# sean-lo/OptimalMatrixCompletion.jl

Measured on AMD Instinct MI355X. Metric: B&B node-relaxations/sec, 100x100 k=1, higher is better.
Workload: dtype f64

## Files before the change

include/omc.h:

```cpp
#ifndef OMC_H
#define OMC_H

#include <stdint.h>

#ifdef __cplusplus
extern "C" {
#endif

#define OMC_VERSION 100

#define OMC_OPTIMAL 0
#define OMC_SLOW_PROGRESS 1
#define OMC_TIME_LIMIT 2
#define OMC_INFEASIBLE 3

#define OMC_CUT_LINEAR 0
#define OMC_CUT_LINEAR2 1
#define OMC_CUT_LINEAR3 2
#define OMC_DIR_LEFT 0
#define OMC_DIR_MIDDLE 1
#define OMC_DIR_RIGHT 2
#define OMC_DIR_INNER_LEFT 3
#define OMC_DIR_INNER_RIGHT 4
#define OMC_SMALLEST_1_EIGVEC 1
// ... 55 lines not shown
                    const double* U_upper, double* objective, double* dual_bound, int* status, int* iters,
                    double* Y, double* U, double* X, double* Theta, double* lambda_min, double* breakpoint_x,
                    double* solve_time);

int omc_relax_stage(omc_instance* h, int B, const omc_relax_params* params, int cut_type, const int* L,
                    const double* cut_x, const double* cut_Uhat, const int8_t* cut_dir, const double* U_lower,
                    const double* U_upper);
int omc_set_node_rho_scales(omc_instance* h, int B, const double* rho_scale);
int omc_relax_solve(omc_instance* h);
int omc_state_pool_create(omc_instance* h, int capacity);
int omc_state_pool_reserve_shor(omc_instance* h, int64_t nq_max);
int omc_relax_set_warm(omc_instance* h, int B, const int* load_from, const int* save_to);
int omc_shor_warm_compat(int64_t n_parent, const int64_t* parent_idx, int64_t n_soc_parent, const int64_t* parent_soc, int64_t n_child,
                         const int64_t* child_idx, int64_t n_soc_child, const int64_t* child_soc);
int omc_last_shor_warm_stats(omc_instance* h, int64_t out[4]);
int omc_state_pool_fetch_shor(omc_instance* h, int entry, int64_t* nq, double* X, double* Theta, double* V);
int omc_relax_submit(omc_instance* h);
int omc_relax_fetch_done(omc_instance* h, int max_nodes, int* node_ids, double* objective, double* dual_bound, int* status, int* iters,
                         double* U, double* lambda_min, double* breakpoint_x, double* Y, int* n_out);
int omc_relax_hold(omc_instance* h, int on);
int omc_relax_reserve(omc_instance* h, int extra_nodes, int max_cuts);
int omc_relax_append(omc_instance* h, int B, const int* L, const double* cut_x, const double* cut_Uhat, const int8_t* cut_dir,
                     const int* load_from, const int* save_to);
int omc_relax_poll(omc_instance* h, int* running, int* nodes_done, int* nodes_total);
int omc_relax_wait(omc_instance* h);
int omc_relax_fetch(omc_instance* h, double* objective, double* dual_bound, int* status, int* iters, double* Y,
                    double* U, double* X, double* Theta, double* lambda_min, double* breakpoint_x,
                    double* solve_time);

int omc_relax_stage_shor(omc_instance* h, int B, const omc_relax_params* params, int cut_type, const int* L,
                         const double* cut_x, const double* cut_Uhat, const int8_t* cut_dir, const double* U_lower,
                         const double* U_upper, const int64_t* n_shor, const int64_t* shor_idx, const int64_t* n_soc,
                         const int64_t* soc_idx);
int omc_relax_fetch_shor(omc_instance* h, double* W );
int omc_set_shor_keep_V(omc_instance* h, int keep);
int omc_relax_fetch_shor_V(omc_instance* h, double* V);
int omc_relax_batch_shor(omc_instance* h, int B, const omc_relax_params* params, int cut_type, const int* L,
                         const double* cut_x, const double* cut_Uhat, const int8_t* cut_dir, const double* U_lower,
                         const double* U_upper, const int64_t* n_shor, const int64_t* shor_idx, const int64_t* n_soc,
                         const int64_t* soc_idx, double* objective, double* dual_bound, int* status, int* iters, double* Y,
                         double* U, double* X, double* Theta, double* W, double* lambda_min, double* breakpoint_x,
                         double* solve_time);
int omc_set_shor_penalties(omc_instance* h, double rho, double r4, double r5);
int omc_relax_reserve_shor(omc_instance* h, int64_t nq_max, int extra_lists);
int omc_relax_append_shor(omc_instance* h, int B, const int* L, const double* cut_x, const double* cut_Uhat, const int8_t* cut_dir,
                          const int64_t* n_shor, const int64_t* shor_idx, const int64_t* n_soc, const int64_t* soc_idx,
                          const int* load_from, const int* save_to);
int omc_relax_fetch_done_shor(omc_instance* h, int n_ids, const int* node_ids, double* X, double* W, double* Theta);

int omc_relax_keep_certificates(omc_instance* h, int on);
int omc_relax_fetch_certificate(omc_instance* h, int n_ids, const int* node_ids, double* Lam, double* lam, int* R, double* Q, int* r,
                                double* Psi3, double* bound);
int omc_certificate_plan(int n, int k, int nnz, int max_cuts, int nonstandard_box_rows, int64_t* out);
int omc_dual_bound_batch(omc_instance* h, int B, int cut_type, int reference_quirk_q1, const int* L, const double* cut_x,
                         const double* cut_Uhat, const int8_t* cut_dir, const double* U_lower, const double* U_upper, const double* Lam,
                         const double* lam, const double* Psi3, double* Q_out, int* r_out, double* bound);

int omc_relax_keep_shor_certificates(omc_instance* h, int on);
int omc_relax_fetch_shor_certificate(omc_instance* h, int n_ids, const int* node_ids, double* scale, double* bound, double* lam, int* R, double* Q,
                                     int* r, double* Psi3, double* Gam, double* zeta, double* xi, double* Xbar, int* nq, int64_t* nq_stride);
int omc_shor_certificate_plan(int n, int m, int k, int64_t nq_stride, int max_cuts, int nonstandard_box_rows, int64_t* out);

int omc_shor_dual_bound_batch(omc_instance* h, int B, int cut_type, int reference_quirk_q1, const int* L, const double* cut_x,
                              const double* cut_Uhat, const int8_t* cut_dir, const double* U_lower, const double* U_upper, const int64_t* n_shor,
                              const int64_t* shor_idx, const int64_t* n_soc, const int64_t* soc_idx, int sanitise, int64_t nq_stride,
                              const double* scale, const double* lam, const double* Psi3, const double* Gam, const double* zeta, const double* xi,
                              const double* Xbar, double* bound, double* defects, double* terms);
int omc_shor_dual_bound_plan(int n, int m, int k, int B, int64_t nq_stride, int max_cuts, int nonstandard_box_rows, int sanitise, int64_t* out);
int omc_last_shor_dual_bound_ms(omc_instance* h, double* ms);

int omc_shor_index_build(omc_instance* h, int where, int64_t nq, const int64_t* shor_idx, int64_t n_soc, const int64_t* soc_idx, int64_t* counts,
                         double* r4, uint64_t* hash, int* mi, int* kid, int* cptr, int* cent, int* v1ptr, int* v1ent, int* v2ptr, int* v2ent,
                         int* slackrow, uint8_t* eclass, uint8_t* ctype);
int omc_shor_index_plan(int n, int m, int64_t nq, int64_t* out);
int omc_last_shor_index_stats(omc_instance* h, double* out);

int omc_altmin_batch(omc_instance* h, int B, int cut_type, int reference_quirk_q1, const int* L,
                     const double* cut_x, const double* cut_Uhat, const int8_t* cut_dir, const double* U_initial,
                     double eps, int max_iters, double time_limit, double* U, double* V, int* converged,
                     int* n_iters, double* objectives, double* solve_time);

int omc_altmin_master_objectives(omc_instance* h, int B, double* objective);
int omc_altmin_plan(int n, int m, int k, int max_cuts, int nolds, int64_t* out);

int omc_evaluate_objective(omc_instance* h, int B, const double* X, double* objective);

int omc_separation_batch(omc_instance* h, int B, int breakpoints, const double* Y, const double* U,
                         double* eigvals, double* x, int* feasible);

int omc_round_Y_batch(omc_instance* h, int B, const double* Y, double* U_rounded);
int omc_left_singular_batch(omc_instance* h, int B, const double* X, double* U_out);

int omc_psd_project_batch(omc_instance* h, int B, int N, const double* M, double lo, double hi, int algo,
                          const double* V0, double* P, double* evals, double* V);
int omc_column_prox_batch(omc_instance* h, int B, int mode, int algo, const double* Y, const double* alpha_old, const double* rho_f,
                          const double* s0, double* alpha, double* s, double* objcol, double* c0col, int* nfact);
int omc_colprox_plan(int n, int cmax, int block_min, int64_t* out);
int omc_last_cone_multi_stats(omc_instance* h, int64_t* out);
int omc_plain_multi_plan(int n, int plain_multi_min, int64_t* out);
double omc_plain_multi_tau(void);
int omc_last_plain_multi_stats(omc_instance* h, int64_t* out);
int omc_cone_multi_budget(int interval_max);
#define OMC_HARVEST_NONE 0
#define OMC_HARVEST_SYNC 1
#define OMC_HARVEST_ASYNC 2
int omc_harvest_plan(int nlive, int nfin, int pending, int check_index, int async_min_live);

int omc_shor_count(omc_instance* h, int n_classes, const int* num_entries_present, int64_t* count_per_class);
int omc_shor_indexes(omc_instance* h, int n_classes, const int* num_entries_present, int64_t capacity, int64_t* out,
                     int64_t* count);
int omc_violated_shor_minors(omc_instance* h, const double* X, int n_classes, const int* num_entries_present,
                             int64_t n_existing, const int64_t* existing, int n_minors, double* scores,
                             int64_t* minors, int* n_out);
int omc_shor_last_stats(omc_instance* h, double* ms, int64_t* candidates);
int omc_shor_last_select_stats(omc_instance* h, int64_t out[4]);

#define OMC_COMM_ID_BYTES 128
int omc_comm_unique_id(void* id_out);
int omc_comm_init(omc_instance* h, int rank, int world_size, const void* id);
int omc_allreduce_bounds(omc_instance* h, double* ub, double* lb, int* owner);
int omc_bcast_incumbent(omc_instance* h, int root, double* X);
int omc_allgather_records(omc_instance* h, const double* rows, int cnt, int width, double* out, int out_capacity_rows, int* counts);
int omc_comm_destroy(omc_instance* h);

#define OMC_KERNEL_COLPROX 0
#define OMC_KERNEL_CONE 1
#define OMC_KERNEL_GLOBAL 2
#define OMC_KERNEL_CHECK 3
#define OMC_KERNEL_SETUP 4
#define OMC_KERNEL_SMALL 5
#define OMC_KERNEL_ACCEL 6
#define OMC_KERNEL_CONESUB 7
#define OMC_KERNEL_CHECK_COL 8
#define OMC_KERNEL_CHECK_BUILD 9
#define OMC_KERNEL_HARVEST 10
#define OMC_KERNEL_SHOR_BIGCONE 11
#define OMC_KERNEL_SHOR_MINORS 12
#define OMC_KERNEL_SHOR_COLS 13
#define OMC_KERNEL_NCLASS 14
int omc_last_solver_info(omc_instance* h, double* info);
#define OMC_RES_CONE_SUB 0
#define OMC_RES_CONE_SUB_CERT 1
#define OMC_RES_CONE_SUB_SEP 2
#define OMC_RES_GLOBAL 3
#define OMC_RES_SMALL 4
#define OMC_RES_COLPROX_PAIR 5
#define OMC_RES_COLPROX_WIDE 6
#define OMC_RES_COLPROX 7
#define OMC_RES_CONE_WS 8
#define OMC_RES_CONE 9
#define OMC_RES_N 10
int omc_kernel_residency(omc_instance* h, int* out);
int omc_last_subspace_stats(omc_instance* h, int64_t* out);
int omc_last_shor_subspace_stats(omc_instance* h, int64_t* out);
int omc_tuning_set(omc_instance* h, const char* name, const char* value);
int omc_tuning_reload_env(omc_instance* h);
int omc_debug_stamps(omc_instance* h, double* out32);
int omc_debug_diag(omc_instance* h, double* out);
int omc_debug_aa(omc_instance* h, int* accepted, int* rejected);
int omc_debug_residuals(omc_instance* h, double* rp, double* rd);
int omc_last_kernel_stats(omc_instance* h, int64_t* launches , double* ms ,
                          int64_t* units );
#define OMC_HOST_CHECK_WAIT 0
#define OMC_HOST_CHECK_SCAN 1
#define OMC_HOST_LIST 2
#define OMC_HOST_EVENT_DRAIN 3
#define OMC_HOST_HARVEST_FLAGS 4
#define OMC_HOST_HARVEST_ENQUEUE 5
#define OMC_HOST_HARVEST_WAIT 6
#define OMC_HOST_HARVEST_BOOK 7
#define OMC_HOST_SETUP_ENQUEUE 8
#define OMC_HOST_CHECK_TOTAL 9
#define OMC_HOST_HARVEST_TOTAL 10
#define OMC_HOST_ASYNC_HARVESTS 11
#define OMC_HOST_QUIET_INTERVALS 12
#define OMC_HOST_BODY_RECORDS 13
#define OMC_HOST_BODY_WAITS 14
#define OMC_HOST_NPHASE 15
int omc_last_host_phases(omc_instance* h, double* ms , int64_t* count );

#ifdef __cplusplus
}
#endif
#endif
```

optimalmatrixcompletion.jl_amd/_lib.py:

```python
from __future__ import annotations

import ctypes as C
import os

import numpy as np

_HERE = os.path.dirname(os.path.abspath(__file__))
LIB_PATH = os.environ.get("OMC_AMD_LIB") or os.path.join(_HERE, "lib", "libomc_hip.so")

EXPORTS = [
    "omc_relax_params_default", "omc_last_error", "omc_version", "omc_device_count", "omc_instance_create",
    "omc_instance_create_bits", "omc_instance_destroy", "omc_relax_batch", "omc_relax_stage", "omc_relax_solve",
    "omc_relax_fetch", "omc_relax_submit", "omc_relax_poll", "omc_relax_wait", "omc_altmin_batch", "omc_evaluate_objective", "omc_separation_batch", "omc_round_Y_batch",
    "omc_last_kernel_stats", "omc_last_host_phases", "omc_kernel_residency", "omc_last_solver_info", "omc_last_subspace_stats", "omc_set_node_rho_scales", "omc_left_singular_batch", "omc_psd_project_batch", "omc_column_prox_batch", "omc_colprox_plan", "omc_last_cone_multi_stats", "omc_cone_multi_budget", "omc_plain_multi_plan", "omc_plain_multi_tau", "omc_last_plain_multi_stats", "omc_harvest_plan", "omc_relax_reserve", "omc_relax_append", "omc_relax_fetch_done", "omc_relax_hold", "omc_debug_stamps", "omc_tuning_set", "omc_tuning_reload_env", "omc_debug_residuals", "omc_debug_diag", "omc_debug_aa",
    "omc_shor_count", "omc_shor_indexes", "omc_violated_shor_minors", "omc_shor_last_stats", "omc_shor_last_select_stats",
    "omc_relax_stage_shor", "omc_relax_fetch_shor", "omc_relax_batch_shor", "omc_set_shor_penalties", "omc_set_shor_keep_V", "omc_relax_fetch_shor_V", "omc_last_shor_subspace_stats", "omc_state_pool_create", "omc_relax_set_warm",
    "omc_state_pool_reserve_shor", "omc_shor_warm_compat", "omc_last_shor_warm_stats", "omc_state_pool_fetch_shor",
    "omc_relax_reserve_shor", "omc_relax_append_shor", "omc_relax_fetch_done_shor",
    "omc_relax_keep_certificates", "omc_relax_fetch_certificate", "omc_certificate_plan", "omc_dual_bound_batch",
    "omc_relax_keep_shor_certificates", "omc_relax_fetch_shor_certificate", "omc_shor_certificate_plan",
    "omc_shor_dual_bound_batch", "omc_shor_dual_bound_plan", "omc_last_shor_dual_bound_ms",
    "omc_shor_index_build", "omc_shor_index_plan", "omc_last_shor_index_stats",
    "omc_altmin_master_objectives", "omc_altmin_plan", "omc_comm_unique_id", "omc_comm_init", "omc_allreduce_bounds", "omc_bcast_incumbent", "omc_allgather_records", "omc_comm_destroy",
]


class RelaxParams(C.Structure):
    _fields_ = [("eps_gap", C.c_double), ("eps_feas", C.c_double), ("max_iters", C.c_int), ("check_every", C.c_int),
                ("rho_scale", C.c_double), ("rho_f_ratio", C.c_double), ("relax", C.c_double), ("time_limit", C.c_double),
                ("reference_quirk_q1", C.c_int), ("breakpoints", C.c_int), ("stall_checks", C.c_int), ("bump_max", C.c_int), ("bump_ratio", C.c_double),
                ("bump_factor", C.c_double), ("bump_after", C.c_int), ("bump_window", C.c_int), ("slots", C.c_int),
                ("accel", C.c_int), ("aa_mem", C.c_int), ("aa_every", C.c_int), ("aa_start", C.c_int), ("aa_reg", C.c_double), ("aa_safeguard", C.c_double), ("first_wins", C.c_int),
                ("early_stop_after", C.c_int), ("early_stop_factor", C.c_double)]


class OmcError(RuntimeError):
    def __init__(self, code, msg):
        super().__init__(f"libomc_hip error {code}: {msg}")
        self.code = code


_lib = None


def load():
    global _lib
    if _lib is not None:
        return _lib
    if not os.path.exists(LIB_PATH):
        raise OmcError(-100, f"{LIB_PATH} not found: build it first (__graft_entry__.build()); there is no CPU fallback")
    lib = C.CDLL(LIB_PATH)
    dp = C.POINTER(C.c_double); ip = C.POINTER(C.c_int); vp = C.c_void_p
    lib.omc_last_error.restype = C.c_char_p
    lib.omc_version.restype = C.c_int
    lib.omc_device_count.restype = C.c_int
    lib.omc_relax_params_default.argtypes = [C.POINTER(RelaxParams)]
    lib.omc_instance_create.argtypes = [C.c_int, C.c_int, C.c_int, vp, vp, C.c_double, C.c_int, C.POINTER(vp)]
    lib.omc_instance_create_bits.argtypes = [C.c_int, C.c_int, C.c_int, vp, vp, C.c_double, C.c_int, C.POINTER(vp)]
    lib.omc_instance_destroy.argtypes = [vp]
    lib.omc_instance_destroy.restype = None
    lib.omc_relax_batch.argtypes = [vp, C.c_int, C.POINTER(RelaxParams), C.c_int] + [vp] * 17
    lib.omc_relax_stage.argtypes = [vp, C.c_int, C.POINTER(RelaxParams), C.c_int] + [vp] * 6
    lib.omc_relax_solve.argtypes = [vp]
    lib.omc_relax_stage_shor.argtypes = [vp, C.c_int, C.POINTER(RelaxParams), C.c_int] + [vp] * 10
    lib.omc_relax_fetch_shor.argtypes = [vp, vp]
    lib.omc_relax_batch_shor.argtypes = [vp, C.c_int, C.POINTER(RelaxParams), C.c_int] + [vp] * 22
    lib.omc_set_shor_penalties.argtypes = [vp, C.c_double, C.c_double, C.c_double]
    lib.omc_set_shor_keep_V.argtypes = [vp, C.c_int]
    lib.omc_relax_fetch_shor_V.argtypes = [vp, vp]
    lib.omc_last_shor_subspace_stats.argtypes = [vp, vp]
    lib.omc_state_pool_create.argtypes = [vp, C.c_int]
    lib.omc_relax_set_warm.argtypes = [vp, C.c_int, vp, vp]
    lib.omc_state_pool_reserve_shor.argtypes = [vp, C.c_int64]
    lib.omc_shor_warm_compat.argtypes = [C.c_int64, vp, C.c_int64, vp, C.c_int64, vp, C.c_int64, vp]
    lib.omc_last_shor_warm_stats.argtypes = [vp, vp]
    lib.omc_state_pool_fetch_shor.argtypes = [vp, C.c_int, vp, vp, vp, vp]
    lib.omc_relax_submit.argtypes = [vp]
    lib.omc_relax_poll.argtypes = [vp, vp, vp, vp]
    lib.omc_relax_wait.argtypes = [vp]
    lib.omc_relax_fetch.argtypes = [vp] + [vp] * 11
    lib.omc_altmin_batch.argtypes = [vp, C.c_int, C.c_int, C.c_int, vp, vp, vp, vp, vp, C.c_double, C.c_int, C.c_double,
                                     vp, vp, vp, vp, vp, vp]
    lib.omc_evaluate_objective.argtypes = [vp, C.c_int, vp, vp]
    lib.omc_separation_batch.argtypes = [vp, C.c_int, C.c_int, vp, vp, vp, vp, vp]
    lib.omc_round_Y_batch.argtypes = [vp, C.c_int, vp, vp]
    lib.omc_last_kernel_stats.argtypes = [vp, vp, vp, vp]
    lib.omc_last_solver_info.argtypes = [vp, vp]
    if hasattr(lib, "omc_last_host_phases"):
        lib.omc_last_host_phases.argtypes = [vp, vp, vp]
    if hasattr(lib, "omc_kernel_residency"):
        lib.omc_kernel_residency.argtypes = [vp, vp]
    lib.omc_last_subspace_stats.argtypes = [vp, vp]
    lib.omc_set_node_rho_scales.argtypes = [vp, C.c_int, vp]
    lib.omc_debug_stamps.argtypes = [vp, vp]
    lib.omc_left_singular_batch.argtypes = [vp, C.c_int, vp, vp]
    lib.omc_psd_project_batch.argtypes = [vp, C.c_int, C.c_int, vp, C.c_double, C.c_double, C.c_int, vp, vp, vp, vp]
    if hasattr(lib, "omc_column_prox_batch"):
        lib.omc_column_prox_batch.argtypes = [vp, C.c_int, C.c_int, C.c_int] + [vp] * 9
        lib.omc_colprox_plan.argtypes = [C.c_int, C.c_int, C.c_int, vp]
    lib.omc_last_cone_multi_stats.argtypes = [vp, vp]
    lib.omc_cone_multi_budget.argtypes = [C.c_int]
    if hasattr(lib, "omc_plain_multi_plan"):
        lib.omc_plain_multi_plan.argtypes = [C.c_int, C.c_int, vp]
        lib.omc_plain_multi_tau.argtypes = []
        lib.omc_plain_multi_tau.restype = C.c_double
        lib.omc_last_plain_multi_stats.argtypes = [vp, vp]
    if hasattr(lib, "omc_harvest_plan"):
        lib.omc_harvest_plan.argtypes = [C.c_int] * 5
    lib.omc_relax_reserve.argtypes = [vp, C.c_int, C.c_int]
    lib.omc_relax_hold.argtypes = [vp, C.c_int]
    lib.omc_relax_fetch_done.argtypes = [vp, C.c_int, vp, vp, vp, vp, vp, vp, vp, vp, vp, vp]
    lib.omc_relax_append.argtypes = [vp, C.c_int, vp, vp, vp, vp, vp, vp]
    lib.omc_relax_reserve_shor.argtypes = [vp, C.c_int64, C.c_int]
    lib.omc_relax_append_shor.argtypes = [vp, C.c_int] + [vp] * 10
    lib.omc_relax_fetch_done_shor.argtypes = [vp, C.c_int, vp, vp, vp, vp]
    if hasattr(lib, "omc_relax_keep_certificates"):
        lib.omc_relax_keep_certificates.argtypes = [vp, C.c_int]
        lib.omc_relax_fetch_certificate.argtypes = [vp, C.c_int] + [vp] * 8
        lib.omc_certificate_plan.argtypes = [C.c_int] * 5 + [vp]
        lib.omc_dual_bound_batch.argtypes = [vp, C.c_int, C.c_int, C.c_int] + [vp] * 12
    if hasattr(lib, "omc_relax_keep_shor_certificates"):
        lib.omc_relax_keep_shor_certificates.argtypes = [vp, C.c_int]
        lib.omc_relax_fetch_shor_certificate.argtypes = [vp, C.c_int] + [vp] * 14
        lib.omc_shor_certificate_plan.argtypes = [C.c_int, C.c_int, C.c_int, C.c_int64, C.c_int, C.c_int, vp]
    if hasattr(lib, "omc_shor_dual_bound_batch"):
        lib.omc_shor_dual_bound_batch.argtypes = [vp, C.c_int, C.c_int, C.c_int] + [vp] * 10 + [C.c_int, C.c_int64] + [vp] * 10
        lib.omc_shor_dual_bound_plan.argtypes = [C.c_int] * 4 + [C.c_int64, C.c_int, C.c_int, C.c_int, vp]
        lib.omc_last_shor_dual_bound_ms.argtypes = [vp, vp]
    if hasattr(lib, "omc_shor_index_build"):
        lib.omc_shor_index_build.argtypes = [vp, C.c_int, C.c_int64, vp, C.c_int64] + [vp] * 15
        lib.omc_shor_index_plan.argtypes = [C.c_int, C.c_int, C.c_int64, vp]
        lib.omc_last_shor_index_stats.argtypes = [vp, vp]
    lib.omc_tuning_set.argtypes = [vp, C.c_char_p, C.c_char_p]
    lib.omc_tuning_reload_env.argtypes = [vp]
    lib.omc_debug_residuals.argtypes = [vp, vp, vp]
    lib.omc_debug_diag.argtypes = [vp, vp]
    lib.omc_debug_aa.argtypes = [vp, vp, vp]
    lib.omc_shor_count.argtypes = [vp, C.c_int, vp, vp]
    lib.omc_shor_indexes.argtypes = [vp, C.c_int, vp, C.c_int64, vp, vp]
    lib.omc_violated_shor_minors.argtypes = [vp, vp, C.c_int, vp, C.c_int64, vp, C.c_int, vp, vp, vp]
    lib.omc_shor_last_stats.argtypes = [vp, vp, vp]
    lib.omc_shor_last_select_stats.argtypes = [vp, vp]
    lib.omc_altmin_master_objectives.argtypes = [vp, C.c_int, vp]
    lib.omc_altmin_plan.argtypes = [C.c_int, C.c_int, C.c_int, C.c_int, C.c_int, vp]
    lib.omc_comm_unique_id.argtypes = [vp]
    lib.omc_comm_init.argtypes = [vp, C.c_int, C.c_int, vp]
    lib.omc_allreduce_bounds.argtypes = [vp, vp, vp, vp]
    lib.omc_bcast_incumbent.argtypes = [vp, C.c_int, vp]
    lib.omc_allgather_records.argtypes = [vp, vp, C.c_int, C.c_int, vp, C.c_int, vp]
    lib.omc_comm_destroy.argtypes = [vp]
    _lib = lib
    return lib


def check(rc):
    if rc != 0:
        raise OmcError(rc, load().omc_last_error().decode("utf-8", "replace"))


def ptr(a):
    return None if a is None else a.ctypes.data_as(C.c_void_p)


def f64(a, order="F"):
    return np.require(np.asarray(a, dtype=np.float64), requirements=["ALIGNED"] + (["F_CONTIGUOUS"] if order == "F" else ["C_CONTIGUOUS"]))
```

optimalmatrixcompletion.jl_amd/api.py:

```python
from __future__ import annotations

import atexit
import weakref
import ctypes as C

import numpy as np

from . import _lib, certificate
from ._lib import RelaxParams, OmcError

CUT_TYPES = {"linear": 0, "linear2": 1, "linear3": 2}
DIR_CODES = {"left": 0, "middle": 1, "right": 2, "inner_left": 3, "inner_right": 4}
BREAKPOINTS = {"smallest_1_eigvec": 1, "smallest_2_eigvec": 2}
STATUS_NAMES = {0: "OPTIMAL", 1: "SLOW_PROGRESS", 2: "TIME_LIMIT", 3: "INFEASIBLE"}
KERNEL_CLASSES = ["colprox", "cone", "global", "check", "setup", "small", "accel", "cone_sub", "check_col", "check_build", "harvest",
                  "shor_bigcone", "shor_minors", "shor_cols"]
HOST_PHASES = ["check_wait", "check_scan", "list", "event_drain", "harvest_flags", "harvest_enqueue", "harvest_wait", "harvest_book",
               "setup_enqueue", "check_total", "harvest_total", "async_harvests", "quiet_intervals", "body_records", "body_waits"]
HOST_BODY_COUNTS = ("body_records", "body_waits")
RESIDENCY_KERNELS = ["k_cone_sub<0>", "k_cone_sub<1>", "k_cone_sub<2>", "k_global", "k_small", "k_colprox_pair", "k_colprox_wide", "k_colprox",
                     "k_cone_ws", "k_cone"]


def default_params(**kw) -> RelaxParams:
# ... 253 lines not shown
        _lib.check(self._lib.omc_relax_reserve(self._h, int(extra_nodes), int(max_cuts)))

    def append(self, nodes, disjunctive_cuts_type="linear", load_from=None, save_to=None):
        n, k = self.n, self.k
        L, cx, cU, cd = _pack_cuts(nodes, n, k, disjunctive_cuts_type)
        lf = None if load_from is None else np.ascontiguousarray(np.asarray(load_from, dtype=np.int32))
        sv = None if save_to is None else np.ascontiguousarray(np.asarray(save_to, dtype=np.int32))
        if (lf is not None and lf.shape != (len(nodes),)) or (sv is not None and sv.shape != (len(nodes),)):
            raise ValueError("load_from / save_to must hold one pool index per node")
        _lib.check(self._lib.omc_relax_append(self._h, len(nodes), _lib.ptr(L), _lib.ptr(cx), _lib.ptr(cU), _lib.ptr(cd), _lib.ptr(lf), _lib.ptr(sv)))
        self._B += len(nodes)

    def reserve_shor(self, nq_max, extra_lists):
        _lib.check(self._lib.omc_relax_reserve_shor(self._h, int(nq_max), int(extra_lists)))
        self._reserved_nq = int(nq_max)

    def append_shor(self, nodes, shor_info, disjunctive_cuts_type="linear", load_from=None, save_to=None):
        n, k = self.n, self.k
        if len(shor_info) != len(nodes):
            raise ValueError("one Shor_info per node")
        L, cx, cU, cd = _pack_cuts(nodes, n, k, disjunctive_cuts_type)
        lf = None if load_from is None else np.ascontiguousarray(np.asarray(load_from, dtype=np.int32))
        sv = None if save_to is None else np.ascontiguousarray(np.asarray(save_to, dtype=np.int32))
        if (lf is not None and lf.shape != (len(nodes),)) or (sv is not None and sv.shape != (len(nodes),)):
            raise ValueError("load_from / save_to must hold one pool index per node")
        nsh, nso, shi, soi = _pack_shor(shor_info)
        _lib.check(self._lib.omc_relax_append_shor(self._h, len(nodes), _lib.ptr(L), _lib.ptr(cx), _lib.ptr(cU), _lib.ptr(cd), _lib.ptr(nsh),
                                                   _lib.ptr(shi), _lib.ptr(nso), _lib.ptr(soi), _lib.ptr(lf), _lib.ptr(sv)))
        self._B += len(nodes)

    def fetch_done_shor(self, ids, want_W=False, want_Theta=False):
        n, m = self.n, self.m
        idv = np.ascontiguousarray(np.asarray(list(ids), dtype=np.int32))
        c = len(idv)
        X = np.zeros((max(c, 1), n * m)); W = np.zeros((max(c, 1), n * m)) if want_W else None; Th = np.zeros((max(c, 1), m * m)) if want_Theta else None
        _lib.check(self._lib.omc_relax_fetch_done_shor(self._h, c, _lib.ptr(idv), _lib.ptr(X), _lib.ptr(W), _lib.ptr(Th)))
        out = []
        for i in range(c):
            d = dict(node=int(idv[i]), X=X[i].reshape((n, m), order="F"))
            if want_W:
                d["W"] = W[i].reshape((n, m), order="F")
            if want_Theta:
                d["Theta"] = Th[i].reshape((m, m), order="F")
            out.append(d)
        return out

    def hold(self, on=True):
        _lib.check(self._lib.omc_relax_hold(self._h, 1 if on else 0))

    def fetch_done(self, max_nodes=4096, want_Y=False):
        n, k = self.n, self.k
        key = (int(max_nodes), bool(want_Y))
        if getattr(self, "_fd_key", None) != key:
            self._fd_key = key
            self._fd = (np.zeros(max_nodes, np.int32), np.zeros(max_nodes), np.zeros(max_nodes), np.zeros(max_nodes, np.int32), np.zeros(max_nodes, np.int32),
                        np.zeros((max_nodes, n * k)), np.zeros((max_nodes, 2)), np.zeros((max_nodes, n)), np.zeros(1, np.int32),
                        np.zeros((max_nodes, n * n)) if want_Y else None)
        ids, obj, lb, st, it, U, ev, bx, cnt, Y = self._fd
        _lib.check(self._lib.omc_relax_fetch_done(self._h, int(max_nodes), _lib.ptr(ids), _lib.ptr(obj), _lib.ptr(lb), _lib.ptr(st), _lib.ptr(it),
                                                  _lib.ptr(U), _lib.ptr(ev), _lib.ptr(bx), _lib.ptr(Y), _lib.ptr(cnt)))
        out = []
        for i in range(int(cnt[0])):
            d = dict(node=int(ids[i]), objective=float(obj[i]), dual_bound=float(lb[i]), status_code=int(st[i]), termination_status=STATUS_NAMES[int(st[i])],
                     feasible=int(st[i]) != 3, iters=int(it[i]), U=U[i].reshape((n, k), order="F").copy(), lambda_min=ev[i].copy(), breakpoint_vec=bx[i].copy())
            if want_Y:
                d["Y"] = Y[i].reshape((n, n), order="F").copy()
            out.append(d)
        return out

    def solve(self):
        _lib.check(self._lib.omc_relax_solve(self._h))

    def submit(self):
        _lib.check(self._lib.omc_relax_submit(self._h))

    def poll(self):
        r = np.zeros(3, np.int32)
        _lib.check(self._lib.omc_relax_poll(self._h, _lib.ptr(r[0:1]), _lib.ptr(r[1:2]), _lib.ptr(r[2:3])))
        return dict(running=bool(r[0]), nodes_done=int(r[1]), nodes_total=int(r[2]))

    def wait(self):
        _lib.check(self._lib.omc_relax_wait(self._h))

    def fetch(self, want_Y=True, want_X=True, want_Theta=False):
        B, n, m, k = self._B, self.n, self.m, self.k
        obj = np.zeros(B); lb = np.zeros(B); st = np.zeros(B, np.int32); it = np.zeros(B, np.int32)
        Y = np.zeros((B, n * n)) if want_Y else None
        U = np.zeros((B, n * k))
        X = np.zeros((B, n * m)) if want_X else None
        Th = np.zeros((B, m * m)) if want_Theta else None
        lmin = np.zeros((B, 2)); bx = np.zeros((B, n)); tm = np.zeros(B)
        _lib.check(self._lib.omc_relax_fetch(self._h, _lib.ptr(obj), _lib.ptr(lb), _lib.ptr(st), _lib.ptr(it), _lib.ptr(Y),
                                             _lib.ptr(U), _lib.ptr(X), _lib.ptr(Th), _lib.ptr(lmin), _lib.ptr(bx), _lib.ptr(tm)))
        out = []
        for b in range(B):
            r = {
                "objective": float(obj[b]), "dual_bound": float(lb[b]), "termination_status": STATUS_NAMES[int(st[b])],
                "status_code": int(st[b]), "feasible": int(st[b]) != 3, "iters": int(it[b]), "solve_time": float(tm[b]),
                "U": U[b].reshape((n, k), order="F"), "lambda_min": lmin[b].copy(), "breakpoint_vec": bx[b].copy(),
            }
            if want_Y: r["Y"] = Y[b].reshape((n, n), order="F")
            if want_X: r["X"] = X[b].reshape((n, m), order="F")
            if want_Theta: r["Theta"] = Th[b].reshape((m, m), order="F")
            out.append(r)
        return out

    def matrix_completion_SDP_relaxation(self, nodes, disjunctive_cuts_type="linear", params=None, U_lower=None, U_upper=None,
                                         want_Y=True, want_X=True, want_Theta=False, rho_scales=None, add_Shor_valid_inequalities=False,
                                         shor_info=None, shor_penalties=None, want_V=False, load_from=None, save_to=None):
        if add_Shor_valid_inequalities:
            if shor_info is None:
                raise ValueError("add_Shor_valid_inequalities = true needs node.Shor_info (OMC.jl:1508)")
            self.stage_shor(nodes, shor_info, disjunctive_cuts_type, params, U_lower, U_upper, shor_penalties, keep_V=(want_V and self.k == 1),
                            load_from=load_from, save_to=save_to)
            self.solve()
            out = self.fetch(want_Y, want_X, want_Theta)
            for r, Wb in zip(out, self.fetch_shor()):
                r["W"] = Wb
            if want_V and self.k == 1:
                for r, Vb, (mi, _) in zip(out, self.fetch_shor_V(), shor_info):
                    r["V"] = Vb[:len(np.asarray(mi).reshape(-1, 4))]
            elif want_V:
                for r, (mi, _) in zip(out, shor_info):
                    r.update(shor_rank_k_extension(self.k, r["X"], r["W"], mi))
            return out
        self.stage(nodes, disjunctive_cuts_type, params, U_lower, U_upper, rho_scales, load_from, save_to)
        self.solve()
        return self.fetch(want_Y, want_X, want_Theta)

    def kernel_stats(self):
        nc = len(KERNEL_CLASSES); la = np.zeros(nc, np.int64); ms = np.zeros(nc); un = np.zeros(nc, np.int64)
        _lib.check(self._lib.omc_last_kernel_stats(self._h, _lib.ptr(la), _lib.ptr(ms), _lib.ptr(un)))
        return {KERNEL_CLASSES[i]: dict(launches=int(la[i]), ms=float(ms[i]), units=int(un[i])) for i in range(nc)}

    def host_phases(self):
        if not hasattr(self._lib, "omc_last_host_phases"):
            raise OmcError(-100, "this build of the library has no omc_last_host_phases")
        ms = np.zeros(len(HOST_PHASES)); cnt = np.zeros(len(HOST_PHASES), np.int64)
        _lib.check(self._lib.omc_last_host_phases(self._h, _lib.ptr(ms), _lib.ptr(cnt)))
        return {HOST_PHASES[i]: dict(ms=float(ms[i]), count=int(cnt[i])) for i in range(len(HOST_PHASES)) if HOST_PHASES[i] not in HOST_BODY_COUNTS}

    def event_counts(self):
        if not hasattr(self._lib, "omc_last_host_phases"):
            raise OmcError(-100, "this build of the library has no omc_last_host_phases")
        ms = np.zeros(len(HOST_PHASES)); cnt = np.zeros(len(HOST_PHASES), np.int64)
        _lib.check(self._lib.omc_last_host_phases(self._h, _lib.ptr(ms), _lib.ptr(cnt)))
        return {name[len("body_"):]: int(cnt[HOST_PHASES.index(name)]) for name in HOST_BODY_COUNTS}

    def subspace_stats(self):
        out = np.zeros(8, np.int64)
        _lib.check(self._lib.omc_last_subspace_stats(self._h, _lib.ptr(out)))
        return dict(calls=int(out[0]), power_steps=int(out[1]), fallbacks=int(out[2]), seeds=int(out[3]), fail_positive=int(out[4]),
                    fail_steps=int(out[5]), fail_cholesky=int(out[6]), ritz_passes=int(out[7]))

    def shor_subspace_stats(self):
        out = np.zeros(8, np.int64)
        _lib.check(self._lib.omc_last_shor_subspace_stats(self._h, _lib.ptr(out)))
        return dict(calls=int(out[0]), power_steps=int(out[1]), fallbacks=int(out[2]), seeds=int(out[3]), fail_positive=int(out[4]),
                    fail_steps=int(out[5]), fail_cholesky=int(out[6]), ritz_passes=int(out[7]))

    def kernel_residency(self):
        out = np.zeros(len(RESIDENCY_KERNELS), np.int32)
        _lib.check(self._lib.omc_kernel_residency(self._h, _lib.ptr(out)))
        return {nm: int(v) for nm, v in zip(RESIDENCY_KERNELS, out)}

    def solver_info(self):
        info = np.zeros(8)
        _lib.check(self._lib.omc_last_solver_info(self._h, _lib.ptr(info)))
        return dict(solve_seconds=info[0], jacobi_sweeps=int(info[1]), rho=info[2], r_max=int(info[3]), cone_lds=bool(info[4]),
                    global_lds=bool(info[5]), small_lds=bool(info[6]), R_max=int(info[7]))

    def keep_certificates(self, on=True):
        _lib.check(self._lib.omc_relax_keep_certificates(self._h, 1 if on else 0))

    def certificate_plan(self, max_cuts=0, nonstandard_box_rows=0):
        return certificate_plan(self.n, self.k, int(self.indices.sum()), max_cuts, nonstandard_box_rows)

    def _support(self):
        cols, rows = np.nonzero(self.indices.T)
        return rows, cols

    def fetch_certificate(self, ids):
        n, m, k = self.n, self.m, self.k
        idv = np.ascontiguousarray(np.asarray(list(ids), dtype=np.int32))
        c = len(idv)
        info = self.solver_info()
        Rmax, rmax = max(info["R_max"], 1), max(info["r_max"], 1)
        rows, cols = self._support()
        nnz = rows.size
        ps = (rmax + k) ** 2
        Lam = np.zeros((max(c, 1), max(nnz, 1))); lam = np.zeros((max(c, 1), Rmax)); R = np.zeros(max(c, 1), np.int32)
        Q = np.zeros((max(c, 1), n * rmax)); r = np.zeros(max(c, 1), np.int32); Psi = np.zeros((max(c, 1), ps)); bd = np.zeros(max(c, 1))
        if nnz:
            Lam = np.zeros((max(c, 1), nnz))
        _lib.check(self._lib.omc_relax_fetch_certificate(self._h, c, _lib.ptr(idv), _lib.ptr(Lam), _lib.ptr(lam), _lib.ptr(R), _lib.ptr(Q),
                                                         _lib.ptr(r), _lib.ptr(Psi), _lib.ptr(bd)))
        out = []
        for i in range(c):
            ri = int(r[i]); N3 = ri + k
            dense = np.zeros((n, m)); dense[rows, cols] = Lam[i, :nnz]
            out.append(certificate.Certificate(Lam=dense, lam=lam[i, :int(R[i])].copy(), Q=Q[i, :n * ri].reshape((n, ri), order="F").copy(),
                                               Psi3=Psi[i, :N3 * N3].reshape((N3, N3), order="F").copy(), bound=float(bd[i])))
        return out

    def keep_shor_certificates(self, on=True):
        _lib.check(self._lib.omc_relax_keep_shor_certificates(self._h, 1 if on else 0))

    def shor_certificate_plan(self, nq_stride, max_cuts=0, nonstandard_box_rows=0):
        return shor_certificate_plan(self.n, self.m, self.k, nq_stride, max_cuts, nonstandard_box_rows)

    def fetch_shor_certificate(self, ids):
        n, m, k = self.n, self.m, self.k
        idv = np.ascontiguousarray(np.asarray(list(ids), dtype=np.int32))
        c = len(idv); c1 = max(c, 1)
        stride = np.zeros(1, np.int64)
        _lib.check(self._lib.omc_relax_fetch_shor_certificate(self._h, 0, None, *([None] * 12), _lib.ptr(stride)))
        ns = int(stride[0])
        info = self.solver_info()
        Rmax, rmax = max(info["R_max"], 1), max(info["r_max"], 1)
        ps = (rmax + k) ** 2
        sc = np.zeros(c1); bd = np.zeros(c1); lam = np.zeros((c1, Rmax)); R = np.zeros(c1, np.int32); Q = np.zeros((c1, n * rmax)); r = np.zeros(c1, np.int32)
        Psi = np.zeros((c1, ps)); Gam = np.zeros((c1, 15 * max(ns, 1))); zeta = np.zeros((c1, m)); xi = np.zeros((c1, n * m)); Xb = np.zeros((c1, n * m))
        nq = np.zeros(c1, np.int32)
        _lib.check(self._lib.omc_relax_fetch_shor_certificate(self._h, c, _lib.ptr(idv), _lib.ptr(sc), _lib.ptr(bd), _lib.ptr(lam), _lib.ptr(R), _lib.ptr(Q),
                                                              _lib.ptr(r), _lib.ptr(Psi), _lib.ptr(Gam) if ns else None, _lib.ptr(zeta), _lib.ptr(xi), _lib.ptr(Xb),
                                                              _lib.ptr(nq), None))
        out = []
        for i in range(c):
            ri = int(r[i]); N3 = ri + k
            G = certificate.unpack_gam(Gam[i, :15 * ns].reshape(15, ns), int(nq[i])) if ns else np.zeros((0, 5, 5))
            out.append(certificate.ShorCertificate(scale=float(sc[i]), lam=lam[i, :int(R[i])].copy(), Q=Q[i, :n * ri].reshape((n, ri), order="F").copy(),
                                                   Psi3=Psi[i, :N3 * N3].reshape((N3, N3), order="F").copy(), Gam=G, zeta=zeta[i].copy(),
                                                   xi=xi[i].reshape((n, m), order="F").copy(), Xbar=Xb[i].reshape((n, m), order="F").copy(),
                                                   bound=float(bd[i])))
        return out

    def _bounds_flat(self, B, U_lower, U_upper):
        lo = hi = None
        if U_lower is not None:
            lo = np.ascontiguousarray(np.stack([np.asfortranarray(np.asarray(u, float)).ravel(order="F") for u in U_lower]))
        if U_upper is not None:
            hi = np.ascontiguousarray(np.stack([np.asfortranarray(np.asarray(u, float)).ravel(order="F") for u in U_upper]))
        for a in (lo, hi):
            if a is not None and a.shape != (B, self.n * self.k):
                raise ValueError("U_lower / U_upper: one (n, k) matrix per node")
        return lo, hi

    def row_basis(self, nodes, disjunctive_cuts_type="linear", U_lower=None, U_upper=None, reference_quirk_q1=True):
        n, k, B = self.n, self.k, len(nodes)
        L, cx, cU, cd = _pack_cuts(nodes, n, k, disjunctive_cuts_type)
        lo, hi = self._bounds_flat(B, U_lower, U_upper)
        args = (self._h, B, CUT_TYPES[disjunctive_cuts_type], int(bool(reference_quirk_q1)), _lib.ptr(L), _lib.ptr(cx), _lib.ptr(cU), _lib.ptr(cd),
                _lib.ptr(lo), _lib.ptr(hi), None, None, None)
        r = np.zeros(B, np.int32)
        _lib.check(self._lib.omc_dual_bound_batch(*args, None, _lib.ptr(r), None))
        rmax = max(1, int(r.max()))
        Q = np.zeros((B, n * rmax))
        _lib.check(self._lib.omc_dual_bound_batch(*args, _lib.ptr(Q), _lib.ptr(r), None))
        return [Q[b, :n * int(r[b])].reshape((n, int(r[b])), order="F").copy() for b in range(B)]

    def dual_bound(self, nodes, certs, disjunctive_cuts_type="linear", U_lower=None, U_upper=None, reference_quirk_q1=True):
        n, m, k, B = self.n, self.m, self.k, len(nodes)
        if len(certs) != B:
            raise ValueError("one certificate per node")
        L, cx, cU, cd = _pack_cuts(nodes, n, k, disjunctive_cuts_type)
        lo, hi = self._bounds_flat(B, U_lower, U_upper)
        dlo, dhi = certificate.default_U_bounds(n, k)
        Rb = []
        for b in range(B):
            lb_ = dlo if lo is None else lo[b]; hb_ = dhi if hi is None else hi[b]
            Rb.append(1 + int((np.asarray(lb_) > -1.0).sum()) + int((np.asarray(hb_) < 1.0).sum()) + int(L[b]) * (2 * k + 1))
        rb = [int(np.asarray(c.Q).shape[1]) for c in certs]
        Rmax, rmax = max(Rb), max(1, max(rb))
        rows, cols = self._support()
        nnz = rows.size
        ps = (rmax + k) ** 2
        Lam = np.zeros((B, max(nnz, 1))); lam = np.zeros((B, Rmax)); Psi = np.zeros((B, ps))
        for b, c in enumerate(certs):
            if np.asarray(c.Lam).shape != (n, m) or len(c.lam) != Rb[b] or np.asarray(c.Psi3).shape != (rb[b] + k, rb[b] + k):
                raise ValueError(f"certificate {b}: Lam must be n x m, lam hold {Rb[b]} multipliers and Psi3 be of order r + k")
            Lam[b, :nnz] = np.asarray(c.Lam, float)[rows, cols]; lam[b, :Rb[b]] = c.lam
            Psi[b, :(rb[b] + k) ** 2] = np.asarray(c.Psi3, float).ravel(order="F")
        r = np.zeros(B, np.int32); bd = np.zeros(B)
        _lib.check(self._lib.omc_dual_bound_batch(self._h, B, CUT_TYPES[disjunctive_cuts_type], int(bool(reference_quirk_q1)), _lib.ptr(L), _lib.ptr(cx),
                                                  _lib.ptr(cU), _lib.ptr(cd), _lib.ptr(lo), _lib.ptr(hi), None, None, None, None, _lib.ptr(r), None))
        if [int(v) for v in r] != rb:
            raise ValueError(f"Q of the certificates has {rb} columns, the library's row basis {[int(v) for v in r]}: build Psi3 in the basis of row_basis()")
        _lib.check(self._lib.omc_dual_bound_batch(self._h, B, CUT_TYPES[disjunctive_cuts_type], int(bool(reference_quirk_q1)), _lib.ptr(L), _lib.ptr(cx),
                                                  _lib.ptr(cU), _lib.ptr(cd), _lib.ptr(lo), _lib.ptr(hi), _lib.ptr(Lam), _lib.ptr(lam), _lib.ptr(Psi),
                                                  None, None, _lib.ptr(bd)))
        return bd

    def shor_dual_bound(self, nodes, shor_info, certs, disjunctive_cuts_type="linear", U_lower=None, U_upper=None, reference_quirk_q1=True,
                        sanitise=True, want_defects=False, want_terms=False, nq_stride=None):
        if not hasattr(self._lib, "omc_shor_dual_bound_batch"):
            raise _lib.OmcError(-100, "this libomc_hip.so has no omc_shor_dual_bound_batch")
        n, m, k, B = self.n, self.m, self.k, len(nodes)
        if len(certs) != B or len(shor_info) != B:
            raise ValueError("one certificate and one (minors, SOC list) pair per node")
        L, cx, cU, cd = _pack_cuts(nodes, n, k, disjunctive_cuts_type)
        lo, hi = self._bounds_flat(B, U_lower, U_upper)
        nsh, nso, shi, soi = _pack_shor(shor_info)
        dlo, dhi = certificate.default_U_bounds(n, k)
        Rb = []
        for b in range(B):
            lb_ = dlo if lo is None else lo[b]; hb_ = dhi if hi is None else hi[b]
# ... 281 lines not shown
```

optimalmatrixcompletion.jl_amd/csrc/omc_api.cpp:

```cpp
#include <hip/hip_runtime.h>
#include <stdint.h>
#include <limits.h>
#include <stdio.h>
#include <stdlib.h>
#include <string.h>
#include <math.h>
#include <string>
#include <vector>
#include <algorithm>
#include <atomic>
#include <thread>
#include <mutex>
#include <execinfo.h>
#include <signal.h>
#include <unistd.h>

#include "omc_altmin.h"
#include "omc_api_internal.h"

thread_local std::string g_err;

static void knob_set(Tuning& t, const Knob& kb, const char* value) {
  if (kb.flag) t.*kb.flag = value != nullptr;
  else t.*kb.num = value ? atoi(value) : Tuning{}.*kb.num;
// ... 286 lines not shown
  return 0;
}

int put_descriptors(const OmcWS& w, const NodePack& pk, int B, size_t rows, size_t first, const int* L, const double* cut_x, hipStream_t s) {
  const size_t n = w.n, k = w.k, Rm = w.Rmax, Lm = w.Lmax, rm = w.rmax;
  std::vector<int> hR(rows, 0), hrr(rows, 0), hk(rows * Rm, 0), hc(rows * Rm, 0), hbi(rows * Rm, 0), hbj(rows * Rm, 0);
  std::vector<double> hcoef(rows * Rm * k, 0.0), hrhs(rows * Rm, 0.0), hx(rows * Lm * n, 0.0), hQ(rows * n * rm, 0.0);
  long cutbase = 0;
  for (int b = 0; b < B; ++b) {
    hR[b] = (int)pk.rk[b].size();
    for (int r = 0; r < hR[b]; ++r) {
      hk[(size_t)b * Rm + r] = pk.rk[b][r]; hc[(size_t)b * Rm + r] = pk.rc[b][r];
      hbi[(size_t)b * Rm + r] = pk.rbi[b][r]; hbj[(size_t)b * Rm + r] = pk.rbj[b][r];
      hrhs[(size_t)b * Rm + r] = pk.rrhs[b][r];
      for (size_t j = 0; j < k; ++j) hcoef[((size_t)b * Rm + r) * k + j] = pk.rcoef[b][(size_t)r * k + j];
    }
    const int Lb = L ? L[b] : 0;
    for (int l = 0; l < Lb; ++l) memcpy(&hx[((size_t)b * Lm + l) * n], cut_x + (size_t)(cutbase + l) * n, sizeof(double) * n);
    cutbase += Lb;
    memcpy(&hQ[(size_t)b * n * rm], pk.Qn[b].data(), sizeof(double) * pk.Qn[b].size());
    hrr[b] = pk.rrv[b];
  }
  HIPCHK(hipMemcpyAsync(w.R + first, hR.data(), sizeof(int) * hR.size(), hipMemcpyHostToDevice, s));
  HIPCHK(hipMemcpyAsync(w.rkind + first * Rm, hk.data(), sizeof(int) * hk.size(), hipMemcpyHostToDevice, s));
  HIPCHK(hipMemcpyAsync(w.rcut + first * Rm, hc.data(), sizeof(int) * hc.size(), hipMemcpyHostToDevice, s));
  HIPCHK(hipMemcpyAsync(w.rbi + first * Rm, hbi.data(), sizeof(int) * hbi.size(), hipMemcpyHostToDevice, s));
  HIPCHK(hipMemcpyAsync(w.rbj + first * Rm, hbj.data(), sizeof(int) * hbj.size(), hipMemcpyHostToDevice, s));
  HIPCHK(hipMemcpyAsync(w.rcoef + first * Rm * k, hcoef.data(), 8 * hcoef.size(), hipMemcpyHostToDevice, s));
  HIPCHK(hipMemcpyAsync(w.rrhs + first * Rm, hrhs.data(), 8 * hrhs.size(), hipMemcpyHostToDevice, s));
  HIPCHK(hipMemcpyAsync(w.cutx + first * Lm * n, hx.data(), 8 * hx.size(), hipMemcpyHostToDevice, s));
  HIPCHK(hipMemcpyAsync(w.Qb + first * n * rm, hQ.data(), 8 * hQ.size(), hipMemcpyHostToDevice, s));
  HIPCHK(hipMemcpyAsync(w.rr + first, hrr.data(), sizeof(int) * hrr.size(), hipMemcpyHostToDevice, s));
  HIPCHK(hipStreamSynchronize(s));
  return 0;
}

static constexpr int CP_SERIES = 6;
static constexpr int CP_MAXPASS = 60;
static constexpr int SUB_GUARD = 2;
static constexpr int SUB_CHUNK = 3;
static constexpr double SUB_TOL = 1e-10;
static constexpr double SUB_ADAPT = 1e-3;

int check_cut_type(int cut_type) {
  if (cut_type != OMC_CUT_LINEAR && cut_type != OMC_CUT_LINEAR2 && cut_type != OMC_CUT_LINEAR3)
    return fail(OMC_ERR_INVALID_ENUM, "Invalid input for disjunctive cuts type: must be linear, linear2 or linear3 (OMC.jl:1456-1462)");
  return 0;
}

int stage_base(omc_instance* h, int B, const omc_relax_params* params, int cut_type, const int* L, const double* cut_x, const double* cut_Uhat,
                      const int8_t* cut_dir, const double* U_lower, const double* U_upper, const StageMode& mode) {
  if (!h) return fail(OMC_ERR_ARGUMENT, "handle is NULL");
  if (B <= 0) return fail(OMC_ERR_ARGUMENT, "B must be positive");
  { int rcc = check_cut_type(cut_type); if (rcc) return rcc; }
  HIPCHK(hipSetDevice(h->device));
  h->staged = false;
  const bool shor = mode.shor;
  h->shor_on = false; h->shor_via_base = false;
  if (params) h->params = *params; else omc_relax_params_default(&h->params);
  if (shor) {
    h->params.early_stop_factor = 0.0;
    h->params.stall_checks = std::max(h->params.stall_checks, 40);
    h->params.bump_max = std::min(h->params.bump_max, 1);
    h->params.first_wins = 0; h->params.accel = 0;
  }
  const omc_relax_params& P = h->params;
  if (P.breakpoints != OMC_SMALLEST_1_EIGVEC && P.breakpoints != OMC_SMALLEST_2_EIGVEC)
    return fail(OMC_ERR_INVALID_ENUM, "Invalid input for disjunctive cuts breakpoints (OMC.jl:2440-2446)");
  const int n = h->n, m = h->m, k = h->k;
  NodePack pk;
  { int rcp = pack_nodes(h, P, cut_type, B, L, cut_x, cut_Uhat, cut_dir, U_lower, U_upper, pk); if (rcp) return rcp; }
  int Rmax = pk.Rmax, rmax = pk.rmax, Lmax = pk.Lmax;
  const int extra_nodes = h->reserve_nodes, extra_cuts = h->reserve_cuts;
  h->reserve_nodes = 0; h->reserve_cuts = 0;
  if (extra_nodes > 0) {
    Lmax = std::max(Lmax, extra_cuts);
    Rmax = std::max(Rmax, 1 + k * (k + 1) / 2 + extra_cuts * (2 * k + 1));
    rmax = std::max(rmax, std::min(n, k + extra_cuts));
  }
  OmcWS& w = h->ws;
  memset(&w, 0, sizeof(w));
  const int Bcap = B + extra_nodes;
  const int S = (P.slots > 0) ? std::min(P.slots, Bcap) : std::min(Bcap, 256);
  h->Btot = B; h->Btot_live.store(B); h->node_cap = B + extra_nodes; h->staged_cut_type = cut_type; { std::lock_guard<std::mutex> lk(h->append_mu); h->append_closed = false; }
  { std::lock_guard<std::mutex> lk(h->done_mu); h->done_q.clear(); h->done_read = 0; }
  h->hold.store(0);
  w.nB = S;
  w.B = S; w.Btot = B; w.max_iters = P.max_iters; w.n = n; w.m = m; w.k = k; w.nnz = h->nnz; w.Rmax = Rmax; w.Lmax = std::max(Lmax, 1); w.rmax = rmax;
  w.max_sweeps = MAX_SWEEPS;
  w.breakpoints = P.breakpoints; w.stall_checks = P.stall_checks > 0 ? P.stall_checks : 1000000;
  w.gamma = h->gamma; w.sumA2 = h->sumA2;
  {
    const double sh = 1.0 + h->gamma * (double)k / (double)n;
    w.rho = P.rho_scale * 0.5 * h->gamma * h->sumA2 / ((double)m * sh * sh);
  }
  if (shor) w.rho = h->shor_rho * P.rho_scale;
  if (!(w.rho > 0.0)) w.rho = 1.0;
  w.clip_hi = 1.0; w.inv_s2 = 1.0; w.shor = 0;
  w.rho_f_ratio = P.rho_f_ratio;
  w.bump_max = P.bump_max; w.bump_ratio = P.bump_ratio; w.bump_factor = P.bump_factor; w.bump_after = P.bump_after;
  w.bump_gap = P.bump_window * std::max(1, P.check_every);
  w.accel = P.accel ? 1 : 0; w.aa_mem = std::max(2, std::min(P.aa_mem, AA_MAXMEM)); w.aa_every = std::max(1, P.aa_every);
  w.aa_start = std::max(2, P.aa_start); w.aa_reg = P.aa_reg; w.aa_safeguard = P.aa_safeguard;
  {
    std::vector<double> hr((size_t)B + extra_nodes, w.rho);
    if (h->rho_scale_per_node.size() == (size_t)B)
      for (int b = 0; b < B; ++b) hr[b] = w.rho / P.rho_scale * h->rho_scale_per_node[b];
    h->rho_scale_per_node.clear();
    int r0 = upload(h->brhon, hr.data(), sizeof(double) * hr.size(), h->stream); if (r0) return r0;
    HIPCHK(hipStreamSynchronize(h->stream));
    w.rho_node = h->brhon.as<double>();
    BIND(h->brho, w.rho_b, (size_t)S);
  }
  w.relax = P.relax; w.eps_gap = P.eps_gap; w.eps_feas = P.eps_feas;
  w.check_every = std::max(1, P.check_every); w.early_stop_after = P.early_stop_after; w.early_stop_factor = (P.first_wins ? 0.0 : P.early_stop_factor);
  const StageDims sd = {(size_t)S, (size_t)B + (size_t)extra_nodes, (size_t)n, (size_t)m, (size_t)k, (size_t)h->nnz, (size_t)rmax, (size_t)Rmax};
  {
    ENS_CARVE(h->bgap, [&](Carve& c) { walk_gap(c, sd, w); });
    BIND(h->bvotes, w.slow_votes, (size_t)S);
    ENS(h->bslotlist, sizeof(int) * (size_t)S);
    w.slot_list = nullptr;
  }
  std::vector<double> wY((size_t)n * n);
  for (size_t e = 0; e < (size_t)n * n; ++e) wY[e] = shor ? 3.0 : P.rho_f_ratio * h->Ncnt[e] + 2.0;
  int rc_ = 0;
  if ((rc_ = upload(h->dwY, wY.data(), sizeof(double) * n * n, h->stream))) return rc_;
  w.col_ptr = h->dcol_ptr.as<int>(); w.col_idx = h->dcol_idx.as<int>(); w.col_val = h->dcol_val.as<double>();
  {
    const bool pair_on = !h->tun.no_colprox_pair && mode.colprox_force != 2;
    if ((rc_ = build_colprox_lists(h, mode.colprox_force == 1 ? INT_MAX : mode.colprox_force == 2 ? 1 : h->tun.colprox_block_min, pair_on))) return rc_;
    w.cp_pair = pair_on ? 1 : 0;
  }
  w.cp_nblock = h->nblock; w.cp_block = h->nblock ? h->dblock.as<int>() : nullptr;
  w.cp_nslab = h->nslab; w.cp_slab = h->nslab ? h->dslab.as<int>() : nullptr;
  w.cp_isblock = (h->nblock + h->nslab) ? h->disblock.as<unsigned char>() : nullptr; w.cp_nrest = h->nrest; w.cp_nfact = nullptr;
  w.cone_512 = h->tun.cone_512 ? 1 : 0; w.cp_series = CP_SERIES; w.cp_maxpass = CP_MAXPASS; w.cp_xcd = h->tun.colprox_no_xcd ? 0 : 1;
  w.cp_nsolo = h->nsolo; w.cp_solo = h->nsolo ? h->dsolo.as<int>() : nullptr;
  w.cp_nwide = h->nwide; w.cp_wide = h->nwide ? h->dwide.as<int>() : nullptr;
  w.Ncnt = h->dNcnt.as<double>(); w.wY1 = h->dwY.as<double>();
  w.row_ptr = h->drow_ptr.as<int>(); w.row_idx = h->drow_idx.as<int>();
  const size_t sB = (size_t)S;
  const size_t sN = (size_t)B + (size_t)extra_nodes;
  hipStream_t s0 = h->stream;
  const size_t nn = (size_t)n * n, nk = (size_t)n * k, nz = (size_t)h->nnz;
  BIND(h->bY, w.Y, sB * nn); BIND(h->bYp, w.Yp, sB * nn); BIND(h->bU, w.U, sB * nk);
  BIND(h->bD1, w.D1, sB * nn); BIND(h->bD3, w.D3, sB * nn); BIND(h->bW1, w.W1, sB * nn); BIND(h->bE3, w.E3, sB * nn);
  BIND(h->bdS, w.dS, sB * rmax * rmax);
  ENS_CARVE(h->bsm, [&](Carve& c) { walk_small_cone(c, sd, w); });
  BIND(h->balpha, w.alpha, sB * nz); BIND(h->balphaX, w.alphaX, sB * nz); BIND(h->bsval, w.sval, sB * m);
  BIND(h->bMchk, w.Mchk, sB * nn);
  size_t chk_bytes = 0;
  ENS_CARVE(h->bchk, [&](Carve& c) { walk_check(c, sd, w); }, &chk_bytes);
  BIND(h->bG, w.G, sB * Rmax * Rmax); BIND(h->blam, w.lam, sB * Rmax);
  ENS_CARVE(h->bscal, [&](Carve& c) { walk_scalars(c, sd, w); });
  BIND(h->bbx, w.bx, sB * n);
  ENS_CARVE(h->bint, [&](Carve& c) { walk_slot_ints(c, sd, w); });
  w.np16 = (n + 15) & ~15;
  const size_t pp = (size_t)w.np16 * w.np16, p16 = (size_t)w.np16 * 16;
  BIND(h->bMbuf, w.Mbuf, sB * pp); BIND(h->bVrow, w.Vrow, sB * pp);
  BIND(h->blamD, w.lamD, sB * m * n, s0);
  w.lamDX = nullptr;
  if (n > 144 || shor) BIND(h->blamDX, w.lamDX, sB * m * n, s0);
  {
    size_t subS_bytes = 0, subI_bytes = 0;
    BIND(h->bXs, w.Xs, sB * p16, s0);
    ENS_CARVE(h->bsubS, [&](Carve& c) { walk_sub_doubles(c, sd, w); }, &subS_bytes);
    ENS_CARVE(h->bsubI, [&](Carve& c) { walk_sub_ints(c, sd, w); }, &subI_bytes);
    HIPCHK(hipMemsetAsync(h->bsubS.p, 0, subS_bytes, s0));
    HIPCHK(hipMemsetAsync(h->bsubI.p, 0, subI_bytes, s0));
    w.ws_phase = 0;
    w.sub_guard = SUB_GUARD; w.sub_qmax = h->tun.sub_qmax; w.sub_chunk = SUB_CHUNK;
    w.sub_tol = SUB_TOL; w.sub_adapt = SUB_ADAPT; w.sub_debug = h->tun.sub_debug;
    w.sub_enable = 0;
    size_t subSC_bytes = 0, subIC_bytes = 0;
    BIND(h->bXsC, w.XsC, sB * p16, s0);
    ENS_CARVE(h->bsubSC, [&](Carve& c) { walk_subC_doubles(c, sd, w); }, &subSC_bytes);
    ENS_CARVE(h->bsubIC, [&](Carve& c) { walk_subC_ints(c, sd, w); }, &subIC_bytes);
    HIPCHK(hipMemsetAsync(h->bsubSC.p, 0, subSC_bytes, s0));
    HIPCHK(hipMemsetAsync(h->bsubIC.p, 0, subIC_bytes, s0));
    w.cert_enable = 0;
  }
  BIND(h->bMbufC, w.MbufC, sB * pp, s0); BIND(h->bVrowC, w.VrowC, sB * pp, s0); BIND(h->bchkS, w.fro2c, sB); BIND(h->bchkI, w.vvalidC, sB, s0);
  w.Yx = nullptr;
  if (!shor && !P.accel) BIND(h->bYx, w.Yx, sB * nn);
  w.skip_yp = (w.Yx && !h->tun.dense_proj) ? 1 : 0;
  ENS_CARVE(h->bobjcol, [&](Carve& c) { walk_objcol(c, sd, w); });
  if (w.accel) {
    w.aa_dim = 4 * n * n + 2 * rmax * k + k * k + h->nnz;
    const size_t ring = sB * (size_t)(w.aa_mem + 1) * w.aa_dim;
    size_t aaI_bytes = 0;
    BIND(h->baaF, w.aa_F, ring); BIND(h->baaG, w.aa_G, ring); BIND(h->baaZ, w.aa_zin, sB * (size_t)w.aa_dim); BIND(h->baaS, w.aa_fn, sB);
    ENS_CARVE(h->baaI, [&](Carve& c) { walk_aa_ints(c, sd, w); }, &aaI_bytes);
    HIPCHK(hipMemsetAsync(h->baaI.p, 0, aaI_bytes, s0));
  }
  HIPCHK(hipMemsetAsync(w.ws_need, 0, sizeof(int), s0));
  {
    size_t map_bytes = 0;
    ENS_CARVE(h->bslotint, [&](Carve& c) { walk_slot_map(c, sd, w.node_of, w.init, w.fin); }, &map_bytes);
    std::vector<int> hs(map_bytes / sizeof(int));
    int *h_node = nullptr, *h_init = nullptr, *h_fin = nullptr;
    { Carve hc(hs.data()); walk_slot_map(hc, sd, h_node, h_init, h_fin); }
    for (size_t b = 0; b < sB; ++b) { h_node[b] = (int)b; h_init[b] = 1; h_fin[b] = 1; }
    HIPCHK(hipMemcpyAsync(h->bslotint.p, hs.data(), map_bytes, hipMemcpyHostToDevice, h->stream));
    HIPCHK(hipStreamSynchronize(h->stream));
    BIND(h->boY, w.oY, sN * nn); BIND(h->boU, w.oU, sN * nk); BIND(h->boal, w.oalphaX, sN * nz); BIND(h->bobx, w.obx, sN * n);
    ENS_CARVE(h->boscal, [&](Carve& c) { walk_out_scalars(c, sd, w); });
    ENS_CARVE(h->boint, [&](Carve& c) { walk_out_ints(c, sd, w); });
  }
  if ((h->keep_cert && !shor) || (h->keep_shor_cert && shor)) {
    const size_t cnnz = shor ? 0 : (size_t)h->nnz;
    size_t cbD_bytes = 0, cbI_bytes = 0, ocD_bytes = 0;
    ENS_CARVE(h->bcbD, [&](Carve& c) { walk_cert_slot(c, sd, cnnz, w); }, &cbD_bytes);
    ENS_CARVE(h->bcbI, [&](Carve& c) { walk_cert_flags(c, sd, w); }, &cbI_bytes);
    ENS_CARVE(h->bocD, [&](Carve& c) { walk_cert_node(c, sd, cnnz, w); }, &ocD_bytes);
    BIND(h->bocI, w.ocHave, sN, s0);
    HIPCHK(hipMemsetAsync(h->bcbD.p, 0, cbD_bytes, s0)); HIPCHK(hipMemsetAsync(h->bcbI.p, 0, cbI_bytes, s0));
    HIPCHK(hipMemsetAsync(h->bocD.p, 0, ocD_bytes, s0));
    if (shor) { w.cbLam = nullptr; w.ocLam = nullptr; }
  }
  w.load_from = nullptr; w.save_to = nullptr;
  const bool warm_ok = !shor || mode.warm_filtered;
  if (h->pool_cap > 0 && warm_ok && extra_nodes > 0) {
    if (h->warm_load.size() != (size_t)B) h->warm_load.assign(B, -1);
    if (h->warm_save.size() != (size_t)B) h->warm_save.assign(B, -1);
    h->warm_load.resize(sN, -1); h->warm_save.resize(sN, -1);
  } else if (extra_nodes == 0) {
    if (h->warm_load.size() != (size_t)B) h->warm_load.clear();
    if (h->warm_save.size() != (size_t)B) h->warm_save.clear();
  }
  h->save_host.assign(sN, -1);
  if (h->pool_cap > 0 && !shor && h->warm_load.size() == sN) {
    std::lock_guard<std::mutex> lk(h->sig_mu);
    for (int& e : h->warm_load) if (e >= 0 && (size_t)e < h->pool_sig.size() && h->pool_sig[e].kind == 2) e = -1;
  }
  if (h->pool_cap > 0 && warm_ok && (h->warm_load.size() == sN || h->warm_save.size() == sN)) {
    if (h->warm_save.size() == sN) h->save_host = h->warm_save;
    if (h->warm_load.size() == sN) { if ((rc_ = upload(h->bwarmL, h->warm_load.data(), sizeof(int) * sN, h->stream))) return rc_; w.load_from = h->bwarmL.as<int>(); }
    if (h->warm_save.size() == sN) { if ((rc_ = upload(h->bwarmS, h->warm_save.data(), sizeof(int) * sN, h->stream))) return rc_; w.save_to = h->bwarmS.as<int>(); }
    HIPCHK(hipStreamSynchronize(h->stream));
    w.pY = h->pY.as<double>(); w.pD1 = h->pD1.as<double>(); w.pD3 = h->pD3.as<double>(); w.pU = h->pU.as<double>(); w.palpha = h->palpha.as<double>();
    w.psval = h->psval.as<double>(); w.pXs = h->pXs.as<double>(); w.ptheta = h->ptheta.as<double>(); w.pscal = h->pscal.as<double>();
  }
  h->warm_load.clear(); h->warm_save.clear();
  BIND(h->bQb, w.Qb, sN * n * rmax); BIND(h->brr, w.rr, sN); BIND(h->bR, w.R, sN);
  BIND(h->brkind, w.rkind, sN * Rmax); BIND(h->brcut, w.rcut, sN * Rmax); BIND(h->brbi, w.rbi, sN * Rmax); BIND(h->brbj, w.rbj, sN * Rmax);
  BIND(h->brcoef, w.rcoef, sN * Rmax * k); BIND(h->brrhs, w.rrhs, sN * Rmax); BIND(h->bcutx, w.cutx, sN * w.Lmax * n);
  if ((rc_ = put_descriptors(w, pk, B, sN, 0, L, cut_x, h->stream))) return rc_;
  w.geo = omc_plan_geometry(n, w.np16, k, rmax, Rmax, h->cmax, h->tun.global_nolds, h->tun.cone_multi_min, h->tun.plain_multi_min);
  BIND(h->bmwstat, w.mw_stat, sB * 4, s0);
  w.mw_budget = MAX_SWEEPS; w.ev_out = nullptr;
  w.pmw_stat = nullptr;
  if (w.geo.plain_mw) BIND(h->bpmwstat, w.pmw_stat, sB * 4, s0);
  geom_set_cpblock(w.geo, h->cpb_cl, h->cpb_cs);
  w.geo.cp_scratch_stride = h->crest_max > w.geo.cp_lds_c ? cp_body_layout(h->crest_max).doubles : 0;
  if (w.geo.cpb_slab_stride && !shor) BIND(h->bcpb, w.cp_bslab, sB * h->nslab * w.geo.cpb_slab_stride);
  if (w.geo.cp_scratch_stride) BIND(h->bcp, w.cp_scratch, sB * m * w.geo.cp_scratch_stride);
  if (w.geo.ws.slab_stride) BIND(h->bcone, w.cone_scratch, sB * w.geo.ws.slab_stride);
  if (w.geo.glob.slab_stride) BIND(h->bglob, w.glob_scratch, sB * w.geo.glob.slab_stride);
  if (w.geo.small.slab_stride) BIND(h->bsmall, w.small_scratch, sB * w.geo.small.slab_stride);
  w.sub_enable = (w.geo.ws_lpp && n >= 48 && w.geo.sub_lds <= OMC_MAX_DYN_LDS && !h->tun.no_subspace) ? 1 : 0;
  w.sub_zscratch = nullptr;
  if (w.sub_enable && w.np16 > 512) BIND(h->bsubz, w.sub_zscratch, sB * 16 * (size_t)(w.np16 + 2));
  w.cert_enable = (w.sub_enable && w.np16 > 512) ? 1 : 0;
  if (!w.sub_enable) w.sep_done = nullptr;
  if (!(!shor && w.sub_enable && w.geo.glob.use_lds && glob_w1_fits(n) && !h->tun.dense_proj)) w.w1_fac = nullptr;
  HIPCHK(hipMemsetAsync(w.sweeps, 0, sizeof(int) * S, s0));
  HIPCHK(hipMemsetAsync(w.stamps, 0, (size_t)((char*)h->bchk.p + chk_bytes - (char*)w.stamps), s0));
  HIPCHK(hipStreamSynchronize(h->stream));
  h->staged = true;
  return 0;
}

int omc_relax_stage(omc_instance* h, int B, const omc_relax_params* params, int cut_type, const int* L,
                    const double* cut_x, const double* cut_Uhat, const int8_t* cut_dir, const double* U_lower,
                    const double* U_upper) {
  return stage_base(h, B, params, cut_type, L, cut_x, cut_Uhat, cut_dir, U_lower, U_upper, StageMode{});
}

int omc_set_node_rho_scales(omc_instance* h, int B, const double* rho_scale) {
  if (!h || B <= 0 || !rho_scale) return fail(OMC_ERR_ARGUMENT, "NULL argument");
  for (int b = 0; b < B; ++b) if (!(rho_scale[b] > 0.0)) return fail(OMC_ERR_ARGUMENT, "rho_scale must be positive");
  h->rho_scale_per_node.assign(rho_scale, rho_scale + B);
  return 0;
}

int omc_state_pool_create(omc_instance* h, int capacity) {
  if (!h) return fail(OMC_ERR_ARGUMENT, "handle is NULL");
  if (capacity < 0) return fail(OMC_ERR_ARGUMENT, "capacity must be non-negative");
  HIPCHK(hipSetDevice(h->device));
  const size_t c = (size_t)capacity, n = h->n, k = h->k, np16 = (h->n + 15) & ~15;
  if (capacity > 0) {
    ENS(h->pY, c * n * n * 8); ENS(h->pD1, c * n * n * 8); ENS(h->pD3, c * n * n * 8); ENS(h->pU, c * n * k * 8); ENS(h->palpha, c * (size_t)h->nnz * 8);
    ENS(h->psval, c * (size_t)h->m * 8); ENS(h->pXs, c * np16 * 16 * 8); ENS(h->ptheta, c * 16 * 8); ENS(h->pscal, c * 4 * 8);
  }
  h->pool_cap = capacity;
  { std::lock_guard<std::mutex> lk(h->sig_mu); h->pool_sig.assign(c, omc_instance::PoolSig{}); }
  h->pool_shor = false; h->pool_nqmax = 0;
  return 0;
}

int omc_relax_set_warm(omc_instance* h, int B, const int* load_from, const int* save_to) {
  if (!h || B <= 0) return fail(OMC_ERR_ARGUMENT, "omc_relax_set_warm: bad arguments");
  if (h->pool_cap <= 0) return fail(OMC_ERR_ARGUMENT, "omc_relax_set_warm: no state pool (omc_state_pool_create)");
  h->warm_load.clear(); h->warm_save.clear();
  for (int b = 0; b < B; ++b) {
    if (load_from && load_from[b] >= h->pool_cap) return fail(OMC_ERR_ARGUMENT, "load_from index beyond the pool");
// ... 118 lines not shown
int require_finished_ids(omc_instance* h, int n_ids, const int* ids, bool upto_read_only, const char* who) {
  bool ended = false;
  if (!upto_read_only) { std::lock_guard<std::mutex> lk(h->append_mu); ended = h->append_closed; }
  std::lock_guard<std::mutex> lk(h->done_mu);
  std::vector<char> seen((size_t)std::max(h->node_cap, 1), 0);
  const size_t upto = ended ? h->done_q.size() : h->done_read;
  for (size_t i = 0; i < upto; ++i) if ((size_t)h->done_q[i] < seen.size()) seen[h->done_q[i]] = 1;
  for (int i = 0; i < n_ids; ++i)
    if (ids[i] < 0 || (size_t)ids[i] >= seen.size() || !seen[ids[i]])
      return fail(OMC_ERR_ARGUMENT, std::string(who) + ": node " + std::to_string(ids[i]) +
                                        (upto_read_only ? " is out of range or has not been returned by omc_relax_fetch_done"
                                                        : " is out of range or has not finished (omc_relax_fetch_done has not returned it)"));
  return 0;
}

int require_certificates(const OmcWS& w, int n_ids, const int* ids, hipStream_t fs, const char* who) {
  std::vector<int> have(n_ids, 0);
  for (int i = 0; i < n_ids; ++i) HIPCHK(hipMemcpyAsync(&have[i], w.ocHave + ids[i], sizeof(int), hipMemcpyDeviceToHost, fs));
  HIPCHK(hipStreamSynchronize(fs));
  for (int i = 0; i < n_ids; ++i)
    if (!have[i]) return fail(OMC_ERR_ARGUMENT, std::string(who) + ": node " + std::to_string(ids[i]) + " never reached a rigorous check (no certificate)");
  return 0;
}

int omc_relax_submit(omc_instance* h) {
  if (!h || !h->staged) return fail(OMC_ERR_ARGUMENT, "omc_relax_submit: nothing staged");
  if (h->worker.joinable()) return fail(OMC_ERR_ARGUMENT, "omc_relax_submit: a solve is already in flight (call omc_relax_wait first)");
  h->nodes_done.store(0); h->worker_running.store(1); h->worker_rc = 0; h->worker_err.clear();
  h->worker = std::thread([h]() {
    const int rc = omc_relax_solve(h);
    h->worker_rc = rc;
    if (rc) h->worker_err = g_err;
    h->worker_running.store(0);
  });
  return 0;
}

int omc_relax_poll(omc_instance* h, int* running, int* nodes_done, int* nodes_total) {
  if (!h) return fail(OMC_ERR_ARGUMENT, "handle is NULL");
  if (running) *running = h->worker_running.load();
  if (nodes_done) *nodes_done = h->nodes_done.load();
  if (nodes_total) *nodes_total = h->Btot_live.load();
  return 0;
}

int omc_relax_wait(omc_instance* h) {
  if (!h) return fail(OMC_ERR_ARGUMENT, "handle is NULL");
  if (!h->worker.joinable()) return fail(OMC_ERR_ARGUMENT, "omc_relax_wait: no solve in flight");
  h->worker.join();
  if (h->worker_rc) g_err = h->worker_err;
  return h->worker_rc;
}

int omc_relax_fetch(omc_instance* h, double* objective, double* dual_bound, int* status, int* iters, double* Y,
                    double* U, double* X, double* Theta, double* lambda_min, double* breakpoint_x, double* solve_time) {
  if (!h || !h->staged) return fail(OMC_ERR_ARGUMENT, "omc_relax_fetch: nothing staged");
  HIPCHK(hipSetDevice(h->device));
  const OmcWS& w = h->ws;
  const size_t B = w.Btot, n = w.n, m = w.m, k = w.k;
  hipStream_t s = h->stream;
  if (objective) HIPCHK(hipMemcpyAsync(objective, w.oobj, 8 * B, hipMemcpyDeviceToHost, s));
  if (dual_bound) HIPCHK(hipMemcpyAsync(dual_bound, w.olb, 8 * B, hipMemcpyDeviceToHost, s));
  if (status) HIPCHK(hipMemcpyAsync(status, w.ostatus, 4 * B, hipMemcpyDeviceToHost, s));
  if (iters) HIPCHK(hipMemcpyAsync(iters, w.oiters, 4 * B, hipMemcpyDeviceToHost, s));
  if (Y) HIPCHK(hipMemcpyAsync(Y, w.oY, 8 * B * n * n, hipMemcpyDeviceToHost, s));
  if (U) HIPCHK(hipMemcpyAsync(U, w.oU, 8 * B * n * k, hipMemcpyDeviceToHost, s));
  if (lambda_min) HIPCHK(hipMemcpyAsync(lambda_min, w.olmin, 8 * 2 * B, hipMemcpyDeviceToHost, s));
  if (breakpoint_x) HIPCHK(hipMemcpyAsync(breakpoint_x, w.obx, 8 * B * n, hipMemcpyDeviceToHost, s));
  if (h->shor_on) {
    if (X) HIPCHK(hipMemcpyAsync(X, h->sh.oX, 8 * B * n * m, hipMemcpyDeviceToHost, s));
    if (Theta) HIPCHK(hipMemcpyAsync(Theta, h->sh.oTh, 8 * B * m * m, hipMemcpyDeviceToHost, s));
  } else if (X || Theta) {
    double *dX = nullptr, *dTh = nullptr;
    BIND(h->bXout, dX, B * n * m);
    omc_launch_make_X(&w, dX, s);
    if (X) HIPCHK(hipMemcpyAsync(X, dX, 8 * B * n * m, hipMemcpyDeviceToHost, s));
    if (Theta) {
      BIND(h->bThout, dTh, B * m * m);
      omc_launch_make_Theta(&w, dX, dTh, s);
      HIPCHK(hipMemcpyAsync(Theta, dTh, 8 * B * m * m, hipMemcpyDeviceToHost, s));
    }
  }
  HIPCHK(hipStreamSynchronize(s));
  if (solve_time) for (size_t b = 0; b < B; ++b) solve_time[b] = h->last_solve_seconds;
  return 0;
}

int omc_relax_batch(omc_instance* h, int B, const omc_relax_params* params, int cut_type, const int* L,
                    const double* cut_x, const double* cut_Uhat, const int8_t* cut_dir, const double* U_lower,
                    const double* U_upper, double* objective, double* dual_bound, int* status, int* iters, double* Y,
                    double* U, double* X, double* Theta, double* lambda_min, double* breakpoint_x, double* solve_time) {
  int rc = omc_relax_stage(h, B, params, cut_type, L, cut_x, cut_Uhat, cut_dir, U_lower, U_upper);
  if (rc) return rc;
  rc = omc_relax_solve(h);
  if (rc) return rc;
  return omc_relax_fetch(h, objective, dual_bound, status, iters, Y, U, X, Theta, lambda_min, breakpoint_x, solve_time);
}

int omc_debug_residuals(omc_instance* h, double* rp, double* rd) {
  if (!h || !rp || !rd || !h->ws.rp) return fail(OMC_ERR_ARGUMENT, "nothing staged");
  HIPCHK(hipMemcpy(rp, h->ws.rp, 8 * (size_t)h->ws.B, hipMemcpyDeviceToHost));
  HIPCHK(hipMemcpy(rd, h->ws.rd, 8 * (size_t)h->ws.B, hipMemcpyDeviceToHost));
  return 0;
}

int omc_tuning_set(omc_instance* h, const char* name, const char* value) {
  if (!h || !name) return fail(OMC_ERR_ARGUMENT, "omc_tuning_set: handle or name is NULL");
  for (const Knob& kb : OMC_KNOBS) if (!strcmp(kb.name, name)) { knob_set(h->tun, kb, value); return 0; }
  return fail(OMC_ERR_ARGUMENT, "omc_tuning_set: unknown knob");
}

int omc_tuning_reload_env(omc_instance* h) {
  if (!h) return fail(OMC_ERR_ARGUMENT, "handle is NULL");
  tuning_from_env(h->tun);
  return 0;
}

int omc_debug_stamps(omc_instance* h, double* out32) {
  if (!h || !out32 || !h->ws.stamps) return fail(OMC_ERR_ARGUMENT, "no stamps");
  if (h->tun.sub_debug == 3 && h->ws.B >= 8) {
    HIPCHK(hipMemcpy(out32, h->ws.stamps, 96 * 8, hipMemcpyDeviceToHost));
    return 0;
  }
  HIPCHK(hipMemcpy(out32, h->ws.stamps, 32 * 8, hipMemcpyDeviceToHost));
  return 0;
}

int omc_debug_aa(omc_instance* h, int* accepted, int* rejected) {
  if (!h || !accepted || !rejected || !h->ws.accel || !h->ws.aa_nacc) return fail(OMC_ERR_ARGUMENT, "acceleration is off or nothing staged");
  HIPCHK(hipMemcpy(accepted, h->ws.aa_nacc, 4 * (size_t)h->ws.B, hipMemcpyDeviceToHost));
  HIPCHK(hipMemcpy(rejected, h->ws.aa_nrej, 4 * (size_t)h->ws.B, hipMemcpyDeviceToHost));
  return 0;
}

int omc_debug_diag(omc_instance* h, double* out ) {
  if (!h || !out || !h->ws.stamps) return fail(OMC_ERR_ARGUMENT, "no diagnostics");
  HIPCHK(hipMemcpy(out, h->ws.stamps + 32, 8 * 8 * (size_t)h->ws.B, hipMemcpyDeviceToHost));
  return 0;
}

int omc_last_host_phases(omc_instance* h, double* ms, int64_t* count) {
  if (!h || !ms || !count) return fail(OMC_ERR_ARGUMENT, "NULL argument");
  for (int q = 0; q < OMC_HOST_NPHASE; ++q) { ms[q] = h->host_ms[q]; count[q] = h->host_cnt[q]; }
  return 0;
}

int omc_last_solver_info(omc_instance* h, double* info) {
  if (!h || !info) return fail(OMC_ERR_ARGUMENT, "NULL argument");
  info[0] = h->last_solve_seconds; info[1] = (double)h->total_sweeps; info[2] = h->ws.rho; info[3] = (double)h->ws.rmax;
  info[4] = (double)h->ws.geo.cone.use_lds; info[5] = (double)h->ws.geo.glob.use_lds; info[6] = (double)h->ws.geo.small.use_lds; info[7] = (double)h->ws.Rmax;
  return 0;
}

int omc_last_subspace_stats(omc_instance* h, int64_t* out) {
  if (!h || !out) return fail(OMC_ERR_ARGUMENT, "NULL argument");
  for (int q = 0; q < 8; ++q) out[q] = h->sub_tot[q];
  return 0;
}

int omc_kernel_residency(omc_instance* h, int* out) {
  if (!h || !out) return fail(OMC_ERR_ARGUMENT, "NULL argument");
  if (!h->ws.geo.sub_lds) return fail(OMC_ERR_ARGUMENT, "omc_kernel_residency: nothing staged yet (the geometry is planned by omc_relax_stage)");
  HIPCHK(hipSetDevice(h->device));
  omc_query_residency(&h->ws, out);
  return 0;
}

int omc_last_kernel_stats(omc_instance* h, int64_t* launches, double* ms, int64_t* units) {
  if (!h) return fail(OMC_ERR_ARGUMENT, "handle is NULL");
  for (int c = 0; c < OMC_KERNEL_NCLASS; ++c) {
    if (launches) launches[c] = h->launches[c];
    if (ms) ms[c] = h->ms[c];
    if (units) units[c] = h->units[c];
  }
  return 0;
}
```

optimalmatrixcompletion.jl_amd/csrc/omc_device.h:

```cpp
#ifndef OMC_DEVICE_H
#define OMC_DEVICE_H
#include <hip/hip_runtime.h>
#include <stdint.h>

#define ROW_TRACE 0
#define ROW_BOX 1
#define ROW_BOUND 2
#define ROW_CUT 3

#define CONE_CLIP01 0
#define CONE_EVALS 2
#define CONE_SEP 3
#define CONE_TOPK 4
#define CONE_BIG 5
#define SMALL_PROJ 0
#define SMALL_RECOVER 1

#define OMC_ST_OPTIMAL 0
#define OMC_ST_SLOW 1
#define OMC_ST_TIME 2
#define OMC_ST_INFEASIBLE 3

#include "omc_layout.h"

struct OmcWS {
  int nB;
  int B, Btot, n, m, k, nnz, Rmax, Lmax, breakpoints, rmax, stall_checks, np16, max_sweeps, max_iters;
  int *node_of, *init, *fin;
  const int* slot_list;
  int check_every, early_stop_after; double early_stop_factor;
  double *gap_prev, *gap_rate; int* slow_votes;
  const double* rho_node;
  double *oY, *oU, *oalphaX, *obx, *oobj, *olb, *olmin, *orho; int *ostatus, *oiters;
  double gamma, rho, rho_f_ratio, relax, eps_gap, eps_feas, sumA2;
  double* rho_b;
  double* bfac;
  int *nbump, *lastbump;
  int bump_max, bump_after, bump_gap; double bump_ratio, bump_factor;
  const int* col_ptr;
  const int* col_idx;
  const double* col_val;
  const double* Ncnt;
  const int* row_ptr;
  const int* row_idx;
  double* lamD;
  double* lamDX;
  const double* wY1;
  double *Y, *Yp;
  double* U;
  double *D1, *D3;
  double *W1, *E3;
  int* w1_fac;
  int skip_yp;
  double* Qb;
  int* rr;
  double *Vt, *D3V, *W3V, *Q3V;
  double *D3T, *W3T, *Q3T;
  double* dS;
  double *alpha, *alphaX;
  double* sval;
  double *objcol, *c0col;
  double* Mchk;
  int check_xs;
  double *Mbuf, *Vrow;
  double* fro2;
  int* vvalid;
  double *MbufC, *VrowC, *fro2c; int* vvalidC; int ws_mode;
  int sub_enable, sub_qmax, sub_chunk, sub_debug; double sub_tol, sub_adapt;
  double* sub_zscratch;
  double* Xs;
  double* sub_theta;
  double* trM;
  double* V3; int* v3valid;
  int *sub_wait, *sub_nfail;
  int *sub_on, *cone_done;
  int* ws_first; int ws_phase;
  int* ws_need;
  int sub_guard;
  int* sep_done;
  int cert_enable; double *XsC, *sub_thetaC, *trMc, *lb_est; int *sub_onC, *confirm;
  int shor;
  int shN;
  const double *shP0, *shD0;
  double clip_hi;
  double inv_s2;
  const int *load_from, *save_to;
  double *pY, *pD1, *pD3, *pU, *palpha, *psval, *pXs, *ptheta, *pscal;
  int mw_budget; int* mw_stat; double* ev_out;
  int* pmw_stat;
  int* sub_stat;
  int* R;
  int *rkind, *rcut, *rbi, *rbj;
  double* rcoef;
  double* rrhs;
  double* cutx;
  double* G;
  int setup_gram_inline;
  double* lam;
  double *obj, *objout, *objprev, *lbprev, *lb, *c0, *evsum, *cpen, *cst, *rp, *rd, *lmin;
  double* bx;
  int *done, *status, *iters, *sweeps, *stall;
  int* rowov;
  OmcGeom geo;
  double* cp_scratch;
  int cp_pair; int cp_nsolo; const int* cp_solo;
  int cp_nwide; const int* cp_wide;
  int cp_nrest;
  int cp_nblock, cp_nslab; const int *cp_block, *cp_slab; const unsigned char* cp_isblock; double* cp_bslab; int* cp_nfact;
  double* Yx;
  int cone_512;
  int cp_series;
  int cp_maxpass;
  int cp_xcd;
  double *cone_scratch, *glob_scratch, *small_scratch;
  double* chk_scratch;
  double* stamps;
  int accel, aa_mem, aa_every, aa_start, aa_dim;
  double aa_reg, aa_safeguard;
  double *aa_F, *aa_G, *aa_zin;
  double* aa_fn;
  int *aa_hist, *aa_head, *aa_pending, *aa_valid, *aa_nacc, *aa_nrej;
  int *cert_flag, *cert_have;
  double *cb_rho, *cbLam, *cblam, *cbPsi, *cbBound;
  double *ocLam, *oclam, *ocPsi, *ocBound; int* ocHave;
};
#define AA_MAXMEM 10
struct OmcDualIn { const double *Lam, *lam, *Psi3; double* T1; const double* c0col; const int* colbad; };

#ifdef __cplusplus
extern "C" {
#endif
void omc_launch_setup(const OmcWS* w, hipStream_t s);
void omc_launch_setup_gram(const OmcWS* w, const int* jobs, int njobs, int nnodes, hipStream_t s);
void omc_launch_colprox(const OmcWS* w, int mode, hipStream_t s);
void omc_launch_cone(const OmcWS* w, int mode, hipStream_t s);
void omc_launch_global(const OmcWS* w, hipStream_t s);
void omc_launch_small(const OmcWS* w, int mode, hipStream_t s);
void omc_launch_cone_ws(const OmcWS* w, hipStream_t s);
void omc_launch_cone_mw(const OmcWS* w, hipStream_t s);
void omc_launch_cone_plain_mw(const OmcWS* w, int mode, hipStream_t s);
void omc_launch_cone_sub(const OmcWS* w, hipStream_t s);
void omc_launch_check_zero(const OmcWS* w, hipStream_t s);
void omc_launch_check_build(const OmcWS* w, hipStream_t s);
void omc_launch_check_final(const OmcWS* w, int last, int phase, hipStream_t s);
void omc_launch_cert_sub(const OmcWS* w, hipStream_t s);
void omc_launch_sep_sub(const OmcWS* w, hipStream_t s);
void omc_launch_rho_rescale(const OmcWS* w, hipStream_t s);
void omc_launch_harvest(const OmcWS* w, hipStream_t s);
void omc_launch_state_save(const OmcWS* w, hipStream_t s);
void omc_launch_dual_assemble(const OmcWS* w, const OmcDualIn* in, hipStream_t s);
void omc_launch_cert_snapshot(const OmcWS* w, hipStream_t s);
void omc_launch_cert_harvest(const OmcWS* w, hipStream_t s);
void omc_launch_aa(const OmcWS* w, hipStream_t s);
void omc_launch_make_X(const OmcWS* w, double* X, hipStream_t s);
void omc_launch_make_Theta(const OmcWS* w, const double* X, double* Th, hipStream_t s);
void omc_launch_eval_objective(int B, int n, int m, double gamma, const double* A, const uint8_t* mask, const double* X,
                               double* out, hipStream_t s);
int omc_set_max_lds(void);
void omc_query_residency(const OmcWS* w, int* out );
void omc_colprox_sweep_residency(int* pair, int* wide);
void omc_launch_gram_XXt(const OmcWS* w, const double* X, int B, hipStream_t s);
void omc_launch_colprox_sweep(const OmcWS* w, hipStream_t s);
void omc_launch_colprox_block(const OmcWS* w, int mode, hipStream_t s);
int omc_colprox_block_set_lds(void);
#ifdef __cplusplus
}
#endif
#endif
```

optimalmatrixcompletion.jl_amd/csrc/omc_device.hip:

```cpp
#include <hip/hip_runtime.h>
#include <type_traits>
#include <stdint.h>
#include "omc_device.h"
#include "omc.h"

#include "omc_wave.h"


#ifdef OMC_STAMPS
#define STAMP(slot) do { __syncthreads(); if (blockIdx.x == 0 && threadIdx.x == 0) { long long t_ = __builtin_amdgcn_s_memtime(); w.stamps[slot] += (double)(t_ - t_prev_); t_prev_ = t_; } } while (0)
#define STAMP_BEGIN() long long t_prev_ = __builtin_amdgcn_s_memtime()
#define DIAG_T0() long long t_diag0_ = __builtin_amdgcn_s_memtime()
#define DIAG_ADD(cls, b, v) atomicAdd(&w.stamps[32 + (size_t)(cls) * w.B + (b)], (double)(v))
#define DIAG_CYC(cls, b) DIAG_ADD(cls, b, __builtin_amdgcn_s_memtime() - t_diag0_)
#define WSTAMP_BEGIN() long long tw_prev_ = __builtin_amdgcn_s_memtime()
#define WSTAMP_BEGIN2() tw_prev_ = __builtin_amdgcn_s_memtime()
#define WSTAMP(slot) do { if (b == 0 && j == 0 && lane == 0) { long long t_ = __builtin_amdgcn_s_memtime(); w.stamps[slot] += (double)(t_ - tw_prev_); tw_prev_ = t_; } } while (0)
#else
#define WSTAMP_BEGIN() do {} while (0)
#define WSTAMP_BEGIN2() do {} while (0)
#define WSTAMP(slot) do {} while (0)
#define STAMP(slot) do {} while (0)
#define STAMP_BEGIN() do {} while (0)
#define DIAG_T0() do {} while (0)
#define DIAG_ADD(cls, b, v) do {} while (0)
#define DIAG_CYC(cls, b) do {} while (0)
#endif

__device__ __forceinline__ double rowU_entry(const OmcWS& w, int nb, int r, int i, int j) {
  const int kind = w.rkind[(size_t)nb * w.Rmax + r];
  if (kind == ROW_TRACE) return 0.0;
  if (kind == ROW_BOX) {
    return (w.rbi[(size_t)nb * w.Rmax + r] == i && w.rbj[(size_t)nb * w.Rmax + r] == j)
               ? w.rcoef[((size_t)nb * w.Rmax + r) * w.k]
               : 0.0;
  }
  const int l = w.rcut[(size_t)nb * w.Rmax + r];
  return w.cutx[((size_t)nb * w.Lmax + l) * w.n + i] * w.rcoef[((size_t)nb * w.Rmax + r) * w.k + j];
}

__device__ __forceinline__ void gram_pair(const OmcWS& w, int nb, int r, int s, double* G, double* red) {
  const int n = w.n, k = w.k, tid = threadIdx.x, T = blockDim.x;
  const int kr = w.rkind[(size_t)nb * w.Rmax + r], ks = w.rkind[(size_t)nb * w.Rmax + s];
  double acc = 0.0;
  const bool yr = (kr == ROW_TRACE || kr == ROW_CUT), ys = (ks == ROW_TRACE || ks == ROW_CUT);
  if (yr && ys) {
    const double* xr = (kr == ROW_CUT) ? w.cutx + ((size_t)nb * w.Lmax + w.rcut[(size_t)nb * w.Rmax + r]) * n : nullptr;
    const double* xs = (ks == ROW_CUT) ? w.cutx + ((size_t)nb * w.Lmax + w.rcut[(size_t)nb * w.Rmax + s]) * n : nullptr;
    if (!xr && !xs) {
      for (int i = tid; i < n; i += T) acc += 1.0 / w.wY1[(size_t)i * n + i];
    } else if (!xr || !xs) {
      const double* x = xr ? xr : xs;
      for (int i = tid; i < n; i += T) acc += x[i] * x[i] / w.wY1[(size_t)i * n + i];
    } else {
      for (int e = tid; e < n * n; e += T) {
        int i = e % n, j = e / n;
        acc += xr[i] * xr[j] * xs[i] * xs[j] / w.wY1[e];
      }
    }
  }
  if (kr != ROW_TRACE && ks != ROW_TRACE) {
    for (int e = tid; e < n * k; e += T) {
      int i = e % n, j = e / n;
      double a = rowU_entry(w, nb, r, i, j);
      if (a != 0.0) acc += a * rowU_entry(w, nb, s, i, j) * 0.5;
    }
  }
  double tot = block_sum(acc, red);
  if (tid == 0) { G[(size_t)r * w.Rmax + s] = tot; G[(size_t)s * w.Rmax + r] = tot; }
}

__global__ void k_setup(OmcWS w) {
  if (!w.init[blockIdx.x]) return;
  const int nb = w.node_of[blockIdx.x];
  const int b = blockIdx.x, n = w.n, k = w.k, tid = threadIdx.x, T = blockDim.x, rm = w.rmax;
  __shared__ double red[32];
  double* Y = w.Y + (size_t)b * n * n;
  double* Yp = w.Yp + (size_t)b * n * n;
  const double d0 = (double)k / (double)n;
  const int lf = w.load_from ? w.load_from[nb] : -1;
  const bool warm = lf >= 0;
  const int NP = w.np16;
  const int rc = w.rr[nb];
  const double* Qc = w.Qb + (size_t)nb * n * rm;
  if (warm) {
    const double fw = w.pscal[(size_t)lf * 4] / w.rho_node[nb];
    double fr2 = 0.0, tr1 = 0.0;
    for (int e = tid; e < n * n; e += T) {
      const int i = e % n, j = e / n;
      const double y = w.pY[(size_t)lf * n * n + e], d1 = w.pD1[(size_t)lf * n * n + e] * fw;
      Y[e] = y; Yp[e] = y; if (w.Yx) w.Yx[(size_t)b * n * n + e] = y;
      w.D1[(size_t)b * n * n + e] = d1; w.D3[(size_t)b * n * n + e] = w.pD3[(size_t)lf * n * n + e] * fw; w.E3[(size_t)b * n * n + e] = 0.0;
      const double mv = y - d1;
      w.Mbuf[(size_t)b * NP * NP + (size_t)j * NP + i] = mv; fr2 += mv * mv; if (i == j) tr1 += mv;
    }
    for (int e = tid; e < NP * NP; e += T) {
      const int i = e % NP, j = e / NP;
      if (i >= n || j >= n) w.Mbuf[(size_t)b * NP * NP + e] = 0.0;
      w.Vrow[(size_t)b * NP * NP + e] = 0.0;
    }
    for (int e = tid; e < NP * 16; e += T) w.Xs[(size_t)b * NP * 16 + e] = w.pXs[(size_t)lf * NP * 16 + e];
    if (tid < 16) w.sub_theta[(size_t)b * 16 + tid] = w.ptheta[(size_t)lf * 16 + tid];
    fr2 = block_sum(fr2, red); tr1 = block_sum(tr1, red);
    if (tid == 0) {
      w.fro2[b] = fr2; w.trM[b] = tr1; w.sub_on[b] = (w.sub_enable && w.pscal[(size_t)lf * 4 + 1] != 0.0) ? 1 : 0; w.sub_wait[b] = 0; w.sub_nfail[b] = 0; w.cone_done[b] = 0; if (w.w1_fac) w.w1_fac[b] = 0; w.v3valid[b] = 0; w.sub_onC[b] = 0; w.confirm[b] = 1; w.lb_est[b] = -1e300; w.vvalid[b] = 0; if (w.vvalidC) w.vvalidC[b] = 0; if (w.ws_first) { w.ws_first[b] = w.sub_on[b] ? 0 : 1; if (w.ws_need && !w.sub_on[b]) *w.ws_need = 1; }
    }
    for (int e = tid; e < rm * k; e += T) {
      const int a = e % rm, j = e / rm;
      double v = 0.0;
      if (a < rc) for (int i = 0; i < n; ++i) v += Qc[(size_t)a * n + i] * w.pU[(size_t)lf * n * k + (size_t)j * n + i];
      w.Vt[(size_t)b * rm * k + e] = v; w.D3V[(size_t)b * rm * k + e] = 0.0;
      w.W3V[(size_t)b * rm * k + e] = 0.0; w.Q3V[(size_t)b * rm * k + e] = 0.0;
    }
    __syncthreads();
    __threadfence_block();
    for (int e = tid; e < n * k; e += T) {
      const int i = e % n, j = e / n;
      double v = 0.0;
      for (int a = 0; a < rc; ++a) v += Qc[(size_t)a * n + i] * w.Vt[(size_t)b * rm * k + (size_t)j * rm + a];
      w.U[(size_t)b * n * k + e] = v;
    }
    for (int e = tid; e < w.nnz; e += T) w.alpha[(size_t)b * w.nnz + e] = w.palpha[(size_t)lf * w.nnz + e];
    for (int e = tid; e < w.m; e += T) w.sval[(size_t)b * w.m + e] = w.psval[(size_t)lf * w.m + e];
  } else {
  for (int e = tid; e < n * n; e += T) {
    int i = e % n, j = e / n;
    double v = (i == j) ? d0 : 0.0;
    Y[e] = v; Yp[e] = v; if (w.Yx) w.Yx[(size_t)b * n * n + e] = v;
    w.D1[(size_t)b * n * n + e] = 0.0; w.D3[(size_t)b * n * n + e] = 0.0; w.E3[(size_t)b * n * n + e] = 0.0;
  }
  {
    for (int e = tid; e < NP * NP; e += T) {
      int i = e % NP, j = e / NP;
      w.Mbuf[(size_t)b * NP * NP + e] = (i == j && i < n) ? d0 : 0.0;
      w.Vrow[(size_t)b * NP * NP + e] = 0.0;
    }
    if (tid == 0) {
      w.fro2[b] = d0 * d0 * n; w.trM[b] = d0 * n; w.sub_on[b] = 0; w.sub_wait[b] = 0; w.sub_nfail[b] = 0; w.cone_done[b] = 0; if (w.w1_fac) w.w1_fac[b] = 0; w.v3valid[b] = 0; w.sub_onC[b] = 0; w.confirm[b] = 1; w.lb_est[b] = -1e300; w.vvalid[b] = 0; if (w.vvalidC) w.vvalidC[b] = 0; if (w.ws_first) { w.ws_first[b] = w.sub_on[b] ? 0 : 1; if (w.ws_need && !w.sub_on[b]) *w.ws_need = 1; }
    }
  }
  for (int e = tid; e < n * k; e += T) w.U[(size_t)b * n * k + e] = 0.0;
  for (int e = tid; e < rm * k; e += T) {
    w.Vt[(size_t)b * rm * k + e] = 0.0; w.D3V[(size_t)b * rm * k + e] = 0.0;
    w.W3V[(size_t)b * rm * k + e] = 0.0; w.Q3V[(size_t)b * rm * k + e] = 0.0;
  }
  for (int e = tid; e < w.nnz; e += T) w.alpha[(size_t)b * w.nnz + e] = 0.0;
  for (int e = tid; e < w.m; e += T) w.sval[(size_t)b * w.m + e] = -1.0;
  }
  for (int e = tid; e < k * k; e += T) {
    w.D3T[(size_t)b * k * k + e] = 0.0; w.Q3T[(size_t)b * k * k + e] = 0.0;
    w.W3T[(size_t)b * k * k + e] = ((e % k) == (e / k)) ? 1.0 : 0.0;
  }
  const int R = w.R[nb];
  for (int e = tid; e < w.Rmax; e += T) w.lam[(size_t)b * w.Rmax + e] = 0.0;
  if (tid == 0) {
    w.init[b] = 0; w.rho_b[b] = w.rho_node[nb];
    if (w.accel) { w.aa_valid[b] = 0; w.aa_hist[b] = 0; w.aa_head[b] = 0; w.aa_pending[b] = 0; w.aa_nacc[b] = 0; w.aa_nrej[b] = 0; }
    w.done[b] = 0; w.rowov[b] = 0; w.gap_prev[b] = 1e300; w.gap_rate[b] = 1.0; w.slow_votes[b] = 0; w.status[b] = OMC_ST_SLOW; w.iters[b] = 0; w.stall[b] = 0; w.nbump[b] = 0; w.lastbump[b] = 0; w.bfac[b] = 1.0;
    w.obj[b] = 1e300; w.objout[b] = 1e300; w.objprev[b] = 1e300; w.lbprev[b] = -1e300; w.lb[b] = -1e300; w.rp[b] = 1e300; w.rd[b] = 1e300;
  }
  if (w.setup_gram_inline) {
    double* G = w.G + (size_t)b * w.Rmax * w.Rmax;
    for (int r = 0; r < R; ++r)
      for (int s = r; s < R; ++s) gram_pair(w, nb, r, s, G, red);
  }
}

__global__ void __launch_bounds__(256) k_setup_gram(OmcWS w, const int* jobs, int njobs, int nnodes) {
  const int q = blockIdx.y;
  if (q >= njobs) return;
  const int b = jobs[2 * q], nb = jobs[2 * q + 1];
  if (b < 0 || b >= w.B || nb < 0 || nb >= nnodes) return;
  const int R = w.R[nb];
  const int npairs = gram_npairs(R);
  int p = blockIdx.x * GRAM_CHUNK;
  if (p >= npairs) return;
  const int pend = (p + GRAM_CHUNK < npairs) ? p + GRAM_CHUNK : npairs;
  __shared__ double red[32];
  double* G = w.G + (size_t)b * w.Rmax * w.Rmax;
  int r, s;
  gram_pair_of(p, R, &r, &s);
  for (; p < pend; ++p) {
    gram_pair(w, nb, r, s, G, red);
    gram_pair_next(R, &r, &s);
  }
}

template <class PT>
__device__ __forceinline__ void colprox_body(const OmcWS& w, int mode, int b, int j, int off, int c, int lane, PT base) {
  const int n = w.n;
  const CpBodyLayout L = cp_body_layout(c);
  auto Bm = base;
  auto Lm = Bm + L.Lm, va = Bm + L.va, vy = Bm + L.vy, vz = Bm + L.vz, vo = Bm + L.vo;
  const int* idx = w.col_idx + off;
  const double g = w.gamma;
  const double* Y = w.Y + (size_t)b * n * n;
  const double* Yp = w.Yp + (size_t)b * n * n;
  double* alpha = ((mode == 0) ? w.alpha : w.alphaX) + (size_t)b * w.nnz + off;
  for (int p = lane; p < c; p += WAVE) {
    va[p] = w.col_val[off + p];
    vo[p] = (mode == 0) ? alpha[p] : 0.0;
  }
  WAVE_SYNC();
  const double rho_f = w.rho_b[b] * w.rho_f_ratio;
  const double coef = (mode == 0) ? g / (2.0 * rho_f) : 0.0;
  for (int e = lane; e < c * c; e += WAVE) {
    int p = e / c, q = e - p * c;
    if (q > p) continue;
    size_t a = (size_t)idx[q] * n + idx[p];
    double yv = (mode == 0) ? (w.Yx ? w.Yx[(size_t)b * n * n + a] : (2.0 * Y[a] - Yp[a])) : Y[a];
    double v = g * (yv - coef * vo[p] * vo[q]);
    if (p == q) v += 1.0;
    Bm[TRI(p, q)] = v;
  }
  WAVE_SYNC();
  double s = 0.0;
  const bool regpath = (c <= WAVE);
  auto dinv = vz;
  const double a_reg = (lane < c) ? va[lane] : 0.0;
  auto solve2 = [&](double& y_out, double& z_out, bool want_z) {
    if (regpath) {
      for (int p = lane; p < c; p += WAVE) dinv[p] = 1.0 / Lm[TRI(p, p)];
      WAVE_SYNC();
      y_out = wave_chol_solve_reg(Lm, dinv, c, a_reg, lane);
      z_out = want_z ? wave_chol_solve_reg(Lm, dinv, c, y_out, lane) : 0.0;
    } else {
      wave_chol_solve(Lm, c, va, vy, lane);
      if (want_z) wave_chol_solve(Lm, c, vy, vz, lane);
    }
  };
  if (mode == 0) {
    const double cp = g * g / (2.0 * rho_f);
    double sprev = w.sval[(size_t)b * w.m + j];
    s = (sprev > 0.0) ? sprev : 0.0;
    double lo = 0.0, hi = -1.0;
    bool lo_valid = false;
    double yr = 0.0, zr = 0.0;
    bool have_final = false;
    int nfact_ = 0; (void)nfact_;
    for (int it = 0; it < 60; ++it) {
      ++nfact_;
      for (int e = lane; e < c * c; e += WAVE) {
        int p = e / c, q = e - p * c;
        if (q <= p) Lm[TRI(p, q)] = Bm[TRI(p, q)] + ((p == q) ? cp * s : 0.0);
      }
      WAVE_SYNC();
      bool ok = wave_cholesky(Lm, c, lane);
      if (!ok) {
        lo = s; lo_valid = false;
        s = (hi > 0.0) ? 0.5 * (s + hi) : (2.0 * s + 1.0);
        continue;
      }
      solve2(yr, zr, true);
      double yy = 0.0, yz = 0.0;
      if (regpath) { yy = yr * yr; yz = yr * zr; }
      else for (int p = lane; p < c; p += WAVE) { yy += vy[p] * vy[p]; yz += vy[p] * vz[p]; }
      yy = wave_sum(yy); yz = wave_sum(yz);
      const double ph = yy - s, dph = -2.0 * cp * yz - 1.0;
      if (ph >= 0.0) { lo = s; lo_valid = true; } else { hi = s; }
      double sn = s - ph / dph;
      if (!(sn > lo) && !lo_valid) sn = 0.5 * (lo + s);
      if (sn < lo) sn = lo;
      if (hi > 0.0 && sn > hi) sn = 0.5 * (lo + hi);
      if (fabs(sn - s) <= 1e-13 * fmax(1.0, fabs(s))) { have_final = true; break; }
      s = sn;
    }
    if (!have_final) {
      ++nfact_;
      for (int e = lane; e < c * c; e += WAVE) {
        int p = e / c, q = e - p * c;
        if (q <= p) Lm[TRI(p, q)] = Bm[TRI(p, q)] + ((p == q) ? cp * s : 0.0);
      }
      WAVE_SYNC();
      wave_cholesky(Lm, c, lane);
      solve2(yr, zr, false);
    }
    if (lane == 0) w.sval[(size_t)b * w.m + j] = s;
    if (lane == 0 && w.cp_nfact) w.cp_nfact[(size_t)b * w.m + j] = nfact_;
    if (lane == 0) DIAG_ADD(1, b, nfact_);
    double* lamD = w.lamD + ((size_t)b * w.m + j) * n;
    if (regpath) { if (lane < c) { alpha[lane] = yr; lamD[idx[lane]] = yr; } }
    else for (int p = lane; p < c; p += WAVE) { alpha[p] = vy[p]; lamD[idx[p]] = vy[p]; }
  } else {
    for (int e = lane; e < c * c; e += WAVE) {
      int p = e / c, q = e - p * c;
      if (q <= p) Lm[TRI(p, q)] = Bm[TRI(p, q)];
    }
    WAVE_SYNC();
    bool ok = wave_cholesky(Lm, c, lane);
    if (!ok) {
      for (int p = lane; p < c; p += WAVE) { alpha[p] = 0.0; if (w.lamDX) w.lamDX[((size_t)b * w.m + j) * n + idx[p]] = 0.0; }
// ... 1558 lines not shown
    while (c * n - ((c * (c - 1)) >> 1) > q) --c;
    while ((c + 1) * n - ((c * (c + 1)) >> 1) <= q) ++c;
    j = c; i = c + q - (c * n - ((c * (c - 1)) >> 1));
  };
  struct In2 { double y, nc, d1, d3, e3; };
  auto load2 = [&](int e) { In2 v; v.y = Y[e]; v.nc = w.Ncnt[e]; v.d1 = D1[e]; v.d3 = D3[e]; v.e3 = E3[e]; return v; };
  auto target2 = [&](int e, int i, int j, double w1, const In2& v) {
    const double y = v.y;
    const double first = w.shor ? rho * (rx * w.shP0[(size_t)b * w.shN * w.shN + (size_t)j * w.shN + i] + (1.0 - rx) * y + w.shD0[(size_t)b * w.shN * w.shN + (size_t)j * w.shN + i])
                                : rho_f * v.nc * y;
    tY[TRIX(i, j)] = first + rho * (rx * w1 + (1.0 - rx) * y + v.d1) + rho * (y + (1.0 - rx) * v.d3 + rx * v.e3);
  };
  for (int q0 = tid; q0 < ntri; q0 += 4 * T) {
    int ii[4], jj[4], ee[4]; bool ok[4]; double w1[4]; In2 v[4];
#pragma unroll
    for (int u = 0; u < 4; ++u) {
      const int q = q0 + u * T;
      ok[u] = q < ntri;
      tri_ij(ok[u] ? q : q0, ii[u], jj[u]);
      ee[u] = jj[u] * n + ii[u];
    }
#pragma unroll
    for (int u = 0; u < 4; ++u) w1[u] = ok[u] ? w1_at(ee[u], ii[u], jj[u]) : 0.0;
#pragma unroll
    for (int u = 0; u < 4; ++u) v[u] = load2(ee[u]);
#pragma unroll
    for (int u = 0; u < 4; ++u) if (ok[u]) target2(ee[u], ii[u], jj[u], w1[u], v[u]);
  }
  for (int e = tid; e < r * k; e += T) {
    int a = e % r, j = e / r;
    tV[(size_t)j * rm + a] = rx * W3V[(size_t)j * rm + a] + (1.0 - rx) * Vt[(size_t)j * rm + a] + D3V[(size_t)j * rm + a];
  }
  for (int e = tid; e < R; e += T) mu[e] = lam[e] / rho;
  __syncthreads();
  STAMP(14);
  if (!w.shor) {
    mfma_LLt<2>(lamD, n, m, [&](int i, int j, double v) {
      const int t = TRIX(i, j);
      double x = tY[t];
      x += 0.5 * g * v;
      tY[t] = x / (rho * w.wY1[(size_t)j * n + i]);
    });
    STAMP(15);
  } else {
    for (int q = tid; q < ntri; q += T) {
      int i, j; tri_ij(q, i, j);
      tY[TRIX(i, j)] /= (rho * w.wY1[(size_t)j * n + i]);
    }
    STAMP(28);
  }
  for (int e = tid; e < n * k; e += T) {
    int i = e % n, j = e / n;
    double acc = 0.0;
    for (int a = 0; a < r; ++a) acc += Q[(size_t)a * n + i] * tV[(size_t)j * rm + a];
    tU[e] = acc;
  }
  __syncthreads();
  STAMP(9);
  const double* cutx = w.cutx + (size_t)nb * w.Lmax * n;
  double *xs = tY + L.xs, *qrow = tY + L.qrow;
  __shared__ int s_crow[GL_XS]; __shared__ int s_nc, s_rnext; __shared__ double s_qp[8][GL_XS];
  if (tid == 0) s_rnext = 0;
  for (;;) {
    __syncthreads();
    if (tid < WAVE) {
      int c = 0, rr0 = s_rnext, rn = R;
      const unsigned long long below = (1ull << tid) - 1ull;
      for (; rr0 < R && c < GL_XS; rr0 += WAVE) {
        const int rr = rr0 + tid;
        const bool cut = rr < R && w.rkind[(size_t)nb * w.Rmax + rr] == ROW_CUT;
        const unsigned long long mk = __ballot(cut);
        const int pos = c + __popcll(mk & below);
        if (cut && pos < GL_XS) s_crow[pos] = rr;
        const unsigned long long last = __ballot(cut && pos == GL_XS - 1);
        if (last) rn = rr0 + __builtin_ctzll(last) + 1;
        c += __popcll(mk);
      }
      if (tid == 0) { s_nc = (c < GL_XS) ? c : GL_XS; s_rnext = rn; }
    }
    __syncthreads();
    const int nc = s_nc, rnext = s_rnext;
    if (nc == 0) break;
    for (int e = tid; e < nc * n; e += T) { const int c = e / n, i = e - c * n; xs[e] = cutx[(size_t)w.rcut[(size_t)nb * w.Rmax + s_crow[c]] * n + i]; }
    __syncthreads();
    {
      const int wv_ = tid >> 6, lane_ = tid & 63, nw_ = T >> 6, li = lane_ & 15, lk = lane_ >> 4;
      const bool vc = li < nc;
      const double* xc = xs + (size_t)(vc ? li : 0) * n;
      double qsum = 0.0;
      for (int ti = wv_; ti < nt16; ti += nw_) {
        const int ia = (ti << 4) + li; const bool va = ia < n; const int ic = va ? ia : 0;
        double4v acc = {0.0, 0.0, 0.0, 0.0};
        for (int k0 = 0; k0 < n; k0 += 4) {
          const int kk = k0 + lk; const bool vk = kk < n; const int kc = vk ? kk : 0;
          const double a = tY[TRIX(ic, kc)], bv = xc[kc];
          acc = __builtin_amdgcn_mfma_f64_16x16x4f64((va && vk) ? a : 0.0, (vc && vk) ? bv : 0.0, acc, 0, 0, 0);
        }
#pragma unroll
        for (int r4 = 0; r4 < 4; ++r4) {
          const int i = (ti << 4) + lk + 4 * r4;
          const double xv = xc[(i < n) ? i : 0];
          qsum += (vc && i < n) ? xv * acc[r4] : 0.0;
        }
      }
      qsum += __shfl_xor(qsum, 16, WAVE);
      qsum += __shfl_xor(qsum, 32, WAVE);
      if (lk == 0) s_qp[wv_][li] = qsum;
    }
    __syncthreads();
    if (tid < nc) {
      double q = 0.0;
      for (int v = 0; v < (T >> 6); ++v) q += s_qp[v][tid];
      qrow[s_crow[tid]] = q;
    }
    if (rnext >= R) break;
  }
  __syncthreads();
  {
    const int wv_ = tid >> 6, lane_ = tid & 63, nw_ = T >> 6;
    int mk = 0, mc = 0; double mf = 0.0, mr = 0.0;
    int it = 0;
    for (int rr = wv_; rr < R; rr += nw_, ++it) {
      if ((it & 63) == 0) {
        const int r2 = rr + nw_ * lane_;
        if (r2 < R) { const size_t d = (size_t)nb * w.Rmax + r2; mk = w.rkind[d]; mc = w.rcut[d]; mf = w.rcoef[d * k]; mr = w.rrhs[d]; }
      }
      const int kind = __shfl(mk, it & 63, WAVE);
      double acc = 0.0;
      if (kind == ROW_TRACE) {
        for (int i = lane_; i < n; i += WAVE) acc += tY[TRIX(i, i)];
      } else if (kind == ROW_BOX) {
        if (lane_ == 0) acc = w.rcoef[((size_t)nb * w.Rmax + rr) * k] * tU[(size_t)w.rbj[(size_t)nb * w.Rmax + rr] * n + w.rbi[(size_t)nb * w.Rmax + rr]];
      } else {
        const double* x = cutx + (size_t)__shfl(mc, it & 63, WAVE) * n;
        const double* cf = w.rcoef + ((size_t)nb * w.Rmax + rr) * k;
        const double c0 = __shfl(mf, it & 63, WAVE);
        if (kind == ROW_CUT && lane_ == 0) acc = qrow[rr];
        for (int j = 0; j < k; ++j) {
          const double cj = (j == 0) ? c0 : cf[j];
          if (cj != 0.0) for (int i = lane_; i < n; i += WAVE) acc += cj * x[i] * tU[(size_t)j * n + i];
        }
      }
      const double tot = wave_sum(acc);
      const double rhs = __shfl(mr, it & 63, WAVE);
      if (lane_ == 0) cvec[rr] = tot - rhs;
    }
  }
  const double* G = w.G + (size_t)b * w.Rmax * w.Rmax;
  const bool gstage = (size_t)w.Rmax * w.Rmax <= (size_t)GL_XS * n;
  if (gstage) {
    for (int e = tid; e < R * w.Rmax; e += T) xs[e] = G[e];
    G = xs;
  }
  __syncthreads();
  STAMP(10);
  if (tid < WAVE) { const int ov = wave_nnqp(G, w.Rmax, cvec, mu, R, s_Gp, s_sv, s_tmp, s_pl, tid); if (tid == 0) w.rowov[b] = ov; }
  __syncthreads();
  for (int e = tid; e < R; e += T) lam[e] = rho * mu[e];
  __shared__ int s_nact; __shared__ int s_act[NNQP_PMAX]; __shared__ double s_mu[NNQP_PMAX]; __shared__ double s_trace_mu;
  int& s_nnz = s_nc;
  if (tid < WAVE) {
    int c0 = 0, c2 = 0; double tm = 0.0;
    const unsigned long long below = (1ull << tid) - 1ull;
    for (int r0 = 0; r0 < R; r0 += WAVE) {
      const int rr = r0 + tid;
      const double mv = (rr < R) ? mu[rr] : 0.0;
      const int kind = (mv != 0.0) ? w.rkind[(size_t)nb * w.Rmax + rr] : -1;
      const unsigned long long nz = __ballot(mv != 0.0), cut = __ballot(kind == ROW_CUT);
      unsigned long long trc = __ballot(kind == ROW_TRACE);
      const int p0 = c0 + __popcll(nz & below), p2 = c2 + __popcll(cut & below);
      if (mv != 0.0 && p0 < NNQP_PMAX) s_pl[p0] = rr;
      if (kind == ROW_CUT && p2 < NNQP_PMAX) { s_act[p2] = w.rcut[(size_t)nb * w.Rmax + rr]; s_mu[p2] = mv; }
      for (; trc; trc &= trc - 1) tm += mu[r0 + __builtin_ctzll(trc)];
      c0 += __popcll(nz); c2 += __popcll(cut);
    }
    if (tid == 0) { s_nnz = (c0 < NNQP_PMAX) ? c0 : NNQP_PMAX; s_nact = (c2 < NNQP_PMAX) ? c2 : NNQP_PMAX; s_trace_mu = tm; }
  }
  __syncthreads();
  STAMP(11);
  const int nnz = s_nnz;
  for (int e = tid; e < n * k; e += T) {
    int i = e % n, j = e / n;
    double corr = 0.0;
    for (int c = 0; c < nnz; ++c) { const int rr = s_pl[c]; corr += mu[rr] * rowU_entry(w, nb, rr, i, j); }
    tU[e] = 0.5 * corr;
  }
  const int nact = s_nact, nstg = (nact < GL_XS) ? nact : GL_XS;
  for (int e = tid; e < nstg * n; e += T) { const int a = e / n, i = e - a * n; xs[e] = cutx[(size_t)s_act[a] * n + i]; }
  if (f1) stage_w1();
  __syncthreads();
  double rp2 = 0.0, rd2 = 0.0, fr2 = 0.0, tr1 = 0.0;
  double* Mb = w.Mbuf + (size_t)b * NP * NP;
  for (int e = tid; e < r * k; e += T) {
    int a = e % r, j = e / r;
    double qc = 0.0;
    for (int i = 0; i < n; ++i) qc += Q[(size_t)a * n + i] * tU[(size_t)j * n + i];
    const size_t ix = (size_t)j * rm + a;
    double vn = tV[ix] - qc, vold = Vt[ix], w3 = W3V[ix];
    D3V[ix] += rx * w3 + (1.0 - rx) * vold - vn;
    rp2 += 2.0 * (w3 - vn) * (w3 - vn); rd2 += 2.0 * (vn - vold) * (vn - vold);
    tV[ix] = vn;
  }
  for (int e = tid; e < k * k; e += T) {
    double zi = ((e % k) == (e / k)) ? 1.0 : 0.0;
    double w3t = w.W3T[(size_t)b * k * k + e];
    w.D3T[(size_t)b * k * k + e] += rx * (w3t - zi);
    rp2 += (w3t - zi) * (w3t - zi);
  }
  __syncthreads();
  for (int e = tid; e < r * k; e += T) { int a = e % r, j = e / r; Vt[(size_t)j * rm + a] = tV[(size_t)j * rm + a]; }
  for (int e = tid; e < n * k; e += T) {
    int i = e % n, j = e / n;
    double acc = 0.0;
    for (int a = 0; a < r; ++a) acc += Q[(size_t)a * n + i] * tV[(size_t)j * rm + a];
    U[e] = acc;
  }
  STAMP(12);
  auto corr_at = [&](int i, int j) {
    double corr = (i == j) ? s_trace_mu : 0.0;
    for (int a = 0; a < nstg; ++a) { const double* x = xs + (size_t)a * n; corr += s_mu[a] * (x[i] * x[j]); }
    for (int a = nstg; a < nact; ++a) { const double* x = cutx + (size_t)s_act[a] * n; corr += s_mu[a] * (x[i] * x[j]); }
    return corr;
  };
  struct In6 { double t, wy, yold, e3, d3, d1; };
  auto load6 = [&](size_t a1, int i, int j) { In6 v; v.t = tY[TRIX(i, j)]; v.wy = w.wY1[a1]; v.yold = Y[a1]; v.e3 = E3[a1]; v.d3 = D3[a1]; v.d1 = D1[a1]; return v; };
  auto update6 = [&](size_t a1, int i, int j, double w1, double corr, const In6& v) {
    const double yn = v.t - corr / v.wy;
    const double yold = v.yold;
    const double e3 = v.e3, d3 = v.d3;
    const double d1n = v.d1 + rx * w1 + (1.0 - rx) * yold - yn;
    const double w3y = yold - d3 + e3;
    const double d3n = (1.0 - rx) * d3 + yold + rx * e3 - yn;
    D1[a1] = d1n; D3[a1] = d3n;
    const double mv = yn - d1n;
    Mb[(size_t)j * NP + i] = mv;
    fr2 += mv * mv;
    if (i == j) tr1 += mv;
    rp2 += (w1 - yn) * (w1 - yn) + (w3y - yn) * (w3y - yn);
    rd2 += (yn - yold) * (yn - yold);
    if (!w.skip_yp) Yp[a1] = yold;
    Y[a1] = yn;
    if (w.Yx) w.Yx[(size_t)b * n * n + a1] = 2.0 * yn - yold;
  };
  const int di6 = (2 * T) % n, dj6 = (2 * T) / n;
  int i6 = tid % n, j6 = tid / n, ib6 = (tid + T) % n, jb6 = (tid + T) / n;
  for (int e = tid; e < n * n; e += 2 * T) {
    const int eb = e + T; const bool two = eb < n * n;
    const int i = i6, j = j6, ib = two ? ib6 : i, jb = two ? jb6 : j;
    i6 += di6; j6 += dj6; if (i6 >= n) { i6 -= n; ++j6; }
    ib6 += di6; jb6 += dj6; if (ib6 >= n) { ib6 -= n; ++jb6; }
    const size_t a1 = (size_t)j * n + i, a1b = (size_t)jb * n + ib;
    const double w1 = w1_at(a1, i, j), w1b = two ? w1_at(a1b, ib, jb) : 0.0;
    const double corr = corr_at(i, j), corrb = two ? corr_at(ib, jb) : 0.0;
    const In6 v = load6(a1, i, j), vb = load6(a1b, ib, jb);
    update6(a1, i, j, w1, corr, v);
    if (two) update6(a1b, ib, jb, w1b, corrb, vb);
  }
  STAMP(13);
  rp2 = block_sum(rp2, red);
  rd2 = block_sum(rd2, red);
  fr2 = block_sum(fr2, red);
  tr1 = block_sum(tr1, red);
  if (tid == 0) { w.rp[b] = sqrt(rp2); w.rd[b] = sqrt(rd2); w.fro2[b] = fr2; w.trM[b] = tr1; w.cone_done[b] = 0; if (w.w1_fac) w.w1_fac[b] = 0; w.iters[b] += 1; if (w.ws_first) { const int f = (!w.sub_on[b] || w.sub_wait[b] > 0) ? 1 : 0; w.ws_first[b] = f; if (f && w.ws_need) *w.ws_need = 1; } DIAG_CYC(4, b); }
}

#define CB_LIST 256
__global__ void __launch_bounds__(512) k_check_build(OmcWS w) {
  __shared__ double red[32];
  __shared__ int s_arow[CB_LIST], s_ccut[CB_LIST], s_na, s_nc;
  __shared__ double s_alam[CB_LIST], s_clam[CB_LIST], s_xs[CB_XS];
  const int b = blockIdx.x, tid = threadIdx.x, T = blockDim.x;
  if (w.done[b]) return;
  const int nb = w.node_of[b];
  const int n = w.n, k = w.k, m = w.m, R = w.R[nb], rm = w.rmax, r = w.rr[nb];
  double* M = w.Mchk + (size_t)b * n * n;
  const double* E3 = w.E3 + (size_t)b * n * n;
  const double* lam = w.lam + (size_t)b * w.Rmax;
  const double* cutx = w.cutx + (size_t)nb * w.Lmax * n;
  const double* Q = w.Qb + (size_t)nb * n * rm;
  const double rho = w.rho_b[b], g = w.gamma;
  double* cU = w.chk_scratch + (size_t)b * n * k;
  const bool listed = R <= CB_LIST;
  if (listed && tid < WAVE) {
    int na = 0, nc = 0;
    const unsigned long long below = (1ull << tid) - 1ull;
    for (int r0 = 0; r0 < R; r0 += WAVE) {
      const int rr = r0 + tid;
      const double lv = rr < R ? lam[rr] : 0.0;
      const bool act = lv != 0.0;
      const bool cut = act && w.rkind[(size_t)nb * w.Rmax + rr] == ROW_CUT;
      const unsigned long long ma = __ballot(act), mc = __ballot(cut);
      if (act) { const int pos = na + __popcll(ma & below); s_arow[pos] = rr; s_alam[pos] = lv; }
      if (cut) { const int pos = nc + __popcll(mc & below); s_ccut[pos] = w.rcut[(size_t)nb * w.Rmax + rr]; s_clam[pos] = lv; }
      na += __popcll(ma); nc += __popcll(mc);
    }
    if (tid == 0) { s_na = na; s_nc = nc; }
  }
  {
    double so = 0.0, sc = 0.0;
    for (int j = tid; j < m; j += T) { so += w.objcol[(size_t)b * m + j]; sc += w.c0col[(size_t)b * m + j]; }
    so = block_sum(so, red); sc = block_sum(sc, red);
    if (tid == 0) { w.obj[b] = so; w.c0[b] = sc; }
  }
  if (listed) {
    const int na = s_na, nc = s_nc;
    const int cap = (w.check_xs * n <= CB_XS) ? w.check_xs : CB_XS / n;
    const int ncs = nc < cap ? nc : cap;
    for (int e = tid; e < ncs * n; e += T) { const int c = e / n, i = e - c * n; s_xs[e] = cutx[(size_t)s_ccut[c] * n + i]; }
    __syncthreads();
// ... 710 lines not shown
```

optimalmatrixcompletion.jl_amd/csrc/omc_host.h:

```cpp
#pragma once
#include <hip/hip_runtime.h>
#include <stdint.h>
#include <atomic>
#include <mutex>
#include <string>
#include <thread>
#include <unordered_map>
#include <vector>

#include "omc.h"
#include "omc_carve.h"
#include "omc_device.h"
#include "omc_shor_relax.h"
#include "omc_shor_index.h"
#include "omc_walks.h"

extern thread_local std::string g_err;
static inline int fail(int code, const std::string& msg) { g_err = msg; return code; }
#define HIPCHK(x)                                                                                         \
  do {                                                                                                    \
    hipError_t e_ = (x);                                                                                  \
    if (e_ != hipSuccess) {                                                                               \
      g_err = std::string(#x) + ": " + hipGetErrorString(e_);                                             \
      return (int)e_ > 0 ? (int)e_ : 999;                                                                 \
    }                                                                                                     \
  } while (0)

struct DevBuf {
  void* p = nullptr; size_t cap = 0;
  DevBuf() = default;
  DevBuf(const DevBuf&) = delete;
  DevBuf& operator=(const DevBuf&) = delete;
  ~DevBuf() { release(); }
  int ensure(size_t bytes) {
    if (bytes <= cap) return 0;
    if (p) (void)hipFree(p);
    p = nullptr; cap = 0;
    size_t want = bytes + bytes / 4 + 256;
    hipError_t e = hipMalloc(&p, want);
    if (e != hipSuccess) { g_err = std::string("hipMalloc: ") + hipGetErrorString(e); return (int)e; }
    cap = want;
    return 0;
  }
  void release() { if (p) (void)hipFree(p); p = nullptr; cap = 0; }
  template <class T> T* as() { return (T*)p; }
};
#define ENS(buf, bytes) do { int r_ = (buf).ensure(bytes); if (r_) return r_; } while (0)

template <class F> static inline int carve_ensure(DevBuf& b, F&& walk, size_t* bytes = nullptr) {
  Carve measure;
  walk(measure);
  if (bytes) *bytes = measure.bytes();
  const int rc = b.ensure(measure.bytes());
  if (rc) return rc;
  Carve place(b.p);
  walk(place);
  return 0;
}
#define ENS_CARVE(buf, ...) do { int r_ = carve_ensure(buf, __VA_ARGS__); if (r_) return r_; } while (0)

template <class T> static inline int bind(DevBuf& b, T*& field, size_t count) {
  field = nullptr;
  const int rc = b.ensure(count * sizeof(T));
  if (rc) return rc;
  field = (T*)b.p;
  return 0;
}
template <class T> static inline int bind(DevBuf& b, T*& field, size_t count, hipStream_t zero_on) {
  const int rc = bind(b, field, count);
  if (rc) return rc;
  HIPCHK(hipMemsetAsync(b.p, 0, count * sizeof(T), zero_on));
  return 0;
}
#define BIND(...) do { int r_ = bind(__VA_ARGS__); if (r_) return r_; } while (0)

struct PinBuf {
  void* p = nullptr; size_t cap = 0;
  PinBuf() = default;
  PinBuf(const PinBuf&) = delete;
  PinBuf& operator=(const PinBuf&) = delete;
  ~PinBuf() { if (p) (void)hipHostFree(p); }
  int ensure(size_t bytes) {
    if (bytes <= cap) return 0;
    if (p) (void)hipHostFree(p);
    p = nullptr; cap = 0;
    hipError_t e = hipHostMalloc(&p, bytes, hipHostMallocDefault);
    if (e != hipSuccess) { g_err = std::string("hipHostMalloc: ") + hipGetErrorString(e); return (int)e; }
    cap = bytes;
    return 0;
  }
  template <class T> T* as() { return (T*)p; }
};

struct Tuning {
  bool altmin_nolds = false;
  bool colprox_no_xcd = false;
  bool cone_512 = false;
  bool dense_proj = false;
  bool host_phases = false;
  bool global_nolds = false;
  bool no_colprox_pair = false;
  bool no_graph = false;
  bool no_subspace = false;
  bool no_ws_split = false;
  bool segv_trace = false;
  bool setup_gram_inline = false;
  bool shor_explicit = false;
  bool shor_no_subspace = false;
  int check_xs = 16;
  int colprox_block_min = 65;
  int cone_multi_min = 1025;
  int event_merge = 1;
  int graph_max = 16;
  int harvest_async = 1;
  int harvest_async_min_live = 256;
  int plain_multi_min = 1025;
  int shor_index_device_min = 0;
  int shor_select_kb = 1048576;
  int streams = 4;
  int sub_debug = 0;
  int sub_qmax = 24;
  int timing_stride = 1;
  int ws_quiet = 1;
};
struct Knob { const char* name; bool Tuning::*flag; int Tuning::*num; };
inline const Knob OMC_KNOBS[] = {
  {"OMC_ALTMIN_NOLDS", &Tuning::altmin_nolds, nullptr},      {"OMC_COLPROX_NO_XCD", &Tuning::colprox_no_xcd, nullptr},
  {"OMC_CONE_512", &Tuning::cone_512, nullptr},              {"OMC_DENSE_PROJ", &Tuning::dense_proj, nullptr},
  {"OMC_GLOBAL_NOLDS", &Tuning::global_nolds, nullptr},      {"OMC_HOST_PHASES", &Tuning::host_phases, nullptr},
  {"OMC_NO_COLPROX_PAIR", &Tuning::no_colprox_pair, nullptr},
  {"OMC_NO_GRAPH", &Tuning::no_graph, nullptr},              {"OMC_NO_SUBSPACE", &Tuning::no_subspace, nullptr},
  {"OMC_NO_WS_SPLIT", &Tuning::no_ws_split, nullptr},        {"OMC_SEGV_TRACE", &Tuning::segv_trace, nullptr},
  {"OMC_SETUP_GRAM_INLINE", &Tuning::setup_gram_inline, nullptr},
  {"OMC_SHOR_EXPLICIT", &Tuning::shor_explicit, nullptr},    {"OMC_SHOR_NO_SUBSPACE", &Tuning::shor_no_subspace, nullptr},
  {"OMC_COLPROX_BLOCK_MIN", nullptr, &Tuning::colprox_block_min},
  {"OMC_CHECK_XS", nullptr, &Tuning::check_xs},              {"OMC_CONE_MULTI_MIN", nullptr, &Tuning::cone_multi_min},
  {"OMC_EVENT_MERGE", nullptr, &Tuning::event_merge},
  {"OMC_GRAPH_MAX", nullptr, &Tuning::graph_max},            {"OMC_SHOR_SELECT_KB", nullptr, &Tuning::shor_select_kb},
  {"OMC_SHOR_INDEX_DEVICE_MIN", nullptr, &Tuning::shor_index_device_min},
  {"OMC_HARVEST_ASYNC", nullptr, &Tuning::harvest_async},    {"OMC_HARVEST_ASYNC_MIN_LIVE", nullptr, &Tuning::harvest_async_min_live},
  {"OMC_WS_QUIET", nullptr, &Tuning::ws_quiet},
  {"OMC_STREAMS", nullptr, &Tuning::streams},                {"OMC_PLAIN_MULTI_MIN", nullptr, &Tuning::plain_multi_min},
  {"OMC_SUB_DEBUG", nullptr, &Tuning::sub_debug},            {"OMC_SUB_QMAX", nullptr, &Tuning::sub_qmax},
  {"OMC_TIMING_STRIDE", nullptr, &Tuning::timing_stride},
};

struct omc_instance {
  int n = 0, m = 0, k = 0, device = 0, nnz = 0, cmax = 0;
  double gamma = 0, sumA2 = 0;
  std::vector<int> col_ptr, col_idx; std::vector<double> col_val;
  std::vector<double> A; std::vector<uint8_t> mask;
  std::vector<double> Ncnt;
  std::vector<int> row_ptr, row_idx; std::vector<double> row_val;
  DevBuf drow_ptr, drow_idx, drow_val, aR, arkind, arcut, arbi, arbj, arcoef, arrhs, acutx, aU0, aU, aV, aobj, aint, aG, aG2;
  hipStream_t stream = nullptr;
  Tuning tun;
  hipStream_t gs[3] = {};
  hipEvent_t gev[5] = {};
  hipEvent_t gevc[5] = {};
  hipEvent_t ev_main = nullptr;
  PinBuf pin_flags[2], pin_list[2], pin_done, pin_jobs; DevBuf bgramjobs;
  hipEvent_t ev_up[4] = {}; bool ev_up_rec[4] = {}; hipEvent_t ev_gram = nullptr; bool ev_gram_rec = false;
  double host_ms[OMC_HOST_NPHASE] = {0}; int64_t host_cnt[OMC_HOST_NPHASE] = {0};
  DevBuf dA, dmask, dcol_ptr, dcol_idx, dcol_val, dNcnt, dwY, dsolo, dwide;
  int nwide = 0;
  int nsolo = 0;
  DevBuf dblock, dslab, disblock, bcpb, bnfact;
  int nblock = 0, nslab = 0, nrest = 0, cpb_cl = 0, cpb_cs = 0, crest_max = 0;
  bool lists_valid = false; int lists_block_min = 0; bool lists_pair = true;
  DevBuf bYx, bY, bYp, bU, bD1, bD3, bW1, bE3, bQb, brr, bsm, bdS, balpha, balphaX, bsval, bMchk, bsmall, bchk;
  DevBuf bR, brkind, brcut, brbi, brbj, brcoef, brrhs, bcutx, bG, blam;
  DevBuf bobjcol, baaF, baaG, baaZ, baaS, baaI, bMbufC, bVrowC, bchkS, bchkI;
  DevBuf bslotlist, bgap, bvotes, blamDX, bXsC, bsubSC, bsubIC;
  DevBuf bsubz, bscal, bbx, bint, bcp, bcone, bglob, bXout, bThout, bXin, bMbuf, bVrow, bXs, bsubS, bsubI;
  long long sub_tot[8] = {0};
  DevBuf bmwstat, sbigmw, pjM, pjV, pjW, pjS, pjD, pjI;
  long long mw_tot[5] = {0};
  DevBuf bpmwstat; long long pmw_tot[4] = {0};
  OmcWS ws{};
  omc_relax_params params{};
  bool staged = false;
  double last_solve_seconds = 0; long long total_sweeps = 0; int last_iters_total = 0;
  std::thread worker; std::atomic<int> worker_running{0}, nodes_done{0}; int worker_rc = 0; std::string worker_err;
  int reserve_nodes = 0, reserve_cuts = 0, node_cap = 0, staged_cut_type = 0; std::atomic<int> Btot_live{0}; bool append_closed = true; std::mutex append_mu; hipStream_t append_stream = nullptr;
  std::atomic<int> hold{0};
  std::vector<int> done_q; size_t done_read = 0; std::mutex done_mu; hipStream_t fetch_stream = nullptr;
  void* comm = nullptr; int comm_rank = 0, comm_world = 1; DevBuf bcomm, amobj; int amobj_B = 0;
  int wall_khz = 0;
  std::vector<double> rho_scale_per_node; DevBuf brho, brhon, blamD, bslotint, boY, boU, boal, bobx, boscal, boint;
  int Btot = 0;
  bool keep_cert = false; DevBuf bcbD, bcbI, bocD, bocI;
  bool keep_shor_cert = false; DevBuf scbD, socD, socNq;
  DevBuf dbD, dbI, dbM, dbS, dbL;
  DevBuf sdD, sdI, sdGi, sdGb, sdGr; double sdb_ms = 0.0;
  DevBuf sbits, scb, scx, scz, soff, stot, sout, shi, slo, sexist, shist, sohi, solo, scnt;
  bool shor_ready = false; int shor_W = 0; long long shor_pairs = 0;
  double shor_last_ms = 0; long long shor_last_candidates = 0;
  int64_t shor_sel[4] = {0, 0, 0, 0};
  bool shor_on = false, shor_keep_V = false, shor_via_base = false; std::vector<int> shor_slackrow; DevBuf soV; double shor_rho = 0.05, shor_r4 = 0.0, shor_r5 = 2.0;
  ShWS sh{}; OmcWS wbig{};
  DevBuf sgInts, sgBytes, sgGroups, sgNodeGroup, sAh, sX, sW, sTh, sV1, sV2, sV3, sD0, sP0, sMbufB, sVrowB, sTq, sPq, sNq, sD5x, sD5t, snu5, sP5x,
      scolpart, sminpart, sminpart2, sfroB, svvB, se1, se2, soX, soW, soTh, sbigscr, sXsB, ssubSB, ssubIB;
  long long big_sub_tot[8] = {0};
  struct ShorListKey { int64_t nq = 0, nsoc = 0; uint64_t hlist = 0; std::vector<int64_t> idx, soc; };
  int64_t reserve_shor_nq = 0; int reserve_shor_lists = 0; bool reserve_shor_set = false;
  std::unordered_map<uint64_t, std::vector<int>> sh_byhash; std::vector<ShorListKey> sh_lists;
  int sh_group_cap = 0; size_t sh_int_used = 0, sh_int_cap = 0, sh_byte_used = 0, sh_byte_cap = 0;
  DevBuf sxD; ShorIndexDims sx_dims{}; ShorIndexWS sx{}; int* sx_stage_int = nullptr; uint8_t* sx_stage_byte = nullptr;
  int sh_index_min = 0; double shidx_stats[5] = {0, 0, 0, 0, 0};
  int pool_cap = 0; DevBuf pY, pD1, pD3, pU, palpha, psval, pXs, ptheta, pscal, bwarmL, bwarmS; std::vector<int> warm_load, warm_save;
  struct PoolSig { int kind = 0; int64_t nq = 0, nsoc = 0; uint64_t hlist = 0, hsoc = 0; };
  bool pool_shor = false; int64_t pool_nqmax = 0; DevBuf pShor, pShorHdr, sloadpart;
  std::vector<PoolSig> pool_sig, node_sig; std::mutex sig_mu;
  std::vector<int> save_host;
  int64_t shor_warm_stats[4] = {0, 0, 0, 0};
  int64_t launches[OMC_KERNEL_NCLASS] = {0}; double ms[OMC_KERNEL_NCLASS] = {0}; int64_t units[OMC_KERNEL_NCLASS] = {0};
  size_t nnz_rows() const { return row_idx.size(); }
  std::vector<hipEvent_t> ev_pool[2];
};

static constexpr int MAX_SWEEPS = 30;
```

optimalmatrixcompletion.jl_amd/csrc/omc_layout.h:

```cpp
#ifndef OMC_LAYOUT_H
#define OMC_LAYOUT_H
#include <hip/hip_runtime.h>
#include <stddef.h>

#define NNQP_PMAX 64
#define NNQP_GP_DOUBLES (NNQP_PMAX * (NNQP_PMAX + 1) / 2)
#define NNQP_STATIC_BYTES ((NNQP_GP_DOUBLES + 2 * NNQP_PMAX) * 8 + NNQP_PMAX * 4)
#define OMC_MAX_DYN_LDS (144 * 1024)
#define SUBP 16
#define GL_XS 16
#define OMC_HD __host__ __device__ inline
struct ConeLayout { int Np, ld; size_t ev, wgt, sel; };
OMC_HD ConeLayout cone_carve(int N, int ld) { const int Np = (N + 1) & ~1; const size_t ev = (size_t)Np * ld; return {Np, ld, ev, ev + Np, ev + 2 * Np}; }
OMC_HD ConeLayout cone_layout(int N) { return cone_carve(N, ((N + 1) & ~1) | 1); }
OMC_HD size_t cone_bytes(int N) { const ConeLayout L = cone_layout(N); return L.sel * 8 + (size_t)L.Np * 4 + 16; }
OMC_HD size_t ws_bytes(int N, int ld) { const ConeLayout L = cone_carve(N, ld); return (L.sel + L.Np) * 8 + (size_t)(L.Np + 2) * 4 + 64; }
OMC_HD int ws_rpl(int N, int lpp) { return (((N + lpp - 1) / lpp) + 1) & ~1; }
struct WsGeometry { int lpp, rpl, ld, use_lds; size_t bytes; };
OMC_HD WsGeometry ws_geometry(int N) {
  const int Np2 = (N + 1) & ~1;
  int lpp = 16; while (lpp > 4 && lpp * (Np2 / 2) > 512) lpp >>= 1;
  int rpl = ws_rpl(N, lpp), Nrp = rpl * lpp;
  int ld = Nrp + ((16 - (Nrp & 31)) & 31);
  if (ws_bytes(N, ld) > OMC_MAX_DYN_LDS) ld = Nrp + 2;
  const int use_lds = ws_bytes(N, ld) <= OMC_MAX_DYN_LDS;
  if (!use_lds) {
    lpp = 16; rpl = ws_rpl(N, 16);
    if (rpl > 32 && N <= 1024) { lpp = 64; rpl = ws_rpl(N, 64); }
    ld = rpl * lpp + 2;
  }
  return {rpl <= 32 ? lpp : 0, rpl, ld, use_lds, ws_bytes(N, ld)};
}
#define GRAM_CHUNK 8
#define CB_XS 4096
OMC_HD int gram_npairs(int R) { return R * (R + 1) / 2; }
OMC_HD int gram_chunks(int R) { return (gram_npairs(R) + GRAM_CHUNK - 1) / GRAM_CHUNK; }
OMC_HD void gram_pair_of(int p, int R, int* r, int* s) {
  int rr = 0;
  while (p >= R - rr) { p -= R - rr; ++rr; }
  *r = rr; *s = rr + p;
}
OMC_HD void gram_pair_next(int R, int* r, int* s) { if (++*s == R) { ++*r; *s = *r; } }
#define MW_B 16
#define MW_MAXSW 32
#define MW_MIN_ORDER 145
#define MW_MAX_ORDER 4096
#define MW_TAU_PLAIN 1e-14
#define MW_PLAIN_SWEEPS 30
struct MwLayout { int ld, Ncp, nb; size_t ev, lam, wgt, sel, smax, head, bytes, fro; };
OMC_HD MwLayout mw_layout(int N) {
  const int NP = (N + 15) & ~15, Ncp = (N + 2 * MW_B - 1) & ~(2 * MW_B - 1), ld = NP + 4;
  static_assert(2 * MW_B >= 16, "fro: the NP / 16 partial sums of the plain sequence lie in the Ncp words of wgt, NP <= Ncp");
  const size_t ev = (size_t)Ncp * ld, sel = ev + 3 * (size_t)Ncp, smax = sel + Ncp / 2, head = smax + MW_MAXSW;
  return {ld, Ncp, Ncp / MW_B, ev, ev + Ncp, ev + 2 * (size_t)Ncp, sel, smax, head, (head + 4) * 8, ev + 2 * (size_t)Ncp};
}
OMC_HD int mw_plain_launches(const MwLayout& L, int sweeps) { return sweeps * (L.nb - 1) + 4; }
struct SubLayout { int LD, zglob; size_t Za, Cs, Hs, Gj, th, evj, red, wgt, sel, bytes; };
OMC_HD SubLayout sub_layout(int np16) {
  const int LD = np16 + 2, zglob = np16 > 512; const size_t blk = (size_t)SUBP * LD, Cs = (zglob ? 1 : 2) * blk, th = Cs + 4 * 256 + 2 * 16 * 17;
  return {LD, zglob, blk, Cs, Cs + 4 * 256, Cs + 4 * 256 + 16 * 17, th, th + 16, th + 32, th + 64, th + 80, (th + 80 + 8) * 8};
}
#define SMALL_STATIC_LDS 1024
struct SmallLayout { int ld3; size_t M3, Gm, ev, wgt, sel, Cc, Qs, bytes; };
OMC_HD SmallLayout small_layout(int n, int rmax, int k) {
  const int ld3 = rmax + k, Npm = (ld3 + 1) & ~1, ldm = Npm | 1;
  const size_t M3 = (size_t)n * rmax, Gm = M3 + (size_t)ld3 * ld3, ev = Gm + (size_t)Npm * ldm, sel = ev + 2 * Npm, Cc = sel + Npm / 2, Qs = Cc + (size_t)rmax * k + 2;
  return {ld3, M3, Gm, ev, ev + Npm, sel, Cc, Qs, (Qs + (size_t)n * 16) * 8 + 104};
}
#define GLOB_STATIC_LDS ((size_t)NNQP_STATIC_BYTES + 2560)
struct GlobLayout { size_t tU, tV, cvec, mu, xs, qrow, bytes; };
OMC_HD GlobLayout glob_layout(int n, int k, int rmax, int Rmax) {
  const size_t tU = (size_t)n * (n + 1) / 2, tV = tU + (size_t)n * k, cvec = tV + (size_t)rmax * k, xs = cvec + 2 * Rmax, qrow = xs + (size_t)GL_XS * n;
  return {tU, tV, cvec, cvec + Rmax, xs, qrow, (qrow + Rmax) * 8 + 80};
}
OMC_HD bool glob_w1_fits(int n) { return (size_t)SUBP * n <= (size_t)NNQP_GP_DOUBLES; }
struct CpRegLayout { int Lm, vo, pinv, sidx, doubles; };
OMC_HD CpRegLayout cp_reg_layout(int c, int keepB) { const int tri = (c * (c + 1)) >> 1, vo = (keepB ? 2 : 1) * tri; return {keepB ? tri : 0, vo, vo + c, vo + 2 * c, vo + 4 * c + 8}; }
struct CpBodyLayout { size_t Lm, va, vy, vz, vo, doubles; };
OMC_HD CpBodyLayout cp_body_layout(int c) { const size_t tri = (size_t)c * (c + 1) / 2, va = 2 * tri; return {tri, va, va + c, va + 2 * c, va + 3 * c, va + 4 * c + 8}; }
#define CPB_TILE 256
#define CPB_STATIC_LDS 4352
struct CpBlockLayout { int nb, ntiles; size_t panel, va, vy, vz, vw, vo, sidx, doubles, slab; };
OMC_HD int cpb_tile(int I, int J) { return ((I * (I + 1)) >> 1) + J; }
OMC_HD CpBlockLayout cp_block_layout(int c, int lds) {
  const int nb = c > 0 ? (c + 15) >> 4 : 1, nt = (nb * (nb + 1)) >> 1;
  const size_t cp = (size_t)16 * nb, va = (size_t)CPB_TILE * (lds ? nt : (nb > 1 ? nb - 1 : 1));
  return {nb, nt, 0, va, va + cp, va + 2 * cp, va + 3 * cp, va + 4 * cp, va + 5 * cp, va + 5 * cp + cp / 2, lds ? 0 : (size_t)CPB_TILE * nt};
}
OMC_HD int cp_block_fits(int c, int lds) { return cp_block_layout(c, lds).doubles * 8 <= (size_t)OMC_MAX_DYN_LDS; }
OMC_HD int cp_block_lds_cmax() { int nb = 1; while (cp_block_fits(16 * (nb + 1), 1)) ++nb; return 16 * nb; }
OMC_HD int cp_block_cmax() { int nb = 1; while (cp_block_fits(16 * (nb + 1), 0)) ++nb; return 16 * nb; }
OMC_HD void cp_block_plan(int cmax, int block_min, long long* out) {
  const int ldsc = cp_block_lds_cmax(), on = cmax >= block_min && cmax >= 1 && cmax <= cp_block_cmax();
  const CpBlockLayout L = cp_block_layout(cmax, cmax <= ldsc);
  out[0] = ldsc; out[1] = on ? (long long)(L.doubles * 8) : 0; out[2] = on ? (long long)L.slab : 0;
  out[3] = on ? (long long)((160 * 1024) / (L.doubles * 8 + CPB_STATIC_LDS)) : 0; out[4] = on;
}
struct Altmin1Layout { size_t v, h, g, u0, cvec, mu, bytes; };
OMC_HD Altmin1Layout altmin1_layout(int n, int m, int Rmax) { const size_t h = (size_t)n + m, cvec = h + 3 * n; return {(size_t)n, h, h + n, h + 2 * n, cvec, cvec + Rmax, (cvec + 2 * Rmax + 8) * 8}; }
struct AltminKLayout { size_t ut, u0, g, H, Hinv, v, cvec, mu, bytes; };
OMC_HD AltminKLayout altmink_layout(int n, int m, int k, int Rmax) {
  const size_t nk = (size_t)n * k, H = 4 * nk, v = H + 2 * nk * k, cvec = v + (size_t)k * m;
  return {nk, 2 * nk, 3 * nk, H, H + nk * k, v, cvec, cvec + Rmax, (cvec + 2 * Rmax + 8) * 8};
}
struct AltminWLayout { size_t ut, u0, g, H, Hinv, v, cvec, mu, th, th2, q, qt, step, tmp, act, J, P, Lc, bytes; };
OMC_HD AltminWLayout altminw_layout(int n, int m, int k, int Rmax) {
  const size_t nk = (size_t)n * k, mq = (size_t)k * k, H = 4 * nk, v = H + 2 * nk * k, cvec = v + (size_t)k * m, th = cvec + 2 * Rmax, J = th + 7 * mq, Lc = J + 2 * mq * mq;
  return {nk, 2 * nk, 3 * nk, H, H + nk * k, v, cvec, cvec + Rmax, th, th + mq, th + 2 * mq, th + 3 * mq, th + 4 * mq, th + 5 * mq, th + 6 * mq, J, J + mq * mq, Lc,
          (Lc + mq * (mq + 1) / 2 + 8) * 8};
}
struct KernelPlan { int use_lds; size_t lds_bytes, slab_stride; };
OMC_HD KernelPlan plan_block(size_t bytes, bool fits) { return {fits ? 1 : 0, fits ? bytes : 0, fits ? 0 : bytes / 8 + 8}; }
#define ALTMIN_KMAX 8
OMC_HD int altmin_variant(int k) { return k == 1 ? 1 : (k <= 4 ? 2 : 3); }
OMC_HD KernelPlan altmin_plan(int n, int m, int k, int Rmax, int nolds) {
  const int var = altmin_variant(k);
  const size_t bytes = (var == 1) ? altmin1_layout(n, m, Rmax).bytes : (var == 2) ? altmink_layout(n, m, k, Rmax).bytes : altminw_layout(n, m, k, Rmax).bytes;
  return plan_block(bytes, bytes + 8 * 1024 <= ((var == 1) ? (size_t)OMC_MAX_DYN_LDS - 8 * 1024 : (size_t)128 * 1024) && !nolds);
}
struct OmcGeom {
  KernelPlan cone, ws, glob, small;
  int ws_lpp, ws_rpl2, ws_ld;
  size_t cpb_lds_bytes, cpb_slab_lds_bytes, cpb_slab_stride;
  int cp_lds_c, cp_lds_doubles, cp_keepB;
  size_t cp_scratch_stride, sub_lds;
  int mw; MwLayout mwl;
  int plain_mw;
};
OMC_HD void geom_set_mw(OmcGeom& g, int n) {
  g.mw = 1; g.mwl = mw_layout(n);
  size_t st = g.mwl.bytes / 8 + 8; if (st < g.ws.slab_stride) st = g.ws.slab_stride;
  g.cone.slab_stride = g.ws.slab_stride = (st + 3) & ~(size_t)3;
}
OMC_HD void geom_set_plain_mw(OmcGeom& g, int n) {
  const int mw = g.mw;
  geom_set_mw(g, n);
  g.mw = mw; g.plain_mw = 1;
}
OMC_HD void geom_set_cpblock(OmcGeom& g, int cl, int cs) {
  g.cpb_lds_bytes = cl > 0 ? cp_block_layout(cl, 1).doubles * 8 : 0;
  g.cpb_slab_lds_bytes = cs > 0 ? cp_block_layout(cs, 0).doubles * 8 : 0;
  g.cpb_slab_stride = cs > 0 ? cp_block_layout(cs, 0).slab : 0;
}
OMC_HD bool mw_order_ok(int n, int use_lds, int knob) { return n >= MW_MIN_ORDER && !use_lds && n >= knob && n <= MW_MAX_ORDER; }
OMC_HD OmcGeom omc_plan_geometry(int n, int np16, int k, int rmax, int Rmax, int cmax, int global_nolds, int cone_multi_min, int plain_multi_min) {
  OmcGeom g;
  const WsGeometry wg = ws_geometry(n);
  g.cone = plan_block(cone_bytes(n), cone_bytes(n) <= OMC_MAX_DYN_LDS);
  g.ws = plan_block(wg.bytes, wg.use_lds != 0);
  g.ws_lpp = wg.lpp; g.ws_rpl2 = wg.rpl >> 1; g.ws_ld = wg.ld;
  g.cone.slab_stride = g.ws.slab_stride = g.cone.slab_stride > g.ws.slab_stride ? g.cone.slab_stride : g.ws.slab_stride;
  g.sub_lds = sub_layout(np16).bytes;
  const size_t gb = glob_layout(n, k, rmax, Rmax).bytes, sb = small_layout(n, rmax, k).bytes;
  g.glob = plan_block(gb, gb + GLOB_STATIC_LDS <= OMC_MAX_DYN_LDS && !global_nolds);
  g.small = plan_block(sb, sb + SMALL_STATIC_LDS <= OMC_MAX_DYN_LDS);
  g.cp_lds_c = cmax < 64 ? cmax : 64; g.cp_keepB = g.cp_lds_c <= 40 ? 1 : 0;
  g.cp_lds_doubles = cp_reg_layout(g.cp_lds_c, g.cp_keepB).doubles;
  g.cp_scratch_stride = cmax > g.cp_lds_c ? cp_body_layout(cmax).doubles : 0;
  g.mw = g.plain_mw = 0; g.mwl = MwLayout{};
  g.cpb_lds_bytes = g.cpb_slab_lds_bytes = g.cpb_slab_stride = 0;
// ... 6 lines not shown
```

optimalmatrixcompletion.jl_amd/csrc/omc_relax_solve.cpp:

```cpp
#include <algorithm>
#include <chrono>
#include <stdio.h>

#include "omc_events.h"
#include "omc_host.h"
#include "omc_slots.h"

static_assert(SLOT_HARVEST_NONE == OMC_HARVEST_NONE && SLOT_HARVEST_SYNC == OMC_HARVEST_SYNC && SLOT_HARVEST_ASYNC == OMC_HARVEST_ASYNC, "omc_slots.h restates the plans of omc.h");

namespace {

using Clock = std::chrono::steady_clock;

int sum_sub_stat(int* sub_stat, int S, long long tot[8], hipStream_t s) {
  std::vector<int> ss(8 * (size_t)S);
  HIPCHK(hipMemcpyAsync(ss.data(), sub_stat, sizeof(int) * ss.size(), hipMemcpyDeviceToHost, s));
  HIPCHK(hipStreamSynchronize(s));
  for (int q = 0; q < 8; ++q) tot[q] = 0;
  for (int b = 0; b < S; ++b) for (int q = 0; q < 8; ++q) tot[q] += ss[8 * b + q];
  HIPCHK(hipMemsetAsync(sub_stat, 0, sizeof(int) * ss.size(), s));
  return 0;
}

enum { T_S = 0, T_M = 1, T_B = 2, T_C = 3, T_NSTREAM = 4 };
// ... 352 lines not shown
      }
      if (shor && sw.cbGam) omc_shor_launch_cert_snapshot(&sw, s);
      if (w.cert_flag) omc_launch_cert_snapshot(&w, s);
      if (w.bump_max > 0) { if (shor) omc_shor_launch_rescale(&sw, s); omc_launch_rho_rescale(&w, s); }
      if (w.accel) omc_launch_aa(&w, s);
    });
  }

  int mw_collect() {
    if (!mw_any) return 0;
    std::vector<int> st(4 * (size_t)S);
    for (int v = 0; v < 2; ++v) {
      const OmcWS& wv = v ? h->wbig : w;
      if (!(v ? shor && wv.geo.mw : wv.geo.mw)) continue;
      HIPCHK(hipMemcpyAsync(st.data(), wv.mw_stat, sizeof(int) * st.size(), hipMemcpyDeviceToHost, s));
      HIPCHK(hipStreamSynchronize(s));
      HIPCHK(hipMemsetAsync(wv.mw_stat, 0, sizeof(int) * st.size(), s));
      int mx = 0;
      for (int b = 0; b < S; ++b) { h->mw_tot[0] += st[4 * b]; h->mw_tot[2] += st[4 * b + 2]; mx = std::max(mx, st[4 * b + 3]); }
      if (mx) h->mw_tot[1] = mx;
      h->mw_tot[3] = std::max<long long>(h->mw_tot[3], mx);
      mw_budget[v] = omc_cone_multi_budget(mx);
    }
    return 0;
  }

  int read_check() {
    stamp_begin();
    const bool track_quiet = split_solve && tun.ws_quiet && w.ws_need;
    done[S] = 1;
    HIPCHK(hipMemcpyAsync(done, w.done, sizeof(int) * ((size_t)S + (track_quiet ? 1 : 0)), hipMemcpyDeviceToHost, s));
    if (track_quiet) HIPCHK(hipMemsetAsync(w.ws_need, 0, sizeof(int), s));
    HIPCHK(hipStreamSynchronize(s));
    stamp(OMC_HOST_CHECK_WAIT);
    quiet_next = track_quiet && done[S] == 0;
    t_check = t_last;
    nrefilled = 0; list_pushed = false;
    { int rc = mw_collect(); if (rc) return rc; }
    if (drain_pool >= 0) { finish_events(drain_pool); drain_pool = -1; }
    drain_pool = tape.current(); tape.swap();
    Btot = h->Btot_live.load();
    if (!P.first_wins) return 0;
    std::vector<int> stv(S);
    HIPCHK(hipMemcpyAsync(stv.data(), w.status, sizeof(int) * S, hipMemcpyDeviceToHost, s));
    HIPCHK(hipStreamSynchronize(s));
    bool won = false;
    for (int b = 0; b < S; ++b) if (book.node(b) >= 0 && done[b] && stv[b] == OMC_ST_OPTIMAL) won = true;
    if (!won) return 0;
    book.finish_all();
    HIPCHK(hipMemcpyAsync(w.done, done, sizeof(int) * S, hipMemcpyHostToDevice, s));
    HIPCHK(hipStreamSynchronize(s));
    return close_unslotted(OMC_ST_SLOW);
  }

  void enqueue_harvest(int nslots) {
    tape.touch(T_S);
    TIMED(OMC_KERNEL_HARVEST, nslots, {
      if (w.save_to) omc_launch_state_save(&w, s);
      if (shor) omc_shor_launch_state_save(&sw, s);
      omc_launch_small(&w, SMALL_RECOVER, s);
      if (w.sep_done) omc_launch_sep_sub(&w, s);
      omc_launch_cone(&w, CONE_SEP, s);
      omc_launch_harvest(&w, s);
      if (w.cert_flag) omc_launch_cert_harvest(&w, s);
      if (shor && sw.cbGam) omc_shor_launch_cert_harvest(&sw, s);
      if (shor) omc_shor_launch_harvest(&sw, s);
    });
  }
  void book_harvested() {
    if (w.save_to) {
      std::lock_guard<std::mutex> lk(h->sig_mu);
      for (int id : harvested_ids) {
        const int sv = (size_t)id < h->save_host.size() ? h->save_host[id] : -1;
        if (sv < 0 || (size_t)sv >= h->pool_sig.size()) continue;
        if (shor) { h->pool_sig[sv] = h->node_sig[id]; ++h->shor_warm_stats[3]; }
        else { h->pool_sig[sv] = omc_instance::PoolSig{}; h->pool_sig[sv].kind = 1; }
      }
    }
    std::lock_guard<std::mutex> lk(h->done_mu); h->done_q.insert(h->done_q.end(), harvested_ids.begin(), harvested_ids.end());
  }

  int book_async_harvest() {
    harvested += book.pending_harvests(); h->nodes_done.store(harvested);
    int rc = gram_jobs_free(); if (rc) return rc;
    nrefilled = book.book_async(Btot, timed_out, harvested_ids);
    book_harvested();
    stamp(OMC_HOST_HARVEST_BOOK);
    rc = gram_launch(nrefilled); if (rc) return rc;
    rc = push_flags(false); if (rc) return rc;
    if (nrefilled) { rc = setup_slots(nrefilled); if (rc) return rc; }
    stamp(OMC_HOST_SETUP_ENQUEUE);
    return 0;
  }

  int harvest_async() {
    const int npend = book.mark_async();
    int rc = push_list(); if (rc) return rc;
    list_pushed = true;
    stamp(OMC_HOST_LIST);
    if (multi) { HIPCHK(hipEventRecord(h->ev_main, s)); ev_main_set = true; tape.touch(T_S); }
    rc = push_flags(false); if (rc) return rc;
    stamp(OMC_HOST_HARVEST_FLAGS);
    enqueue_harvest(npend);
    stamp(OMC_HOST_HARVEST_ENQUEUE);
    h->host_cnt[OMC_HOST_ASYNC_HARVESTS] += 1;
    return 0;
  }

  int harvest_sync(int nfin) {
    int rc = gram_jobs_free(); if (rc) return rc;
    rc = gram_launch(book.mark_sync(Btot, timed_out)); if (rc) return rc;
    rc = push_flags(false); if (rc) return rc;
    stamp(OMC_HOST_HARVEST_FLAGS);
    enqueue_harvest(nfin);
    stamp(OMC_HOST_HARVEST_ENQUEUE);
    harvested += nfin; h->nodes_done.store(harvested);
    const int ninit = book.harvest_sync(Btot, timed_out, harvested_ids);
    rc = push_flags(true); if (rc) return rc;
    stamp(OMC_HOST_HARVEST_WAIT);
    book_harvested();
    stamp(OMC_HOST_HARVEST_BOOK);
    if (ninit) { rc = setup_slots(ninit); if (rc) return rc; }
    stamp(OMC_HOST_SETUP_ENQUEUE);
    return 0;
  }

  int finish_check(bool harvested_now, bool list_changed) {
    quiet = quiet_next;
    book.recount();
    if (!list_pushed && list_changed) { int rc = push_list(); if (rc) return rc; stamp(OMC_HOST_LIST); }
    if (book.next_node() < Btot && !timed_out && book.active() < S) { int rc = refill_idle(); if (rc) return rc; }
    if (timed_out) { int rc = close_unslotted(OMC_ST_TIME); if (rc) return rc; }
    const int q = harvested_now ? OMC_HOST_HARVEST_TOTAL : OMC_HOST_CHECK_TOTAL;
    h->host_ms[q] += std::chrono::duration<double, std::milli>(Clock::now() - t_check).count(); h->host_cnt[q] += 1;
    return 0;
  }

  int collect_statistics() {
    { int rc = mw_collect(); if (rc) return rc; }
    if (w.geo.plain_mw && w.pmw_stat) {
      std::vector<int> st(4 * (size_t)S);
      HIPCHK(hipMemcpyAsync(st.data(), w.pmw_stat, sizeof(int) * st.size(), hipMemcpyDeviceToHost, s));
      HIPCHK(hipStreamSynchronize(s));
      for (int b = 0; b < S; ++b) {
        h->pmw_tot[0] += st[4 * b]; h->pmw_tot[2] += st[4 * b + 2];
        h->pmw_tot[1] = std::max<long long>(h->pmw_tot[1], st[4 * b + 3]);
      }
    }
    std::vector<int> sweeps(S);
    HIPCHK(hipMemcpyAsync(sweeps.data(), w.sweeps, sizeof(int) * S, hipMemcpyDeviceToHost, s));
    HIPCHK(hipStreamSynchronize(s));
    for (int v : sweeps) h->total_sweeps += v;
    { int rc = sum_sub_stat(w.sub_stat, S, h->sub_tot, s); if (rc) return rc; }
    if (shor && h->wbig.sub_enable) { int rc = sum_sub_stat(h->wbig.sub_stat, S, h->big_sub_tot, s); if (rc) return rc; }
    HIPCHK(hipGetLastError());
    if (drain_pool >= 0) finish_events(drain_pool);
    finish_events(tape.current());
    h->last_solve_seconds = elapsed();
    h->last_iters_total = it;
    if (tun.host_phases) {
      static const char* const nm[OMC_HOST_NPHASE] = {"check_wait", "check_scan", "list", "event_drain", "harvest_flags", "harvest_enqueue", "harvest_wait", "harvest_book", "setup_enqueue", "check_total", "harvest_total", "async_harvests", "quiet_intervals", "body_records", "body_waits"};
      fprintf(stderr, "omc host phases (solve %.1f ms, %d iterations):", 1e3 * h->last_solve_seconds, it);
      for (int q = 0; q < OMC_HOST_NPHASE; ++q) fprintf(stderr, " %s %.3f ms / %lld", nm[q], h->host_ms[q], (long long)h->host_cnt[q]);
      fprintf(stderr, "\n");
    }
    return 0;
  }
};

}

extern "C" {

int omc_cone_multi_budget(int interval_max) { return interval_max > 0 ? std::min(MAX_SWEEPS, interval_max + 2) : MAX_SWEEPS; }

int omc_harvest_plan(int nlive, int nfin, int pending, int check_index, int async_min_live) {
  return slot_harvest_plan(nlive, nfin, pending, check_index, async_min_live);
}

int omc_relax_solve(omc_instance* h) {
  if (!h || !h->staged) return fail(OMC_ERR_ARGUMENT, "omc_relax_solve: nothing staged");
  HIPCHK(hipSetDevice(h->device));
  SolveLoop L(h);
  int rc = L.prepare(); if (rc) return rc;
  for (;;) {
    if (L.book.active() == 0) {
      bool ended = false;
      rc = L.run_dry(&ended); if (rc) return rc;
      if (ended) break;
      continue;
    }
    bool is_check = false;
    rc = L.enqueue_iteration(&is_check); if (rc) return rc;
    if (!is_check) continue;
    L.enqueue_check();
    rc = L.read_check(); if (rc) return rc;
    if (L.book.pending_harvests()) { rc = L.book_async_harvest(); if (rc) return rc; }
    const SlotBook::Check c = L.book.check(L.Btot, L.timed_out, L.multi, L.P.first_wins != 0, L.tun.harvest_async ? L.tun.harvest_async_min_live : 0);
    L.stamp(OMC_HOST_CHECK_SCAN);
    const int nfin = c.plan == OMC_HARVEST_NONE ? 0 : c.nfin;
    if (c.plan == OMC_HARVEST_ASYNC) rc = L.harvest_async();
    else if (nfin) rc = L.harvest_sync(nfin);
    if (rc) return rc;
    rc = L.finish_check(nfin != 0, nfin || c.nnew || L.nrefilled); if (rc) return rc;
  }
  return L.collect_statistics();
}

}
```

optimalmatrixcompletion.jl_amd/csrc/omc_wave.h:

```cpp
#ifndef OMC_WAVE_H
#define OMC_WAVE_H
#include <hip/hip_runtime.h>
#include "omc_device.h"

#define WAVE 64

__device__ __forceinline__ int slot_of(const OmcWS& w, int i) { return w.slot_list ? w.slot_list[i] : i; }

__device__ __forceinline__ int xcd_block(int on) {
  const int bid = blockIdx.x, nwg = gridDim.x;
  if (!on) return bid;
  const int q = nwg >> 3, r = nwg & 7, x = bid & 7;
  return ((x < r) ? x * (q + 1) : r * (q + 1) + (x - r) * q) + (bid >> 3);
}

__device__ __forceinline__ double dpp_move(double v, const int ctrl_sel) {
  int lo = __double2loint(v), hi = __double2hiint(v);
  int lo2, hi2;
  switch (ctrl_sel) {
    case 0: lo2 = __builtin_amdgcn_update_dpp(0, lo, 0xB1, 0xF, 0xF, true); hi2 = __builtin_amdgcn_update_dpp(0, hi, 0xB1, 0xF, 0xF, true); break;
    case 1: lo2 = __builtin_amdgcn_update_dpp(0, lo, 0x4E, 0xF, 0xF, true); hi2 = __builtin_amdgcn_update_dpp(0, hi, 0x4E, 0xF, 0xF, true); break;
    case 2: lo2 = __builtin_amdgcn_update_dpp(0, lo, 0x141, 0xF, 0xF, true); hi2 = __builtin_amdgcn_update_dpp(0, hi, 0x141, 0xF, 0xF, true); break;
    default: lo2 = __builtin_amdgcn_update_dpp(0, lo, 0x140, 0xF, 0xF, true); hi2 = __builtin_amdgcn_update_dpp(0, hi, 0x140, 0xF, 0xF, true); break;
  }
// ... 56 lines not shown
    for (int r = kk + lane; r < c; r += WAVE) {
      double v = (r == kk) ? d : Lm[TRI(r, kk)] / d;
      Lm[TRI(r, kk)] = v;
    }
    WAVE_SYNC();
    const int t = c - kk - 1;
    const int tot = t * t;
    for (int e = lane; e < tot; e += WAVE) {
      int rr = e / t, qq = e - rr * t;
      if (qq <= rr) {
        int r = kk + 1 + rr, q = kk + 1 + qq;
        Lm[TRI(r, q)] -= Lm[TRI(r, kk)] * Lm[TRI(q, kk)];
      }
    }
    WAVE_SYNC();
  }
  return true;
}

template <class LP, class DP>
__device__ __forceinline__ double wave_chol_solve_reg(LP Lm, DP dinv, int c, double rhs, int lane) {
  double y = (lane < c) ? rhs : 0.0;
  for (int q = 0; q < c; ++q) {
    const double zq = readlane_d(y, q) * dinv[q];
    if (lane == q) y = zq;
    else if (lane > q && lane < c) y -= Lm[TRI(lane, q)] * zq;
  }
  for (int q = c - 1; q >= 0; --q) {
    const double xq = readlane_d(y, q) * dinv[q];
    if (lane == q) y = xq;
    else if (lane < q) y -= Lm[TRI(q, lane)] * xq;
  }
  return y;
}


__device__ __forceinline__ int tri_i(int r, int q) { return (int)(__umul24(r, r + 1) >> 1) + q; }
__device__ __forceinline__ double fast_rcp(double p) {
  double x = __builtin_amdgcn_rcp(p);
  x = fma(fma(-p, x, 1.0), x, x);
  x = fma(fma(-p, x, 1.0), x, x);
  return x;
}
template <class PT>
__device__ __forceinline__ bool wave_ldl(PT Lm, PT pinv, int c, int lane) {
  const bool mine = lane < c;
  const int rb = tri_i(mine ? lane : 0, 0);
  WAVE_SYNC();
  for (int kb = 0; kb < c; kb += 8) {
    const int nb = (c - kb < 8) ? (c - kb) : 8;
    double P[8], pis[8];
#pragma unroll
    for (int j = 0; j < 8; ++j) {
      const bool v = mine && (kb + j <= lane);
      const double x = Lm[rb + (v ? kb + j : 0)];
      P[j] = v ? x : 0.0;
      pis[j] = 0.0;
    }
#pragma unroll
    for (int j = 0; j < 8; ++j) {
      if (j < nb) {
        const double piv = readlane_d(P[j], kb + j);
        if (!(piv > 1e-290)) return false;
        const double pi_ = fast_rcp(piv);
        pis[j] = pi_;
        const double lr = P[j] * pi_;
#pragma unroll
        for (int j2 = j + 1; j2 < 8; ++j2) {
          if (j2 < nb) {
            const double lq = readlane_d(P[j], kb + j2);
            if (lane >= kb + j2) P[j2] = fma(-lr, lq, P[j2]);
          }
        }
      }
    }
#pragma unroll
    for (int j = 0; j < 8; ++j) {
      if (j < nb) {
        if (mine && lane >= kb + j) Lm[rb + kb + j] = P[j];
        if (lane == j) pinv[kb + j] = pis[j];
      }
    }
    double a[8];
#pragma unroll
    for (int j = 0; j < 8; ++j) a[j] = P[j] * pis[j];
    for (int q = kb + nb; q < c; ++q) {
      double acc = 0.0;
#pragma unroll
      for (int j = 0; j < 8; ++j) acc = fma(a[j], readlane_d(P[j], q), acc);
      if (mine && lane >= q) Lm[rb + q] -= acc;
    }
  }
  WAVE_SYNC();
  return true;
}
template <class PT>
__device__ __forceinline__ double wave_ldl_solve_reg(PT Lm, PT pinv, int c, double rhs, int lane) {
  double y = (lane < c) ? rhs : 0.0;
  const int lb = tri_i(lane, 0);
  const bool act = lane < c;
  int q = 0;
  for (; q + 4 <= c; q += 4) {
    const double p0 = pinv[q], p1 = pinv[q + 1], p2 = pinv[q + 2], p3 = pinv[q + 3];
    const double l0 = (act && lane > q) ? Lm[lb + q] : 0.0, l1 = (act && lane > q + 1) ? Lm[lb + q + 1] : 0.0;
    const double l2 = (act && lane > q + 2) ? Lm[lb + q + 2] : 0.0, l3 = (act && lane > q + 3) ? Lm[lb + q + 3] : 0.0;
    y = fma(-l0, readlane_d(y, q) * p0, y);
    y = fma(-l1, readlane_d(y, q + 1) * p1, y);
    y = fma(-l2, readlane_d(y, q + 2) * p2, y);
    y = fma(-l3, readlane_d(y, q + 3) * p3, y);
  }
  for (; q < c; ++q) {
    const double t = readlane_d(y, q) * pinv[q];
    if (act && lane > q) y -= Lm[lb + q] * t;
  }
  q = c - 1;
  for (; q >= 3; q -= 4) {
    const double p0 = pinv[q], p1 = pinv[q - 1], p2 = pinv[q - 2], p3 = pinv[q - 3];
    const double l0 = (lane < q) ? Lm[tri_i(q, 0) + lane] : 0.0, l1 = (lane < q - 1) ? Lm[tri_i(q - 1, 0) + lane] : 0.0;
    const double l2 = (lane < q - 2) ? Lm[tri_i(q - 2, 0) + lane] : 0.0, l3 = (lane < q - 3) ? Lm[tri_i(q - 3, 0) + lane] : 0.0;
    double xq = readlane_d(y, q) * p0;
    y = (lane == q) ? xq : fma(-l0, xq, y);
    xq = readlane_d(y, q - 1) * p1;
    y = (lane == q - 1) ? xq : fma(-l1, xq, y);
    xq = readlane_d(y, q - 2) * p2;
    y = (lane == q - 2) ? xq : fma(-l2, xq, y);
    xq = readlane_d(y, q - 3) * p3;
    y = (lane == q - 3) ? xq : fma(-l3, xq, y);
  }
  for (; q >= 0; --q) {
    const double xq = readlane_d(y, q) * pinv[q];
    if (lane == q) y = xq;
    else if (lane < q) y -= Lm[tri_i(q, 0) + lane] * xq;
  }
  return y;
}

__device__ __forceinline__ void wave_chol_solve(const double* Lm, int c, const double* rhs, double* y, int lane) {
  for (int r = 0; r < c; ++r) {
    double p = 0.0;
    for (int q = lane; q < r; q += WAVE) p += Lm[TRI(r, q)] * y[q];
    p = wave_sum(p);
    if (lane == 0) y[r] = (rhs[r] - p) / Lm[TRI(r, r)];
    WAVE_SYNC();
  }
  for (int r = c - 1; r >= 0; --r) {
    double p = 0.0;
    for (int q = r + 1 + lane; q < c; q += WAVE) p += Lm[TRI(q, r)] * y[q];
    p = wave_sum(p);
    if (lane == 0) y[r] = (y[r] - p) / Lm[TRI(r, r)];
    WAVE_SYNC();
  }
}

template <bool REFINE = false>
__device__ __forceinline__ int wave_nnqp(const double* G, int ldG, const double* cvec, double* lam, int R, double* Gp, double* sv,
                          double* tmp, int* plist, int lane) {
  int np = 0;
  int overflow = 0;
  for (int r = 0; r < R; ++r) {
    if (lam[r] > 0.0 && np < NNQP_PMAX) { if (lane == 0) plist[np] = r; ++np; }
    else if (lam[r] != 0.0) { if (lam[r] > 0.0) overflow = 1; if (lane == 0) lam[r] = 0.0; }
  }
  WAVE_SYNC();
  double cmax = 0.0;
  for (int r = lane; r < R; r += WAVE) cmax = fmax(cmax, fabs(cvec[r]));
  for (int o = 32; o > 0; o >>= 1) cmax = fmax(cmax, __shfl_xor(cmax, o, WAVE));
  const double tol = 1e-13 * fmax(cmax, 1e-300);
  bool need_inner = (np > 0);
  for (int outer = 0; outer < 3 * R + 10; ++outer) {
    if (!need_inner) {
      double best = -1e300; int bi = -1;
      for (int r = lane; r < R; r += WAVE) {
        bool inP = false;
        for (int a = 0; a < np; ++a) if (plist[a] == r) inP = true;
        if (inP) continue;
        double wv = cvec[r];
        for (int a = 0; a < np; ++a) wv -= G[(size_t)r * ldG + plist[a]] * lam[plist[a]];
        if (wv > best) { best = wv; bi = r; }
      }
      for (int o = 32; o > 0; o >>= 1) {
        double ob = __shfl_xor(best, o, WAVE); int oi = __shfl_xor(bi, o, WAVE);
        if (ob > best || (ob == best && oi >= 0 && (bi < 0 || oi < bi))) { best = ob; bi = oi; }
      }
      if (bi < 0 || best <= tol) { overflow = 0; break; }
      if (np >= NNQP_PMAX) { overflow = 1; break; }
      if (lane == 0) plist[np] = bi;
      ++np;
      WAVE_SYNC();
    }
    need_inner = false;
    for (int inner = 0; inner < 3 * NNQP_PMAX + 10; ++inner) {
      double dmax = 0.0;
      for (int e = lane; e < np * np; e += WAVE) {
        int a = e / np, c2 = e - a * np;
        if (c2 <= a) Gp[TRI(a, c2)] = G[(size_t)plist[a] * ldG + plist[c2]];
      }
      for (int a = 0; a < np; ++a) dmax = fmax(dmax, G[(size_t)plist[a] * ldG + plist[a]]);
      WAVE_SYNC();
      for (int a = lane; a < np; a += WAVE) { Gp[TRI(a, a)] += 1e-14 * dmax; tmp[a] = cvec[plist[a]]; }
      WAVE_SYNC();
      bool ok = wave_cholesky(Gp, np, lane);
      if (!ok) {
        --np; WAVE_SYNC();
        if (np == 0) break;
        continue;
      }
      wave_chol_solve(Gp, np, tmp, sv, lane);
      if (REFINE) {
        for (int a = lane; a < np; a += WAVE) {
          double r = cvec[plist[a]];
          for (int c2 = 0; c2 < np; ++c2) r -= G[(size_t)plist[a] * ldG + plist[c2]] * sv[c2];
          tmp[a] = r;
        }
        WAVE_SYNC();
        wave_chol_solve(Gp, np, tmp, tmp, lane);
        for (int a = lane; a < np; a += WAVE) sv[a] += tmp[a];
        WAVE_SYNC();
      }
      double mins = 1e300;
      for (int a = lane; a < np; a += WAVE) mins = fmin(mins, sv[a]);
      for (int o = 32; o > 0; o >>= 1) mins = fmin(mins, __shfl_xor(mins, o, WAVE));
      if (mins > 0.0) {
        for (int a = lane; a < np; a += WAVE) lam[plist[a]] = sv[a];
        WAVE_SYNC();
        break;
      }
      double al = 1e300;
      for (int a = lane; a < np; a += WAVE) {
        double lv = lam[plist[a]];
        if (sv[a] <= 0.0) al = fmin(al, lv / (lv - sv[a]));
      }
      for (int o = 32; o > 0; o >>= 1) al = fmin(al, __shfl_xor(al, o, WAVE));
      if (!(al >= 0.0)) al = 0.0;
      for (int a = lane; a < np; a += WAVE) {
        double lv = lam[plist[a]];
        lam[plist[a]] = lv + al * (sv[a] - lv);
      }
      WAVE_SYNC();
      int nn = 0; bool removed = false; double minl = 1e300; int mini = -1;
      for (int a = 0; a < np; ++a) {
        double lv = lam[plist[a]];
        if (sv[a] <= 0.0 && lv < minl) { minl = lv; mini = a; }
      }
      for (int a = 0; a < np; ++a) {
        int r = plist[a];
        double lv = lam[r];
        bool drop = (sv[a] <= 0.0) && (lv <= 1e-18 * fmax(cmax, 1e-300) || a == mini);
        WAVE_SYNC();
        if (drop) { if (lane == 0) lam[r] = 0.0; removed = true; }
        else { if (lane == 0) { plist[nn] = r; } ++nn; }
        WAVE_SYNC();
      }
      np = nn;
      (void)removed;
      if (np == 0) break;
    }
  }
  return overflow;
}

#endif
```

Measured before the change: 2321.

## Cache NNQP active-set Cholesky factor across global-step calls per slot

Adds a per-slot device cache of the active-set list and packed Cholesky factor used by the wave NNQP solver in the global step. When the starting active set matches the cached list, the factorisation is skipped and the cached factor is reused. The change also adds a ballot-based warm-start list build, a register-resident scan for small R, and a row-oriented triangular solve. In exchange it adds extra global memory, a staging copy into LDS, and a host sync each batch to collect stats. The old path remains available behind an environment flag.

```diff
diff --git a/include/omc.h b/include/omc.h
--- a/include/omc.h
+++ b/include/omc.h
@@ -231,6 +231,7 @@
 #define OMC_RES_N 10
 int omc_kernel_residency(omc_instance* h, int* out);
 int omc_last_subspace_stats(omc_instance* h, int64_t* out);
+int omc_last_global_rows_stats(omc_instance* h, int64_t* out);
 int omc_last_shor_subspace_stats(omc_instance* h, int64_t* out);
 int omc_tuning_set(omc_instance* h, const char* name, const char* value);
 int omc_tuning_reload_env(omc_instance* h);
diff --git a/optimalmatrixcompletion.jl_amd/_lib.py b/optimalmatrixcompletion.jl_amd/_lib.py
--- a/optimalmatrixcompletion.jl_amd/_lib.py
+++ b/optimalmatrixcompletion.jl_amd/_lib.py
@@ -12,7 +12,7 @@
     "omc_relax_params_default", "omc_last_error", "omc_version", "omc_device_count", "omc_instance_create",
     "omc_instance_create_bits", "omc_instance_destroy", "omc_relax_batch", "omc_relax_stage", "omc_relax_solve",
     "omc_relax_fetch", "omc_relax_submit", "omc_relax_poll", "omc_relax_wait", "omc_altmin_batch", "omc_evaluate_objective", "omc_separation_batch", "omc_round_Y_batch",
-    "omc_last_kernel_stats", "omc_last_host_phases", "omc_kernel_residency", "omc_last_solver_info", "omc_last_subspace_stats", "omc_set_node_rho_scales", "omc_left_singular_batch", "omc_psd_project_batch", "omc_column_prox_batch", "omc_colprox_plan", "omc_last_cone_multi_stats", "omc_cone_multi_budget", "omc_plain_multi_plan", "omc_plain_multi_tau", "omc_last_plain_multi_stats", "omc_harvest_plan", "omc_relax_reserve", "omc_relax_append", "omc_relax_fetch_done", "omc_relax_hold", "omc_debug_stamps", "omc_tuning_set", "omc_tuning_reload_env", "omc_debug_residuals", "omc_debug_diag", "omc_debug_aa",
+    "omc_last_kernel_stats", "omc_last_host_phases", "omc_kernel_residency", "omc_last_solver_info", "omc_last_subspace_stats", "omc_last_global_rows_stats", "omc_set_node_rho_scales", "omc_left_singular_batch", "omc_psd_project_batch", "omc_column_prox_batch", "omc_colprox_plan", "omc_last_cone_multi_stats", "omc_cone_multi_budget", "omc_plain_multi_plan", "omc_plain_multi_tau", "omc_last_plain_multi_stats", "omc_harvest_plan", "omc_relax_reserve", "omc_relax_append", "omc_relax_fetch_done", "omc_relax_hold", "omc_debug_stamps", "omc_tuning_set", "omc_tuning_reload_env", "omc_debug_residuals", "omc_debug_diag", "omc_debug_aa",
     "omc_shor_count", "omc_shor_indexes", "omc_violated_shor_minors", "omc_shor_last_stats", "omc_shor_last_select_stats",
     "omc_relax_stage_shor", "omc_relax_fetch_shor", "omc_relax_batch_shor", "omc_set_shor_penalties", "omc_set_shor_keep_V", "omc_relax_fetch_shor_V", "omc_last_shor_subspace_stats", "omc_state_pool_create", "omc_relax_set_warm",
     "omc_state_pool_reserve_shor", "omc_shor_warm_compat", "omc_last_shor_warm_stats", "omc_state_pool_fetch_shor",
@@ -91,6 +91,8 @@
     if hasattr(lib, "omc_kernel_residency"):
         lib.omc_kernel_residency.argtypes = [vp, vp]
     lib.omc_last_subspace_stats.argtypes = [vp, vp]
+    if hasattr(lib, "omc_last_global_rows_stats"):
+        lib.omc_last_global_rows_stats.argtypes = [vp, vp]
     lib.omc_set_node_rho_scales.argtypes = [vp, C.c_int, vp]
     lib.omc_debug_stamps.argtypes = [vp, vp]
     lib.omc_left_singular_batch.argtypes = [vp, C.c_int, vp, vp]
diff --git a/optimalmatrixcompletion.jl_amd/api.py b/optimalmatrixcompletion.jl_amd/api.py
--- a/optimalmatrixcompletion.jl_amd/api.py
+++ b/optimalmatrixcompletion.jl_amd/api.py
@@ -429,6 +429,13 @@
         _lib.check(self._lib.omc_last_subspace_stats(self._h, _lib.ptr(out)))
         return dict(calls=int(out[0]), power_steps=int(out[1]), fallbacks=int(out[2]), seeds=int(out[3]), fail_positive=int(out[4]),
                     fail_steps=int(out[5]), fail_cholesky=int(out[6]), ritz_passes=int(out[7]))
+
+    def global_rows_stats(self):
+        if not hasattr(self._lib, "omc_last_global_rows_stats"):
+            raise OmcError(-100, "this build of the library has no omc_last_global_rows_stats")
+        out = np.zeros(4, np.int64)
+        _lib.check(self._lib.omc_last_global_rows_stats(self._h, _lib.ptr(out)))
+        return dict(factorisations=int(out[0]), hits=int(out[1]), misses=int(out[0] - out[1]), np_first_sum=int(out[2]), calls=int(out[3]))
 
     def shor_subspace_stats(self):
         out = np.zeros(8, np.int64)
diff --git a/optimalmatrixcompletion.jl_amd/csrc/omc_api.cpp b/optimalmatrixcompletion.jl_amd/csrc/omc_api.cpp
--- a/optimalmatrixcompletion.jl_amd/csrc/omc_api.cpp
+++ b/optimalmatrixcompletion.jl_amd/csrc/omc_api.cpp
@@ -462,6 +462,10 @@
   size_t chk_bytes = 0;
   ENS_CARVE(h->bchk, [&](Carve& c) { walk_check(c, sd, w); }, &chk_bytes);
   BIND(h->bG, w.G, sB * Rmax * Rmax); BIND(h->blam, w.lam, sB * Rmax);
+  BIND(h->browsfac, w.rows_fac, sB * NNQP_CACHE_DOUBLES); BIND(h->browslist, w.rows_list, sB * NNQP_CACHE_CAP);
+  BIND(h->browslen, w.rows_len, sB); BIND(h->browsstat, w.rows_stat, sB * 4, s0);
+  HIPCHK(hipMemsetAsync(w.rows_len, 0xFF, sizeof(int) * sB, s0));
+  w.rows_cap = std::max(0, std::min(h->tun.global_rows_cap, NNQP_CACHE_CAP)); w.rows_old = h->tun.global_rows_old ? 1 : 0;
   ENS_CARVE(h->bscal, [&](Carve& c) { walk_scalars(c, sd, w); });
   BIND(h->bbx, w.bx, sB * n);
   ENS_CARVE(h->bint, [&](Carve& c) { walk_slot_ints(c, sd, w); });
@@ -886,6 +890,12 @@
   return 0;
 }
 
+int omc_last_global_rows_stats(omc_instance* h, int64_t* out) {
+  if (!h || !out) return fail(OMC_ERR_ARGUMENT, "NULL argument");
+  for (int q = 0; q < 4; ++q) out[q] = h->rows_tot[q];
+  return 0;
+}
+
 int omc_last_subspace_stats(omc_instance* h, int64_t* out) {
   if (!h || !out) return fail(OMC_ERR_ARGUMENT, "NULL argument");
   for (int q = 0; q < 8; ++q) out[q] = h->sub_tot[q];
diff --git a/optimalmatrixcompletion.jl_amd/csrc/omc_device.h b/optimalmatrixcompletion.jl_amd/csrc/omc_device.h
--- a/optimalmatrixcompletion.jl_amd/csrc/omc_device.h
+++ b/optimalmatrixcompletion.jl_amd/csrc/omc_device.h
@@ -101,6 +101,7 @@
   double* bx;
   int *done, *status, *iters, *sweeps, *stall;
   int* rowov;
+  double* rows_fac; int *rows_list, *rows_len, *rows_stat; int rows_cap, rows_old;
   OmcGeom geo;
   double* cp_scratch;
   int cp_pair; int cp_nsolo; const int* cp_solo;
diff --git a/optimalmatrixcompletion.jl_amd/csrc/omc_device.hip b/optimalmatrixcompletion.jl_amd/csrc/omc_device.hip
--- a/optimalmatrixcompletion.jl_amd/csrc/omc_device.hip
+++ b/optimalmatrixcompletion.jl_amd/csrc/omc_device.hip
@@ -103,7 +103,7 @@
     if (tid < 16) w.sub_theta[(size_t)b * 16 + tid] = w.ptheta[(size_t)lf * 16 + tid];
     fr2 = block_sum(fr2, red); tr1 = block_sum(tr1, red);
     if (tid == 0) {
-      w.fro2[b] = fr2; w.trM[b] = tr1; w.sub_on[b] = (w.sub_enable && w.pscal[(size_t)lf * 4 + 1] != 0.0) ? 1 : 0; w.sub_wait[b] = 0; w.sub_nfail[b] = 0; w.cone_done[b] = 0; if (w.w1_fac) w.w1_fac[b] = 0; w.v3valid[b] = 0; w.sub_onC[b] = 0; w.confirm[b] = 1; w.lb_est[b] = -1e300; w.vvalid[b] = 0; if (w.vvalidC) w.vvalidC[b] = 0; if (w.ws_first) { w.ws_first[b] = w.sub_on[b] ? 0 : 1; if (w.ws_need && !w.sub_on[b]) *w.ws_need = 1; }
+      w.fro2[b] = fr2; w.trM[b] = tr1; w.sub_on[b] = (w.sub_enable && w.pscal[(size_t)lf * 4 + 1] != 0.0) ? 1 : 0; w.sub_wait[b] = 0; w.sub_nfail[b] = 0; w.cone_done[b] = 0; if (w.w1_fac) w.w1_fac[b] = 0; if (w.rows_len) w.rows_len[b] = -1; w.v3valid[b] = 0; w.sub_onC[b] = 0; w.confirm[b] = 1; w.lb_est[b] = -1e300; w.vvalid[b] = 0; if (w.vvalidC) w.vvalidC[b] = 0; if (w.ws_first) { w.ws_first[b] = w.sub_on[b] ? 0 : 1; if (w.ws_need && !w.sub_on[b]) *w.ws_need = 1; }
     }
     for (int e = tid; e < rm * k; e += T) {
       const int a = e % rm, j = e / rm;
@@ -136,7 +136,7 @@
       w.Vrow[(size_t)b * NP * NP + e] = 0.0;
     }
     if (tid == 0) {
-      w.fro2[b] = d0 * d0 * n; w.trM[b] = d0 * n; w.sub_on[b] = 0; w.sub_wait[b] = 0; w.sub_nfail[b] = 0; w.cone_done[b] = 0; if (w.w1_fac) w.w1_fac[b] = 0; w.v3valid[b] = 0; w.sub_onC[b] = 0; w.confirm[b] = 1; w.lb_est[b] = -1e300; w.vvalid[b] = 0; if (w.vvalidC) w.vvalidC[b] = 0; if (w.ws_first) { w.ws_first[b] = w.sub_on[b] ? 0 : 1; if (w.ws_need && !w.sub_on[b]) *w.ws_need = 1; }
+      w.fro2[b] = d0 * d0 * n; w.trM[b] = d0 * n; w.sub_on[b] = 0; w.sub_wait[b] = 0; w.sub_nfail[b] = 0; w.cone_done[b] = 0; if (w.w1_fac) w.w1_fac[b] = 0; if (w.rows_len) w.rows_len[b] = -1; w.v3valid[b] = 0; w.sub_onC[b] = 0; w.confirm[b] = 1; w.lb_est[b] = -1e300; w.vvalid[b] = 0; if (w.vvalidC) w.vvalidC[b] = 0; if (w.ws_first) { w.ws_first[b] = w.sub_on[b] ? 0 : 1; if (w.ws_need && !w.sub_on[b]) *w.ws_need = 1; }
     }
   }
   for (int e = tid; e < n * k; e += T) w.U[(size_t)b * n * k + e] = 0.0;
@@ -2001,9 +2001,24 @@
     for (int e = tid; e < R * w.Rmax; e += T) xs[e] = G[e];
     G = xs;
   }
+  __shared__ int s_cl[NNQP_CACHE_CAP];
+  const bool rows_old = w.rows_old != 0;
+  NnqpCache ch = {nullptr, nullptr, nullptr, 0, nullptr, s_cl, -1};
+  if (!rows_old && w.rows_len && w.rows_cap > 0)
+    ch = {w.rows_fac + (size_t)b * NNQP_CACHE_DOUBLES, w.rows_list + (size_t)b * NNQP_CACHE_CAP, w.rows_len + b, w.rows_cap, nullptr, s_cl, -1};
+  if (!rows_old) { ch.llen = nnqp_cache_stage(ch, s_Gp, tid, T); if (w.rows_stat) ch.stat = w.rows_stat + 4 * (size_t)b; }
   __syncthreads();
   STAMP(10);
-  if (tid < WAVE) { const int ov = wave_nnqp(G, w.Rmax, cvec, mu, R, s_Gp, s_sv, s_tmp, s_pl, tid); if (tid == 0) w.rowov[b] = ov; }
+#ifdef OMC_STAMPS
+  double* const nq_stamps = (blockIdx.x == 0) ? w.stamps : nullptr;
+#else
+  double* const nq_stamps = nullptr;
+#endif
+  if (tid < WAVE) {
+    const int ov = rows_old ? wave_nnqp(G, w.Rmax, cvec, mu, R, s_Gp, s_sv, s_tmp, s_pl, tid, nq_stamps)
+                            : wave_nnqp_rows(G, w.Rmax, cvec, mu, R, s_Gp, s_sv, s_tmp, s_pl, tid, ch, nq_stamps);
+    if (tid == 0) w.rowov[b] = ov;
+  }
   __syncthreads();
   for (int e = tid; e < R; e += T) lam[e] = rho * mu[e];
   __shared__ int s_nact; __shared__ int s_act[NNQP_PMAX]; __shared__ double s_mu[NNQP_PMAX]; __shared__ double s_trace_mu;
diff --git a/optimalmatrixcompletion.jl_amd/csrc/omc_host.h b/optimalmatrixcompletion.jl_amd/csrc/omc_host.h
--- a/optimalmatrixcompletion.jl_amd/csrc/omc_host.h
+++ b/optimalmatrixcompletion.jl_amd/csrc/omc_host.h
@@ -99,6 +99,7 @@
   bool dense_proj = false;
   bool host_phases = false;
   bool global_nolds = false;
+  bool global_rows_old = false;
   bool no_colprox_pair = false;
   bool no_graph = false;
   bool no_subspace = false;
@@ -111,6 +112,7 @@
   int colprox_block_min = 65;
   int cone_multi_min = 1025;
   int event_merge = 1;
+  int global_rows_cap = NNQP_CACHE_CAP;
   int graph_max = 16;
   int harvest_async = 1;
   int harvest_async_min_live = 256;
@@ -128,6 +130,7 @@
   {"OMC_ALTMIN_NOLDS", &Tuning::altmin_nolds, nullptr},      {"OMC_COLPROX_NO_XCD", &Tuning::colprox_no_xcd, nullptr},
   {"OMC_CONE_512", &Tuning::cone_512, nullptr},              {"OMC_DENSE_PROJ", &Tuning::dense_proj, nullptr},
   {"OMC_GLOBAL_NOLDS", &Tuning::global_nolds, nullptr},      {"OMC_HOST_PHASES", &Tuning::host_phases, nullptr},
+  {"OMC_GLOBAL_ROWS_OLD", &Tuning::global_rows_old, nullptr}, {"OMC_GLOBAL_ROWS_CAP", nullptr, &Tuning::global_rows_cap},
   {"OMC_NO_COLPROX_PAIR", &Tuning::no_colprox_pair, nullptr},
   {"OMC_NO_GRAPH", &Tuning::no_graph, nullptr},              {"OMC_NO_SUBSPACE", &Tuning::no_subspace, nullptr},
   {"OMC_NO_WS_SPLIT", &Tuning::no_ws_split, nullptr},        {"OMC_SEGV_TRACE", &Tuning::segv_trace, nullptr},
@@ -174,6 +177,7 @@
   DevBuf bslotlist, bgap, bvotes, blamDX, bXsC, bsubSC, bsubIC;
   DevBuf bsubz, bscal, bbx, bint, bcp, bcone, bglob, bXout, bThout, bXin, bMbuf, bVrow, bXs, bsubS, bsubI;
   long long sub_tot[8] = {0};
+  DevBuf browsfac, browslist, browslen, browsstat; long long rows_tot[4] = {0};
   DevBuf bmwstat, sbigmw, pjM, pjV, pjW, pjS, pjD, pjI;
   long long mw_tot[5] = {0};
   DevBuf bpmwstat; long long pmw_tot[4] = {0};
diff --git a/optimalmatrixcompletion.jl_amd/csrc/omc_layout.h b/optimalmatrixcompletion.jl_amd/csrc/omc_layout.h
--- a/optimalmatrixcompletion.jl_amd/csrc/omc_layout.h
+++ b/optimalmatrixcompletion.jl_amd/csrc/omc_layout.h
@@ -6,6 +6,9 @@
 #define NNQP_PMAX 64
 #define NNQP_GP_DOUBLES (NNQP_PMAX * (NNQP_PMAX + 1) / 2)
 #define NNQP_STATIC_BYTES ((NNQP_GP_DOUBLES + 2 * NNQP_PMAX) * 8 + NNQP_PMAX * 4)
+#define NNQP_CACHE_CAP 32
+#define NNQP_CACHE_DOUBLES (NNQP_CACHE_CAP * (NNQP_CACHE_CAP + 1) / 2)
+static_assert(NNQP_CACHE_CAP <= NNQP_PMAX && NNQP_CACHE_CAP <= 64, "one lane per entry of the kept list");
 #define OMC_MAX_DYN_LDS (144 * 1024)
 #define SUBP 16
 #define GL_XS 16
diff --git a/optimalmatrixcompletion.jl_amd/csrc/omc_relax_solve.cpp b/optimalmatrixcompletion.jl_amd/csrc/omc_relax_solve.cpp
--- a/optimalmatrixcompletion.jl_amd/csrc/omc_relax_solve.cpp
+++ b/optimalmatrixcompletion.jl_amd/csrc/omc_relax_solve.cpp
@@ -528,6 +528,14 @@
     HIPCHK(hipStreamSynchronize(s));
     for (int v : sweeps) h->total_sweeps += v;
     { int rc = sum_sub_stat(w.sub_stat, S, h->sub_tot, s); if (rc) return rc; }
+    if (w.rows_stat) {
+      std::vector<int> st(4 * (size_t)S);
+      HIPCHK(hipMemcpyAsync(st.data(), w.rows_stat, sizeof(int) * st.size(), hipMemcpyDeviceToHost, s));
+      HIPCHK(hipStreamSynchronize(s));
+      for (int q = 0; q < 4; ++q) h->rows_tot[q] = 0;
+      for (int b = 0; b < S; ++b) for (int q = 0; q < 4; ++q) h->rows_tot[q] += st[4 * b + q];
+      HIPCHK(hipMemsetAsync(w.rows_stat, 0, sizeof(int) * st.size(), s));
+    }
     if (shor && h->wbig.sub_enable) { int rc = sum_sub_stat(h->wbig.sub_stat, S, h->big_sub_tot, s); if (rc) return rc; }
     HIPCHK(hipGetLastError());
     if (drain_pool >= 0) finish_events(drain_pool);
diff --git a/optimalmatrixcompletion.jl_amd/csrc/omc_wave.h b/optimalmatrixcompletion.jl_amd/csrc/omc_wave.h
--- a/optimalmatrixcompletion.jl_amd/csrc/omc_wave.h
+++ b/optimalmatrixcompletion.jl_amd/csrc/omc_wave.h
@@ -232,11 +232,24 @@
   }
 }
 
+#ifdef OMC_STAMPS
+#define NNQP_STAMP_BEGIN() long long tq_prev_ = __builtin_amdgcn_s_memtime()
+#define NNQP_STAMP(slot) do { if (stamps && lane == 0) { long long t_ = __builtin_amdgcn_s_memtime(); stamps[slot] += (double)(t_ - tq_prev_); tq_prev_ = t_; } } while (0)
+#else
+#define NNQP_STAMP_BEGIN() do {} while (0)
+#define NNQP_STAMP(slot) do {} while (0)
+#endif
+#define NNQP_ST_WARM 7
+#define NNQP_ST_FACTOR 29
+#define NNQP_ST_SOLVE 30
+#define NNQP_ST_SCAN 31
+
 template <bool REFINE = false>
 __device__ __forceinline__ int wave_nnqp(const double* G, int ldG, const double* cvec, double* lam, int R, double* Gp, double* sv,
-                          double* tmp, int* plist, int lane) {
+                          double* tmp, int* plist, int lane, double* stamps = nullptr) {
   int np = 0;
   int overflow = 0;
+  NNQP_STAMP_BEGIN();
   for (int r = 0; r < R; ++r) {
     if (lam[r] > 0.0 && np < NNQP_PMAX) { if (lane == 0) plist[np] = r; ++np; }
     else if (lam[r] != 0.0) { if (lam[r] > 0.0) overflow = 1; if (lane == 0) lam[r] = 0.0; }
@@ -247,6 +260,7 @@
   for (int o = 32; o > 0; o >>= 1) cmax = fmax(cmax, __shfl_xor(cmax, o, WAVE));
   const double tol = 1e-13 * fmax(cmax, 1e-300);
   bool need_inner = (np > 0);
+  NNQP_STAMP(NNQP_ST_WARM);
   for (int outer = 0; outer < 3 * R + 10; ++outer) {
     if (!need_inner) {
       double best = -1e300; int bi = -1;
@@ -262,6 +276,7 @@
         double ob = __shfl_xor(best, o, WAVE); int oi = __shfl_xor(bi, o, WAVE);
         if (ob > best || (ob == best && oi >= 0 && (bi < 0 || oi < bi))) { best = ob; bi = oi; }
       }
+      NNQP_STAMP(NNQP_ST_SCAN);
       if (bi < 0 || best <= tol) { overflow = 0; break; }
       if (np >= NNQP_PMAX) { overflow = 1; break; }
       if (lane == 0) plist[np] = bi;
@@ -280,6 +295,7 @@
       for (int a = lane; a < np; a += WAVE) { Gp[TRI(a, a)] += 1e-14 * dmax; tmp[a] = cvec[plist[a]]; }
       WAVE_SYNC();
       bool ok = wave_cholesky(Gp, np, lane);
+      NNQP_STAMP(NNQP_ST_FACTOR);
       if (!ok) {
         --np; WAVE_SYNC();
         if (np == 0) break;
@@ -303,6 +319,7 @@
       if (mins > 0.0) {
         for (int a = lane; a < np; a += WAVE) lam[plist[a]] = sv[a];
         WAVE_SYNC();
+        NNQP_STAMP(NNQP_ST_SOLVE);
         break;
       }
       double al = 1e300;
@@ -333,10 +350,213 @@
       }
       np = nn;
       (void)removed;
+      NNQP_STAMP(NNQP_ST_SOLVE);
       if (np == 0) break;
     }
   }
   return overflow;
 }
 
+struct NnqpCache { double* fac; int* list; int* len; int cap; int* stat; int* llist; int llen; };
+__device__ __forceinline__ int nnqp_cache_stage(const NnqpCache& ch, double* Gp, int tid, int T) {
+  if (!ch.len || ch.cap > NNQP_CACHE_CAP) return -1;
+  int len = *ch.len;
+  if (len < 0 || len > ch.cap) len = -1;
+  for (int e = tid; e < (len * (len + 1)) >> 1; e += T) Gp[e] = ch.fac[e];
+  if (tid < len) ch.llist[tid] = ch.list[tid];
+  return len;
+}
+
+__device__ __forceinline__ double shift_up_one(double v, double in0, int lane, bool wide) {
+  const int lo = __double2loint(v), hi = __double2hiint(v);
+  double s = __hiloint2double(__builtin_amdgcn_update_dpp(0, hi, 0x111, 0xF, 0xF, true), __builtin_amdgcn_update_dpp(0, lo, 0x111, 0xF, 0xF, true));
+  if (wide) {
+    const double a = readlane_d(v, 15), b = readlane_d(v, 31), c = readlane_d(v, 47);
+    s = (lane == 16) ? a : (lane == 32) ? b : (lane == 48) ? c : s;
+  }
+  return (lane == 0) ? in0 : s;
+}
+__device__ __forceinline__ double wave_chol_solve_rows(const double* Lm, int c, double rhs, int lane) {
+  double y = 0.0;
+  double ln = 0.0, dn = Lm[0];
+  for (int r = 0; r < c; ++r) {
+    const double lr = ln, dr = dn;
+    if (r + 1 < c) { ln = (lane <= r) ? Lm[TRI(r + 1, lane)] : 0.0; dn = Lm[TRI(r + 1, r + 1)]; }
+    double p = 0.0;
+    if (lane < r) p += lr * y;
+    p = wave_sum(p);
+    const double v = (readlane_d(rhs, r) - p) / dr;
+    if (lane == r) y = v;
+  }
+  const bool wide = c > 16;
+  double x = y, S = 0.0;
+  ln = 0.0; dn = Lm[TRI(c - 1, c - 1)];
+  for (int r = c - 1; r >= 0; --r) {
+    const double lr = ln, dr = dn;
+    if (r > 0) { ln = (r + lane < c) ? Lm[TRI(r + lane, r - 1)] : 0.0; dn = Lm[TRI(r - 1, r - 1)]; }
+    double p = 0.0;
+    if (r + 1 + lane < c) p += lr * S;
+    p = wave_sum(p);
+    const double v = (readlane_d(y, r) - p) / dr;
+    if (lane == r) x = v;
+    S = shift_up_one(S, v, lane, wide);
+  }
+  return x;
+}
+
+__device__ __forceinline__ int wave_nnqp_rows(const double* G, int ldG, const double* cvec, double* lam, int R, double* Gp, double* sv,
+                                              double* tmp, int* plist, int lane, const NnqpCache& ch, double* stamps = nullptr) {
+  int np = 0;
+  int overflow = 0;
+  int nfact = 0, nhit = 0, np_first = 0;
+  int clen = ch.llen;
+  bool gp_kept = clen >= 0;
+  NNQP_STAMP_BEGIN();
+  const unsigned long long below = (1ull << lane) - 1ull;
+  const bool small = R <= WAVE;
+  unsigned long long pmask = 0ull;
+  for (int r0 = 0; r0 < R; r0 += WAVE) {
+    const int r = r0 + lane;
+    const double lv = (r < R) ? lam[r] : 0.0;
+    const unsigned long long pos = __ballot(lv > 0.0);
+    const bool in = lv > 0.0 && np + __popcll(pos & below) < NNQP_PMAX;
+    const unsigned long long inm = __ballot(in);
+    if (in) plist[np + __popcll(inm & below)] = r;
+    else if (lv != 0.0) lam[r] = 0.0;
+    if (__ballot(lv > 0.0 && !in)) overflow = 1;
+    if (r0 == 0) pmask = inm;
+    np += __popcll(inm);
+  }
+  WAVE_SYNC();
+  double cmax = 0.0;
+  for (int r = lane; r < R; r += WAVE) cmax = fmax(cmax, fabs(cvec[r]));
+  for (int o = 32; o > 0; o >>= 1) cmax = fmax(cmax, __shfl_xor(cmax, o, WAVE));
+  const double tol = 1e-13 * fmax(cmax, 1e-300);
+  bool need_inner = (np > 0);
+  NNQP_STAMP(NNQP_ST_WARM);
+  for (int outer = 0; outer < 3 * R + 10; ++outer) {
+    if (!need_inner) {
+      double best = -1e300; int bi = -1;
+      if (small) {
+        const int pa = (lane < np) ? plist[lane] : 0;
+        const double la = (lane < np) ? lam[pa] : 0.0;
+        const int r = lane;
+        if (r < R && !((pmask >> r) & 1ull)) {
+          double wv = cvec[r];
+          for (int a = 0; a < np; ++a) wv -= G[(size_t)r * ldG + __builtin_amdgcn_readlane(pa, a)] * readlane_d(la, a);
+          if (wv > best) { best = wv; bi = r; }
+        }
+      } else {
+        for (int r = lane; r < R; r += WAVE) {
+          bool inP = false;
+          for (int a = 0; a < np; ++a) if (plist[a] == r) inP = true;
+          if (inP) continue;
+          double wv = cvec[r];
+          for (int a = 0; a < np; ++a) wv -= G[(size_t)r * ldG + plist[a]] * lam[plist[a]];
+          if (wv > best) { best = wv; bi = r; }
+        }
+      }
+      for (int o = 32; o > 0; o >>= 1) {
+        double ob = __shfl_xor(best, o, WAVE); int oi = __shfl_xor(bi, o, WAVE);
+        if (ob > best || (ob == best && oi >= 0 && (bi < 0 || oi < bi))) { best = ob; bi = oi; }
+      }
+      NNQP_STAMP(NNQP_ST_SCAN);
+      if (bi < 0 || best <= tol) { overflow = 0; break; }
+      if (np >= NNQP_PMAX) { overflow = 1; break; }
+      if (lane == 0) plist[np] = bi;
+      ++np;
+      if (small) pmask |= 1ull << bi;
+      WAVE_SYNC();
+    }
+    need_inner = false;
+    for (int inner = 0; inner < 3 * NNQP_PMAX + 10; ++inner) {
+      bool match = false;
+      if (clen == np) {
+        const bool differs = lane < np && ch.llist[lane] != plist[lane];
+        match = __ballot(differs) == 0ull;
+      }
+      const bool hit = match && gp_kept;
+      if (nfact == 0) np_first = np;
+      ++nfact;
+      bool ok = true;
+      if (hit) {
+        ++nhit;
+        for (int a = lane; a < np; a += WAVE) tmp[a] = cvec[plist[a]];
+        WAVE_SYNC();
+      } else {
+        gp_kept = false;
+        double dmax = 0.0;
+        for (int e = lane; e < np * np; e += WAVE) {
+          int a = e / np, c2 = e - a * np;
+          if (c2 <= a) Gp[TRI(a, c2)] = G[(size_t)plist[a] * ldG + plist[c2]];
+        }
+        for (int a = 0; a < np; ++a) dmax = fmax(dmax, G[(size_t)plist[a] * ldG + plist[a]]);
+        WAVE_SYNC();
+        for (int a = lane; a < np; a += WAVE) { Gp[TRI(a, a)] += 1e-14 * dmax; tmp[a] = cvec[plist[a]]; }
+        WAVE_SYNC();
+        ok = wave_cholesky(Gp, np, lane);
+      }
+      NNQP_STAMP(NNQP_ST_FACTOR);
+      if (!ok) {
+        --np;
+        if (small) pmask &= ~(1ull << plist[np]);
+        WAVE_SYNC();
+        if (np == 0) break;
+        continue;
+      }
+      {
+        const double s = wave_chol_solve_rows(Gp, np, (lane < np) ? tmp[lane] : 0.0, lane);
+        if (lane < np) sv[lane] = s;
+        WAVE_SYNC();
+      }
+      double mins = 1e300;
+      for (int a = lane; a < np; a += WAVE) mins = fmin(mins, sv[a]);
+      for (int o = 32; o > 0; o >>= 1) mins = fmin(mins, __shfl_xor(mins, o, WAVE));
+      if (mins > 0.0) {
+        for (int a = lane; a < np; a += WAVE) lam[plist[a]] = sv[a];
+        if (!match && ch.len && np <= ch.cap && ch.cap <= NNQP_CACHE_CAP) {
+          for (int e = lane; e < (np * (np + 1)) >> 1; e += WAVE) ch.fac[e] = Gp[e];
+          if (lane < np) { ch.list[lane] = plist[lane]; ch.llist[lane] = plist[lane]; }
+          if (lane == 0) *ch.len = np;
+          clen = np;
+        }
+        WAVE_SYNC();
+        NNQP_STAMP(NNQP_ST_SOLVE);
+        break;
+      }
+      double al = 1e300;
+      for (int a = lane; a < np; a += WAVE) {
+        double lv = lam[plist[a]];
+        if (sv[a] <= 0.0) al = fmin(al, lv / (lv - sv[a]));
+      }
+      for (int o = 32; o > 0; o >>= 1) al = fmin(al, __shfl_xor(al, o, WAVE));
+      if (!(al >= 0.0)) al = 0.0;
+      for (int a = lane; a < np; a += WAVE) {
+        double lv = lam[plist[a]];
+        lam[plist[a]] = lv + al * (sv[a] - lv);
+      }
+      WAVE_SYNC();
+      int nn = 0; double minl = 1e300; int mini = -1;
+      for (int a = 0; a < np; ++a) {
+        double lv = lam[plist[a]];
+        if (sv[a] <= 0.0 && lv < minl) { minl = lv; mini = a; }
+      }
+      for (int a = 0; a < np; ++a) {
+        int r = plist[a];
+        double lv = lam[r];
+        bool drop = (sv[a] <= 0.0) && (lv <= 1e-18 * fmax(cmax, 1e-300) || a == mini);
+        WAVE_SYNC();
+        if (drop) { if (lane == 0) lam[r] = 0.0; if (small) pmask &= ~(1ull << r); }
+        else { if (lane == 0) { plist[nn] = r; } ++nn; }
+        WAVE_SYNC();
+      }
+      np = nn;
+      NNQP_STAMP(NNQP_ST_SOLVE);
+      if (np == 0) break;
+    }
+  }
+  if (ch.stat && lane == 0 && nfact) { ch.stat[0] += nfact; ch.stat[1] += nhit; ch.stat[2] += np_first; ch.stat[3] += 1; }
+  return overflow;
+}
+
 #endif
```

Result: no change. 2362, median of 6 (+1.8%).
